# SonSang/dmesh2_renderer

Hardware: AMD Instinct MI355X
Metric: Mpixels/s fwd+bwd @1080p/1M tris (higher is better)
Workload: dtype f32

## Files before the change

dmesh2_renderer_amd/_C.py:

```python
from __future__ import annotations

import ctypes
import os
import threading

import torch

_HERE = os.path.dirname(os.path.abspath(__file__))
LIB_PATH = os.environ.get("DM2_HIP_LIB") or os.path.join(_HERE, "csrc", "libdm2_hip.so")
_lib = None
_lock = threading.Lock()

DM2_FLAG_CORRECTED_DV = 1
DM2_FLAG_LEGACY_KERNELS = 2
DM2_FLAG_NO_BACKWARD = 4
DM2_FLAG_ANALYTIC_RAYS = 8
DM2_FLAG_AA_GRAD_TO_VERTS = 16
DM2_FLAG_TABLES_FROM_IMAGE = 32
DM2_FLAG_NO_PAIR_POOL = 64
SCRATCH_FACE, SCRATCH_IMAGE, SCRATCH_BINNING, SCRATCH_LAYER_IMAGE, SCRATCH_LAYER_TETS, SCRATCH_PAIR_POOL, SCRATCH_TIE_QUEUE = range(7)
FWD_UNKNOWN, FWD_NONE, FWD_MASKS, FWD_POOL, FWD_POINT = 0, 1, 2, 3, 4
ABI_VERSION = 6

_flags = 0
_bin_hint: dict = {}

_vp, _i32, _i64, _sz = ctypes.c_void_p, ctypes.c_int32, ctypes.c_int64, ctypes.c_size_t


class RenderDesc(ctypes.Structure):
    _fields_ = [
        ("B", _i32), ("P", _i32), ("F", _i32), ("W", _i32), ("H", _i32), ("K", _i32),
        ("aa_temperature", ctypes.c_float), ("flags", _i32), ("full_W", _i32), ("full_H", _i32),
        ("background", _vp), ("patch_min", _vp), ("verts", _vp), ("faces", _vp), ("verts_color", _vp),
        ("faces_opacity", _vp), ("verts_ndc", _vp), ("verts_image", _vp), ("faces_intense", _vp),
        ("aa_face_verts", _vp), ("aa_face_edges", _vp), ("aa_face_edges_iszero", _vp),
        ("aa_face_edges_recip", _vp), ("aa_face_edges_normal", _vp), ("aa_face_edges_normal_c", _vp),
        ("image_ray_o", _vp), ("image_ray_d", _vp), ("ray_cam", _vp),
    ]


class PrepDesc(ctypes.Structure):
    _fields_ = [
        ("B", _i32), ("P", _i32), ("F", _i32), ("W", _i32), ("H", _i32),
        ("verts", _vp), ("faces", _vp), ("mv", _vp), ("proj", _vp),
        ("verts_ndc", _vp), ("verts_image", _vp), ("aa_face_verts", _vp), ("aa_face_edges", _vp),
        ("aa_face_edges_iszero", _vp), ("aa_face_edges_recip", _vp), ("aa_face_edges_normal", _vp),
        ("aa_face_edges_normal_c", _vp),
    ]


class LayersDesc(ctypes.Structure):
    _fields_ = [
        ("B", _i32), ("P", _i32), ("F", _i32), ("T", _i32), ("W", _i32), ("H", _i32), ("L", _i32), ("flags", _i32),
        ("verts", _vp), ("faces", _vp), ("tets", _vp), ("face_tets", _vp), ("tet_faces", _vp),
        ("face_existence", _vp), ("verts_ndc", _vp), ("verts_image", _vp), ("image_ray_o", _vp), ("image_ray_d", _vp),
        ("ray_cam", _vp),
    ]


class LayerCompositeDesc(ctypes.Structure):
    _fields_ = [
        ("B", _i32), ("P", _i32), ("F", _i32), ("W", _i32), ("H", _i32), ("L", _i32), ("flags", _i32),
        ("render_layers", _vp), ("verts", _vp), ("faces", _vp), ("verts_color", _vp), ("faces_opacity", _vp),
        ("faces_intense", _vp), ("verts_ndc", _vp), ("background", _vp), ("image_ray_o", _vp), ("image_ray_d", _vp),
        ("ray_cam", _vp),
    ]


EXPORTS = {
    "dm2_abi_version": (ctypes.c_int, []),
    "dm2_last_error": (ctypes.c_char_p, []),
    "dm2_scratch_bytes": (_sz, [ctypes.c_int, _i64, _i64]),
    "dm2_forward_plan": (ctypes.c_int, [ctypes.POINTER(RenderDesc), _vp, _sz, _vp, ctypes.POINTER(_i64), ctypes.POINTER(_i64), ctypes.POINTER(_i64)]),
    "dm2_forward_run": (ctypes.c_int, [ctypes.POINTER(RenderDesc), _i64, _i64, _i64, _vp, _sz, _vp, _sz, _vp, _sz, _vp, _vp, _vp, _vp,
                                       ctypes.POINTER(_i32)]),
    "dm2_forward": (ctypes.c_int, [ctypes.POINTER(RenderDesc), _vp, _sz, _vp, _sz, _vp, _sz, _vp, _vp, _vp, _vp,
                                   ctypes.POINTER(_i64), ctypes.POINTER(_i64), ctypes.POINTER(_i64), ctypes.POINTER(_i32)]),
    "dm2_backward": (ctypes.c_int, [ctypes.POINTER(RenderDesc), _i64, _i32, _vp, _vp, _vp, _sz, _vp, _sz, _vp, _sz, _vp, _sz,
                                    _vp, _vp, _vp, _vp, _vp, _vp, _vp]),
    "dm2_layers_plan": (ctypes.c_int, [ctypes.POINTER(LayersDesc), _vp, _sz, _vp, ctypes.POINTER(_i64), ctypes.POINTER(_i64)]),
    "dm2_layers_run": (ctypes.c_int, [ctypes.POINTER(LayersDesc), _i64, _i64, _vp, _sz, _vp, _sz, _vp, _sz, _vp, _sz, _vp, _vp, _vp]),
    "dm2_rasterize_run": (ctypes.c_int, [ctypes.POINTER(LayersDesc), _i64, _i64, _vp, _sz, _vp, _sz, _vp, _sz, _vp, _vp, _vp, _vp, _vp]),
    "dm2_rasterize_backward": (ctypes.c_int, [ctypes.POINTER(LayersDesc), _vp, _vp, _vp, _vp, _vp]),
    "dm2_interpolate": (ctypes.c_int, [_i32] * 8 + [_vp] * 6),
    "dm2_interpolate_backward": (ctypes.c_int, [_i32] * 8 + [_vp] * 8),
    "dm2_texture": (ctypes.c_int, [_i32] * 10 + [_vp] * 5),
    "dm2_texture_backward": (ctypes.c_int, [_i32] * 10 + [_vp] * 7),
    "dm2_layers_composite": (ctypes.c_int, [ctypes.POINTER(LayerCompositeDesc), _vp, _vp, _vp, _vp, _vp]),
    "dm2_layers_composite_backward": (ctypes.c_int, [ctypes.POINTER(LayerCompositeDesc), _vp, _vp, _vp, _vp, _vp, _vp, _vp, _vp]),
    "dm2_layers_composite_backward_alpha": (ctypes.c_int, [ctypes.POINTER(LayerCompositeDesc), _vp, _vp, _vp, _vp, _vp, _vp, _vp, _vp,
                                                            _vp]),
    "dm2_forward_alpha": (ctypes.c_int, [ctypes.POINTER(RenderDesc), _vp, _sz, _vp, _vp]),
    "dm2_forward_weights": (ctypes.c_int, [ctypes.POINTER(RenderDesc), _vp, _sz, _vp, _sz, _vp, _sz, _vp, _vp, _vp, _vp, _vp,
                                           ctypes.POINTER(_i64), ctypes.POINTER(_i64), ctypes.POINTER(_i64), ctypes.POINTER(_i32)]),
    "dm2_forward_run_weights": (ctypes.c_int, [ctypes.POINTER(RenderDesc), _i64, _i64, _i64, _vp, _sz, _vp, _sz, _vp, _sz, _vp, _vp,
                                               _vp, _vp, _vp, ctypes.POINTER(_i32)]),
    "dm2_layers_composite_weights": (ctypes.c_int, [ctypes.POINTER(LayerCompositeDesc), _vp, _vp, _vp, _vp, _vp, _vp]),
    "dm2_backward_alpha": (ctypes.c_int, [ctypes.POINTER(RenderDesc), _i64, _i32, _vp, _vp, _vp, _vp, _sz, _vp, _sz, _vp, _sz, _vp,
                                          _sz, _vp, _vp, _vp, _vp, _vp, _vp, _vp]),
    "dm2_prepare_faces": (ctypes.c_int, [ctypes.POINTER(PrepDesc), _vp]),
    "dm2_prepare_faces_backward": (ctypes.c_int, [ctypes.POINTER(PrepDesc), _vp, _vp, _vp, _vp, _vp, _vp]),
    "dm2_prepare_faces_camera_scratch_bytes": (_sz, [_i32, _i32]),
    "dm2_prepare_faces_backward_camera": (ctypes.c_int, [ctypes.POINTER(PrepDesc), _vp, _vp, _vp, _vp, _vp, _vp, _vp, _vp, _vp]),
    "dm2_exchange_mark": (ctypes.c_int, [_i32, _i32, _i32, _i32, _vp, _vp, _sz, _vp, _vp, _vp]),
    "dm2_exchange_pack": (ctypes.c_int, [_i32, _i32, _i32, _i32, _vp, _vp, _vp, _vp, _vp, _vp, _vp, _vp, _vp]),
    "dm2_exchange_unpack": (ctypes.c_int, [_i32, _i32, _i32, _i32, _i32, _vp, _vp, _i64, _vp, _vp, _vp]),
    "dm2_debug_aa_overlap": (ctypes.c_int, [ctypes.c_int, _i64, _vp, _vp, _vp, _vp, _vp, _vp, _vp, _vp, _vp, _vp, _vp]),
    "dm2_debug_fetch": (ctypes.c_int, [ctypes.c_int, _i64, _i64, _i64, _vp, _sz, _vp, _vp]),
    "dm2_profile_enable": (None, [ctypes.c_int]),
    "dm2_profile_read": (ctypes.c_int, [ctypes.POINTER(ctypes.c_float), ctypes.c_int]),
    "dm2_debug_stamps": (ctypes.c_int, [ctypes.POINTER(ctypes.c_uint64), ctypes.c_int, ctypes.c_int]),
}

STAGE_NAMES = ["preprocess_scan", "bin_scatter", "tile_sort", "tile_ranges", "forward_composite", "backward_composite", "backward_ties"]


def profile_enable(on: bool):
    load_library().dm2_profile_enable(1 if on else 0)


def profile_read():
    buf = (ctypes.c_float * len(STAGE_NAMES))()
    n = load_library().dm2_profile_read(buf, len(STAGE_NAMES))
    return {STAGE_NAMES[i]: float(buf[i]) for i in range(n)}


def load_library(path: str | None = None):
    global _lib
    with _lock:
        if _lib is not None and path is None:
            return _lib
        p = path or LIB_PATH
        if not os.path.exists(p):
            raise RuntimeError(
                f"dmesh2_renderer_amd: native library not found at {p}; build it with "
                f"`python -c 'import __graft_entry__ as g; g.build()'` or `make -C dmesh2_renderer_amd/csrc` "
                f"(there is no CPU fallback)")
        lib = ctypes.CDLL(p)
        for name, (res, args) in EXPORTS.items():
            fn = getattr(lib, name)
            fn.restype = res
            fn.argtypes = args
        if lib.dm2_abi_version() != ABI_VERSION:
            raise RuntimeError("dmesh2_renderer_amd: ABI version mismatch")
        if path is None:
            _lib = lib
        return lib


def set_flags(flags: int):
    global _flags
    old, _flags = _flags, int(flags)
    return old


def _err(lib, what):
    msg = lib.dm2_last_error()
    return RuntimeError(f"{what}: {msg.decode() if msg else 'unknown error'}")


def _require_gpu(*tensors):
    for t in tensors:
        if not t.is_cuda:
            raise RuntimeError(
                "dmesh2_renderer_amd: all tensors must live on a ROCm GPU (got a CPU tensor); "
                "this build has no CPU path -- the CPU restatement under oracle/ is test infrastructure only")
    dev = tensors[0].device
    for t in tensors:
        if t.device != dev:
            raise RuntimeError("dmesh2_renderer_amd: tensors are on different devices")
    return dev


def _c(t, dtype):
    if t.dtype != dtype:
        raise RuntimeError(f"expected dtype {dtype}, got {t.dtype}")
    return t.contiguous()


def _ptr(t):
    return ctypes.c_void_p(t.data_ptr() if t is not None and t.numel() > 0 else 0)


def _stream(dev):
    return ctypes.c_void_p(torch.cuda.current_stream(dev).cuda_stream)


def _bytes(dev, n):
    return torch.empty((max(int(n), 0),), dtype=torch.uint8, device=dev)


def _check_render_shapes(background, patch_min, verts, faces, verts_color, faces_opacity, verts_ndc, verts_image,
                         faces_intense, aa_v, aa_e, aa_z, aa_r, aa_n, aa_c, ray_o, ray_d, temp, K):
    def bad(cond, msg):
        if cond:
            raise RuntimeError(msg)
    bad(background.dim() != 1 or background.size(0) != 3, "background must have dimensions (3,)")
    bad(patch_min.dim() != 2 or patch_min.size(1) != 2, "patch_min must have dimensions (B, 2)")
    bad(verts.dim() != 2 or verts.size(1) != 3, "verts must have dimensions (P, 3)")
    bad(faces.dim() != 2 or faces.size(1) != 3, "faces must have dimensions (F, 3)")
    bad(verts_color.dim() != 2 or verts_color.size(1) != 3, "vert color must have dimensions (P, 3)")
    bad(faces_opacity.dim() != 1 or faces_opacity.size(0) != faces.size(0), "face opacity must have dimensions (F,)")
    bad(verts_ndc.dim() != 3 or verts_ndc.size(2) != 3, "verts_ndc must have dimensions (B, P, 3)")
    bad(verts_image.dim() != 3 or verts_image.size(2) != 2, "verts_image must have dimensions (B, P, 2)")
    bad(faces_intense.dim() != 2 or faces_intense.size(1) != faces.size(0), "faces_intense must have dimensions (B, F,)")
    for t, nm in ((aa_v, "aa_face_verts"), (aa_e, "aa_face_edges"), (aa_z, "aa_face_edges_iszero"),
                  (aa_r, "aa_face_edges_recip"), (aa_n, "aa_face_edges_normal")):
        bad(t.dim() != 4 or t.size(2) != 3 or t.size(3) != 2, f"{nm} must have dimensions (B, F, 3, 2)")
    bad(aa_c.dim() != 3 or aa_c.size(2) != 3, "aa_face_edges_normal_c must have dimensions (B, F, 3)")
    bad(ray_o.dim() != 4 or ray_o.size(3) != 3, "image_ray_o must have dimensions (B, H, W, 3)")
    bad(ray_d.dim() != 4 or ray_d.size(3) != 3, "image_ray_d must have dimensions (B, H, W, 3)")
    bad(temp < 0 or temp > 1, "aa_temperature must be in the range [0, 1]")
    bad(K < 0, "len_oarea_buffer must be non-negative")


def _make_desc(args, keep):
    (background, patch_min, pw, ph, verts, faces, verts_color, faces_opacity, verts_ndc, verts_image, faces_intense,
     temp, aa_v, aa_e, aa_z, aa_r, aa_n, aa_c, K, ray_o, ray_d) = args
    temp = float(temp); K = int(K); pw = int(pw); ph = int(ph)
    _check_render_shapes(background, patch_min, verts, faces, verts_color, faces_opacity, verts_ndc, verts_image,
                         faces_intense, aa_v, aa_e, aa_z, aa_r, aa_n, aa_c, ray_o, ray_d, temp, K)
    dev = _require_gpu(background, patch_min, verts, faces, verts_color, faces_opacity, verts_ndc, verts_image,
                       faces_intense, aa_v, aa_e, aa_z, aa_r, aa_n, aa_c, ray_o, ray_d)
    f32, i32 = torch.float32, torch.int32
    B, P, F = verts_ndc.size(0), verts.size(0), faces.size(0)
    def need(t, shape, nm):
        if tuple(t.shape) != tuple(shape):
            raise RuntimeError(f"{nm} has shape {tuple(t.shape)}, expected {tuple(shape)}")
    need(patch_min, (B, 2), "patch_min"); need(verts_color, (P, 3), "verts_color"); need(verts_ndc, (B, P, 3), "verts_ndc")
    need(verts_image, (B, P, 2), "verts_image"); need(faces_intense, (B, F), "faces_intense")
    from_image = bool(getattr(_tls, "tables_from_image", False))
    if not from_image:
        for t, nm in ((aa_v, "aa_face_verts"), (aa_e, "aa_face_edges"), (aa_z, "aa_face_edges_iszero"),
                      (aa_r, "aa_face_edges_recip"), (aa_n, "aa_face_edges_normal")):
            need(t, (B, F, 3, 2), nm)
        need(aa_c, (B, F, 3), "aa_face_edges_normal_c")
    ana = _analytic(B, dev)
    if ana is None:
        need(ray_o, (B, ph, pw, 3), "image_ray_o"); need(ray_d, (B, ph, pw, 3), "image_ray_d")
    if temp == 0.0:
        K = 0
    ts = dict(
        background=_c(background, f32), patch_min=_c(patch_min, i32), verts=_c(verts, f32), faces=_c(faces, i32),
        verts_color=_c(verts_color, f32), faces_opacity=_c(faces_opacity, f32), verts_ndc=_c(verts_ndc, f32),
        verts_image=_c(verts_image, f32), faces_intense=_c(faces_intense, f32), aa_face_verts=_c(aa_v, f32),
        aa_face_edges=_c(aa_e, f32), aa_face_edges_iszero=_c(aa_z, torch.bool), aa_face_edges_recip=_c(aa_r, f32),
        aa_face_edges_normal=_c(aa_n, f32), aa_face_edges_normal_c=_c(aa_c, f32), image_ray_o=_c(ray_o, f32),
        image_ray_d=_c(ray_d, f32))
    keep.append(ts)
    d = RenderDesc()
    d.B, d.P, d.F, d.W, d.H, d.K = B, P, F, pw, ph, K
    d.aa_temperature = temp
    d.flags = _flags
    for k, t in ts.items():
        setattr(d, k, t.data_ptr() if t.numel() > 0 else None)
    if from_image:
        d.flags |= DM2_FLAG_TABLES_FROM_IMAGE
        for k in ("aa_face_verts", "aa_face_edges", "aa_face_edges_iszero", "aa_face_edges_recip", "aa_face_edges_normal", "aa_face_edges_normal_c"):
            setattr(d, k, None)
    if ana is not None:
# ... 101 lines not shown

    def __exit__(self, *exc):
        _tls.fwd_mode = self.old


def last_forward_mode():
    return getattr(_tls, "last_fwd_mode", FWD_UNKNOWN)


def last_pair_bound():
    return getattr(_tls, "last_pair_bound", 0)


def _pool_budget(N, R):
    return min(max(256 * N, 16 * R, 1 << 24), 400_000_000)


def _analytic(B, dev):
    a = getattr(_tls, "analytic", None)
    if a is None:
        return None
    cam, w, h = a
    if cam.dtype != torch.float32 or tuple(cam.shape) != (B, 32) or cam.device != dev:
        raise RuntimeError(f"analytic_rays: ray_cam must be float32 (B, 32) on {dev}, got {cam.dtype} {tuple(cam.shape)} on {cam.device}")
    return cam.contiguous(), w, h


def render_forward_cuda(*args):
    if len(args) != 21:
        raise TypeError(f"render_forward_cuda() takes 21 positional arguments ({len(args)} given)")
    lib = load_library()
    keep: list = []
    d, dev, (B, P, F, W, H, K) = _make_desc(args, keep)
    if getattr(_tls, "forward_only", False):
        d.flags |= DM2_FLAG_NO_BACKWARD
    if getattr(_tls, "aa_to_verts", False):
        d.flags |= DM2_FLAG_AA_GRAD_TO_VERTS
    want_alpha = bool(getattr(_tls, "alpha_output", False))
    want_weights = bool(getattr(_tls, "face_weights_output", False))
    with torch.cuda.device(dev):
        st = _stream(dev)
        f32, i32 = torch.float32, torch.int32
        weights = torch.zeros((B, F), dtype=f32, device=dev) if want_weights else None
        color = torch.empty((B, H, W, 3), dtype=f32, device=dev)
        depth = torch.empty((B, H, W), dtype=f32, device=dev)
        oarea = torch.empty((B, H, W, 0), dtype=f32, device=dev)
        tri_id = torch.empty((B, H, W, 0), dtype=i32, device=dev)
        doarea = torch.empty((B, H, W, 0, 3, 2), dtype=f32, device=dev)
        N, Tn, BF = B * H * W, _tiles(B, W, H), B * F
        if P == 0 or BF == 0 or N == 0:
            color.zero_(); depth.zero_()
            tri_cnt = torch.zeros((B, H, W), dtype=i32, device=dev)
            e = _bytes(dev, 0)
            _tls.last_pair_bound = 0
            out = (0, color, depth, oarea, tri_id, tri_cnt, doarea, e, _bytes(dev, 0), _bytes(dev, 0))
            if want_alpha:
                out += (torch.zeros((B, H, W), dtype=f32, device=dev),)
            return out + (weights,) if want_weights else out
        tri_cnt = torch.empty((B, H, W), dtype=i32, device=dev)
        face_buf = _bytes(dev, lib.dm2_scratch_bytes(SCRATCH_FACE, BF, 2 * Tn + 1))
        img_buf = _bytes(dev, lib.dm2_scratch_bytes(SCRATCH_IMAGE, N, Tn))
        nr, longest, pairs, mode = _i64(0), _i64(0), _i64(0), _i32(0)
        key = (dev.index, B, W, H, F)
        with _lock:
            hint = _bin_hint.get(key, 0)
        if _pool_budget(N, 0) <= 0:
            d.flags |= DM2_FLAG_NO_PAIR_POOL
        bin_buf = _bytes(dev, hint)
        fwd_args = (ctypes.byref(d), _ptr(face_buf), face_buf.numel(), _ptr(bin_buf), bin_buf.numel(), _ptr(img_buf), img_buf.numel(),
                    _ptr(color), _ptr(depth), _ptr(tri_cnt))
        fwd_tail = (st, ctypes.byref(nr), ctypes.byref(longest), ctypes.byref(pairs), ctypes.byref(mode))
        if want_weights:
            rc = lib.dm2_forward_weights(*fwd_args, _ptr(weights), *fwd_tail)
        else:
            rc = lib.dm2_forward(*fwd_args, *fwd_tail)
        if rc not in (0, 2):
            raise _err(lib, "render_forward_cuda")
        R = int(nr.value)
        wants_pool = d.aa_temperature > 0.0 and not (d.flags & (DM2_FLAG_NO_BACKWARD | DM2_FLAG_LEGACY_KERNELS | DM2_FLAG_NO_PAIR_POOL))
        over = wants_pool and int(pairs.value) > _pool_budget(N, R)
        pool = lib.dm2_scratch_bytes(SCRATCH_PAIR_POOL, int(pairs.value), 0) if wants_pool and not over else 0
        need = lib.dm2_scratch_bytes(SCRATCH_BINNING, R, Tn) + pool
        if rc == 2 or (over and int(mode.value) == FWD_POOL):
            if over:
                d.flags |= DM2_FLAG_NO_PAIR_POOL
            bin_buf = _bytes(dev, need + need // 4)
            run_args = (ctypes.byref(d), R, int(longest.value), int(pairs.value), _ptr(face_buf), face_buf.numel(), _ptr(bin_buf),
                        bin_buf.numel(), _ptr(img_buf), img_buf.numel(), _ptr(color), _ptr(depth), _ptr(tri_cnt))
            if want_weights:
                weights.zero_()
                rc = lib.dm2_forward_run_weights(*run_args, _ptr(weights), st, ctypes.byref(mode))
            else:
                rc = lib.dm2_forward_run(*run_args, st, ctypes.byref(mode))
            if rc:
                raise _err(lib, "render_forward_cuda (run)")
        with _lock:
            hint = _bin_hint.get(key, 0)
            if need > hint or 2 * (need + need // 4) < hint:
                if len(_bin_hint) > 64:
                    _bin_hint.clear()
                _bin_hint[key] = need + need // 4
        if want_alpha:
            alpha = torch.empty((B, H, W), dtype=f32, device=dev)
            if lib.dm2_forward_alpha(ctypes.byref(d), _ptr(img_buf), img_buf.numel(), _ptr(alpha), st):
                raise _err(lib, "render_forward_cuda (alpha)")
    _tls.last_fwd_mode = int(mode.value)
    _tls.last_pair_bound = int(pairs.value)
    bin_buf._dm2_fwd_mode = int(mode.value)
    out = (R, color, depth, oarea, tri_id, tri_cnt, doarea, face_buf, bin_buf, img_buf)
    if want_alpha:
        out += (alpha,)
    return out + (weights,) if want_weights else out


def render_backward_cuda(*args, dL_dout_alpha=None):
    if len(args) != 31:
        raise TypeError(f"render_backward_cuda() takes 31 positional arguments ({len(args)} given)")
    lib = load_library()
    num_rendered = int(args[0])
    fwd_args = args[1:22]
    dL_dcolor, dL_ddepth = args[22], args[23]
    face_buf, bin_buf, img_buf = args[24], args[25], args[26]
    keep: list = []
    d, dev, (B, P, F, W, H, K) = _make_desc(fwd_args, keep)
    _require_gpu(dL_dcolor, dL_ddepth)
    f32 = torch.float32
    to_verts = bool(getattr(_tls, "aa_to_verts", False))
    if to_verts:
        d.flags |= DM2_FLAG_AA_GRAD_TO_VERTS
    sizes = [P * 3, P * 3, F, B * F, B * P * 3, B * P * 2 if to_verts else B * F * 6]
    packed = torch.zeros((sum(sizes),), dtype=f32, device=dev)
    parts = torch.split(packed, sizes)
    g_verts = parts[0].view(P, 3); g_color = parts[1].view(P, 3); g_opac = parts[2].view(F)
    g_int = parts[3].view(B, F); g_ndc = parts[4].view(B, P, 3)
    g_aa = parts[5].view(B, P, 2) if to_verts else parts[5].view(B, F, 3, 2)
    if F != 0 and P != 0 and num_rendered > 0 and B * H * W > 0:
        if tuple(dL_dcolor.shape) != (B, H, W, 3) or tuple(dL_ddepth.shape) != (B, H, W):
            raise RuntimeError("dL_dout_color / dL_dout_depth must have dimensions (B, H, W, 3) / (B, H, W)")
        dc = _c(dL_dcolor, f32); dd = _c(dL_ddepth, f32)
        da = None
        if dL_dout_alpha is not None:
            if tuple(dL_dout_alpha.shape) != (B, H, W):
                raise RuntimeError("dL_dout_alpha must have dimensions (B, H, W)")
            _require_gpu(dL_dcolor, dL_dout_alpha)
            da = _c(dL_dout_alpha, f32)
        mode = getattr(_tls, "fwd_mode", None)
        if mode is None:
            mode = getattr(bin_buf, "_dm2_fwd_mode", FWD_UNKNOWN)
        with torch.cuda.device(dev):
            tie_buf = None
            if mode not in (FWD_MASKS, FWD_NONE) and d.aa_temperature > 0.0 and not (d.flags & DM2_FLAG_LEGACY_KERNELS):
                pool_pairs = max(0, bin_buf.numel() - lib.dm2_scratch_bytes(SCRATCH_BINNING, num_rendered, _tiles(B, W, H))) // 4
                if pool_pairs > 0:
                    tie_buf = _bytes(dev, lib.dm2_scratch_bytes(SCRATCH_TIE_QUEUE, pool_pairs, 0))
            tail = (_ptr(face_buf), face_buf.numel(), _ptr(bin_buf), bin_buf.numel(), _ptr(img_buf), img_buf.numel(),
                    _ptr(tie_buf), tie_buf.numel() if tie_buf is not None else 0,
                    _ptr(g_verts), _ptr(g_color), _ptr(g_opac), _ptr(g_ndc), _ptr(g_int), _ptr(g_aa), _stream(dev))
            if da is None:
                rc = lib.dm2_backward(ctypes.byref(d), num_rendered, int(mode), _ptr(dc), _ptr(dd), *tail)
            else:
                rc = lib.dm2_backward_alpha(ctypes.byref(d), num_rendered, int(mode), _ptr(dc), _ptr(dd), _ptr(da), *tail)
            if rc:
                raise _err(lib, "render_backward_cuda")
    g_verts._dm2_packed = packed
    return g_verts, g_color, g_opac, g_ndc, g_int, g_aa


def generate_render_layers_cuda(width, height, verts, faces, tets, face_tets, tet_faces, face_existence,
                                verts_ndc, verts_image, image_ray_o, image_ray_d, num_layers):
    lib = load_library()

    def bad(cond, msg):
        if cond:
            raise RuntimeError(msg)
    bad(verts.dim() != 2 or verts.size(1) != 3, "verts must have dimensions (P, 3)")
    bad(faces.dim() != 2 or faces.size(1) != 3, "faces must have dimensions (F, 3)")
    bad(tets.dim() != 2 or tets.size(1) != 4, "tets must have dimensions (T, 4)")
    bad(face_tets.dim() != 2 or face_tets.size(1) != 2, "face_tets must have dimensions (F, 2)")
    bad(tet_faces.dim() != 2 or tet_faces.size(1) != 4, "tet_faces must have dimensions (T, 4)")
    bad(face_existence.dim() != 1 or face_existence.size(0) != faces.size(0), "face_existence must have dimensions (F,)")
    bad(verts_ndc.dim() != 3 or verts_ndc.size(2) != 3, "verts_ndc must have dimensions (B, P, 3)")
    bad(verts_image.dim() != 3 or verts_image.size(2) != 2, "verts_image must have dimensions (B, P, 2)")
    bad(image_ray_o.dim() != 4 or image_ray_o.size(3) != 3, "image_ray_o must have dimensions (B, H, W, 3)")
    bad(image_ray_d.dim() != 4 or image_ray_d.size(3) != 3, "image_ray_d must have dimensions (B, H, W, 3)")
    num_layers = int(num_layers); width = int(width); height = int(height)
    bad(num_layers < 0, "num_layers must be non-negative")
    dev = _require_gpu(verts, faces, tets, face_tets, tet_faces, face_existence, verts_ndc, verts_image, image_ray_o, image_ray_d)
    f32, i32 = torch.float32, torch.int32
    B, P, F, T = verts_ndc.size(0), verts.size(0), faces.size(0), tets.size(0)
    bad(tuple(face_tets.shape) != (F, 2), "face_tets must have dimensions (F, 2)")
    bad(tuple(tet_faces.shape) != (T, 4), "tet_faces must have dimensions (T, 4)")
    bad(tuple(verts_ndc.shape) != (B, P, 3) or tuple(verts_image.shape) != (B, P, 2), "verts_ndc/verts_image shape mismatch")
    ana = _analytic(B, dev)
    bad(ana is None and (tuple(image_ray_o.shape) != (B, height, width, 3) or tuple(image_ray_d.shape) != (B, height, width, 3)),
        "image_ray_o/image_ray_d must have dimensions (B, H, W, 3)")
    ts = dict(verts=_c(verts, f32), faces=_c(faces, i32), tets=_c(tets, i32), face_tets=_c(face_tets, i32),
              tet_faces=_c(tet_faces, i32), face_existence=_c(face_existence, i32), verts_ndc=_c(verts_ndc, f32),
              verts_image=_c(verts_image, f32), image_ray_o=_c(image_ray_o, f32), image_ray_d=_c(image_ray_d, f32))
    d = LayersDesc()
    d.B, d.P, d.F, d.T, d.W, d.H, d.L, d.flags = B, P, F, T, width, height, num_layers, _flags
    for k, t in ts.items():
        setattr(d, k, t.data_ptr() if t.numel() > 0 else None)
    if ana is not None:
        if (ana[1], ana[2]) != (width, height):
            raise RuntimeError("analytic_rays: the image size differs from generate_render_layers_cuda's width / height")
        d.flags |= DM2_FLAG_ANALYTIC_RAYS
        d.ray_cam = ana[0].data_ptr()
        d.image_ray_o = d.image_ray_d = None
    with torch.cuda.device(dev):
        st = _stream(dev)
        cnt = torch.zeros((B, height, width), dtype=i32, device=dev)
        layers = torch.full((B, height, width, num_layers), -1, dtype=i32, device=dev)
        N, Tn, BF = B * height * width, _tiles(B, width, height), B * F
        if N == 0:
            return layers, cnt
        face_buf = _bytes(dev, lib.dm2_scratch_bytes(SCRATCH_FACE, BF, 2 * Tn))
        img_buf = _bytes(dev, lib.dm2_scratch_bytes(SCRATCH_LAYER_IMAGE, N, Tn))
        nr, longest = _i64(0), _i64(0)
        if lib.dm2_layers_plan(ctypes.byref(d), _ptr(face_buf), face_buf.numel(), st, ctypes.byref(nr), ctypes.byref(longest)):
            raise _err(lib, "generate_render_layers_cuda (plan)")
        R = int(nr.value)
        bin_buf = _bytes(dev, lib.dm2_scratch_bytes(SCRATCH_BINNING, R, Tn))
        tet_buf = _bytes(dev, lib.dm2_scratch_bytes(SCRATCH_LAYER_TETS, T, 0))
        if lib.dm2_layers_run(ctypes.byref(d), R, int(longest.value), _ptr(face_buf), face_buf.numel(), _ptr(bin_buf), bin_buf.numel(),
                              _ptr(img_buf), img_buf.numel(), _ptr(tet_buf), tet_buf.numel(), _ptr(layers), _ptr(cnt), st):
            raise _err(lib, "generate_render_layers_cuda (run)")
    generate_render_layers_cuda.last_debug = (R, face_buf, bin_buf, img_buf)
    return layers, cnt


def _rasterize_desc(width, height, B, verts, faces, image_ray_o, image_ray_d, num_layers, keep, face_existence=None,
                    verts_ndc=None, verts_image=None):
    def bad(cond, msg):
        if cond:
            raise RuntimeError(msg)
    bad(verts.dim() != 2 or verts.size(1) != 3, "verts must have dimensions (P, 3)")
    bad(faces.dim() != 2 or faces.size(1) != 3, "faces must have dimensions (F, 3)")
    bad(face_existence is not None and (face_existence.dim() != 1 or face_existence.size(0) != faces.size(0)),
        "face_existence must have dimensions (F,)")
    bad(verts_ndc is not None and (verts_ndc.dim() != 3 or verts_ndc.size(2) != 3), "verts_ndc must have dimensions (B, P, 3)")
    bad(verts_image is not None and (verts_image.dim() != 3 or verts_image.size(2) != 2), "verts_image must have dimensions (B, P, 2)")
    bad(image_ray_o.dim() != 4 or image_ray_o.size(3) != 3, "image_ray_o must have dimensions (B, H, W, 3)")
    bad(image_ray_d.dim() != 4 or image_ray_d.size(3) != 3, "image_ray_d must have dimensions (B, H, W, 3)")
    num_layers = int(num_layers); width = int(width); height = int(height)
    bad(num_layers < 0, "num_layers must be non-negative")
    tensors = [t for t in (verts, faces, face_existence, verts_ndc, verts_image, image_ray_o, image_ray_d) if t is not None]
    dev = _require_gpu(*tensors)
    f32, i32 = torch.float32, torch.int32
    P, F = verts.size(0), faces.size(0)
    bad((verts_ndc is not None and tuple(verts_ndc.shape) != (B, P, 3)) or (verts_image is not None and tuple(verts_image.shape) != (B, P, 2)),
        "verts_ndc/verts_image shape mismatch")
    ana = _analytic(B, dev)
    bad(ana is None and (tuple(image_ray_o.shape) != (B, height, width, 3) or tuple(image_ray_d.shape) != (B, height, width, 3)),
        "image_ray_o/image_ray_d must have dimensions (B, H, W, 3)")
    ts = dict(verts=_c(verts, f32), faces=_c(faces, i32), image_ray_o=_c(image_ray_o, f32), image_ray_d=_c(image_ray_d, f32))
    for k, x, dt in (("face_existence", face_existence, i32), ("verts_ndc", verts_ndc, f32), ("verts_image", verts_image, f32)):
        if x is not None:
            ts[k] = _c(x, dt)
    keep += list(ts.values())
    d = LayersDesc()
    d.B, d.P, d.F, d.T, d.W, d.H, d.L, d.flags = B, P, F, 0, width, height, num_layers, _flags
    for k, t in ts.items():
        setattr(d, k, t.data_ptr() if t.numel() > 0 else None)
    if ana is not None:
        if (ana[1], ana[2]) != (width, height):
            raise RuntimeError("analytic_rays: the image size differs from the rasterize call's width / height")
        keep.append(ana[0])
        d.flags |= DM2_FLAG_ANALYTIC_RAYS
        d.ray_cam = ana[0].data_ptr()
        d.image_ray_o = d.image_ray_d = None
    return d, dev


def rasterize_layers_cuda(width, height, verts, faces, face_existence, verts_ndc, verts_image, image_ray_o, image_ray_d,
                          num_layers):
    lib = load_library()
    keep: list = []
    if verts_ndc is None or verts_ndc.dim() != 3 or verts_image is None:
        raise RuntimeError("verts_ndc / verts_image must have dimensions (B, P, 3) / (B, P, 2)")
    d, dev = _rasterize_desc(width, height, verts_ndc.size(0), verts, faces, image_ray_o, image_ray_d, num_layers, keep,
                             face_existence=face_existence, verts_ndc=verts_ndc, verts_image=verts_image)
    B, F, H, W, L = d.B, d.F, d.H, d.W, d.L
    f32, i32 = torch.float32, torch.int32
    N, Tn, BF = B * H * W, _tiles(B, W, H), B * F
    if N == 0 or L == 0 or F == 0:
        return (torch.full((B, H, W, L), -1, dtype=i32, device=dev), torch.zeros((B, H, W), dtype=i32, device=dev),
                torch.full((B, H, W, L, 3), -1.0, dtype=f32, device=dev), torch.full((B, H, W, L), -1.0, dtype=f32, device=dev))
    layers = torch.empty((B, H, W, L), dtype=i32, device=dev)
    cnt = torch.empty((B, H, W), dtype=i32, device=dev)
    bary = torch.empty((B, H, W, L, 3), dtype=f32, device=dev)
    t = torch.empty((B, H, W, L), dtype=f32, device=dev)
    with torch.cuda.device(dev):
        st = _stream(dev)
        face_buf = _bytes(dev, lib.dm2_scratch_bytes(SCRATCH_FACE, BF, 2 * Tn))
        img_buf = _bytes(dev, lib.dm2_scratch_bytes(SCRATCH_LAYER_IMAGE, N, Tn))
        nr, longest = _i64(0), _i64(0)
        if lib.dm2_layers_plan(ctypes.byref(d), _ptr(face_buf), face_buf.numel(), st, ctypes.byref(nr), ctypes.byref(longest)):
            raise _err(lib, "rasterize_layers_cuda (plan)")
        R = int(nr.value)
        bin_buf = _bytes(dev, lib.dm2_scratch_bytes(SCRATCH_BINNING, R, Tn))
        if lib.dm2_rasterize_run(ctypes.byref(d), R, int(longest.value), _ptr(face_buf), face_buf.numel(), _ptr(bin_buf),
                                 bin_buf.numel(), _ptr(img_buf), img_buf.numel(), _ptr(layers), _ptr(cnt), _ptr(bary), _ptr(t), st):
            raise _err(lib, "rasterize_layers_cuda (run)")
    return layers, cnt, bary, t


def rasterize_layers_backward_cuda(render_layers, verts, faces, image_ray_o, image_ray_d, dL_dbary, dL_dt):
# ... 197 lines not shown
    f32 = torch.float32
    color = torch.empty((B, H, W, 3), dtype=f32, device=dev)
    depth = torch.empty((B, H, W), dtype=f32, device=dev)
    final_T = torch.empty((B, H, W), dtype=f32, device=dev)
    n_contrib = torch.empty((B, H, W), dtype=torch.int32, device=dev)
    weights = torch.zeros((B, d.F), dtype=f32, device=dev) if getattr(_tls, "face_weights_output", False) else None
    extra = (weights,) if weights is not None else ()
    if B * H * W == 0:
        return (color, depth, final_T, n_contrib) + extra
    with torch.cuda.device(dev):
        if weights is None:
            rc = lib.dm2_layers_composite(ctypes.byref(d), _ptr(color), _ptr(depth), _ptr(final_T), _ptr(n_contrib), _stream(dev))
        else:
            rc = lib.dm2_layers_composite_weights(ctypes.byref(d), _ptr(color), _ptr(depth), _ptr(final_T), _ptr(n_contrib),
                                                  _ptr(weights), _stream(dev))
        if rc:
            raise _err(lib, "composite_layers_cuda")
    return (color, depth, final_T, n_contrib) + extra


def composite_layers_backward_cuda(render_layers, verts, faces, verts_color, faces_opacity, faces_intense, verts_ndc, background,
                                   image_ray_o, image_ray_d, n_contrib, dL_dcolor, dL_ddepth, dL_dout_alpha=None):
    lib = load_library()
    keep: list = []
    d, dev = _composite_desc(render_layers, verts, faces, verts_color, faces_opacity, faces_intense, verts_ndc, background,
                             image_ray_o, image_ray_d, keep)
    B, P, F, H, W = d.B, d.P, d.F, d.H, d.W
    f32 = torch.float32
    checks = [(n_contrib, (B, H, W), "n_contrib"), (dL_dcolor, (B, H, W, 3), "dL_dcolor"), (dL_ddepth, (B, H, W), "dL_ddepth")]
    if dL_dout_alpha is not None:
        checks.append((dL_dout_alpha, (B, H, W), "dL_dout_alpha"))
    for t, shape, nm in checks:
        if tuple(t.shape) != shape:
            raise RuntimeError(f"{nm} must have dimensions {shape}, got {tuple(t.shape)}")
        _require_gpu(render_layers, t)
    nc, gc, gd = _c(n_contrib, torch.int32), _c(dL_dcolor, f32), _c(dL_ddepth, f32)
    ga = _c(dL_dout_alpha, f32) if dL_dout_alpha is not None else None
    dcolor = torch.zeros((P, 3), dtype=f32, device=dev)
    dopacity = torch.zeros((F,), dtype=f32, device=dev)
    dndc = torch.zeros((B, P, 3), dtype=f32, device=dev)
    dintense = torch.zeros((B, F), dtype=f32, device=dev)
    if B * H * W == 0:
        return dcolor, dopacity, dndc, dintense
    with torch.cuda.device(dev):
        if ga is None:
            rc = lib.dm2_layers_composite_backward(ctypes.byref(d), _ptr(gc), _ptr(gd), _ptr(nc), _ptr(dcolor), _ptr(dopacity),
                                                   _ptr(dndc), _ptr(dintense), _stream(dev))
        else:
            rc = lib.dm2_layers_composite_backward_alpha(ctypes.byref(d), _ptr(gc), _ptr(gd), _ptr(ga), _ptr(nc), _ptr(dcolor),
                                                         _ptr(dopacity), _ptr(dndc), _ptr(dintense), _stream(dev))
        if rc:
            raise _err(lib, "composite_layers_backward_cuda")
    return dcolor, dopacity, dndc, dintense

def _prep_desc(verts, faces, mv, proj, width, height, keep):
    dev = _require_gpu(verts, faces, mv, proj)
    if verts.dim() != 2 or verts.size(1) != 3:
        raise RuntimeError("verts must have dimensions (P, 3)")
    if faces.dim() != 2 or faces.size(1) != 3:
        raise RuntimeError("faces must have dimensions (F, 3)")
    if mv.dim() != 3 or tuple(mv.shape[1:]) != (4, 4) or tuple(proj.shape) != tuple(mv.shape):
        raise RuntimeError("mv and proj must have dimensions (B, 4, 4)")
    f32, i32 = torch.float32, torch.int32
    v, fc, m, pr = _c(verts, f32), _c(faces, i32), _c(mv, f32), _c(proj, f32)
    keep += [v, fc, m, pr]
    d = PrepDesc()
    d.B, d.P, d.F, d.W, d.H = m.shape[0], v.shape[0], fc.shape[0], int(width), int(height)
    d.verts, d.faces, d.mv, d.proj = _ptr(v), _ptr(fc), _ptr(m), _ptr(pr)
    return d, dev


def prepare_faces(verts, faces, mv, proj, width, height, tables=True):
    lib = load_library()
    keep = []
    d, dev = _prep_desc(verts, faces, mv, proj, width, height, keep)
    B, P, F = d.B, d.P, d.F
    f32 = torch.float32
    ndc = torch.empty((B, P, 3), dtype=f32, device=dev)
    image = torch.empty((B, P, 2), dtype=f32, device=dev)
    d.verts_ndc, d.verts_image = _ptr(ndc), _ptr(image)
    outs = [ndc, image]
    if tables:
        aav, aae, aar, aan = (torch.empty((B, F, 3, 2), dtype=f32, device=dev) for _ in range(4))
        aaz = torch.empty((B, F, 3, 2), dtype=torch.bool, device=dev)
        aac = torch.empty((B, F, 3), dtype=f32, device=dev)
        d.aa_face_verts, d.aa_face_edges, d.aa_face_edges_iszero = _ptr(aav), _ptr(aae), _ptr(aaz)
        d.aa_face_edges_recip, d.aa_face_edges_normal, d.aa_face_edges_normal_c = _ptr(aar), _ptr(aan), _ptr(aac)
        outs += [aav, aae, aaz, aar, aan, aac]
    with torch.cuda.device(dev):
        if lib.dm2_prepare_faces(ctypes.byref(d), _stream(dev)):
            raise _err(lib, "dm2_prepare_faces")
    return tuple(outs)


def prepare_faces_backward(verts, faces, mv, proj, width, height, g_verts_ndc=None, g_verts_image=None, g_aa_face_verts=None,
                           need_verts=True, need_camera=False):
    lib = load_library()
    keep = []
    d, dev = _prep_desc(verts, faces, mv, proj, width, height, keep)
    f32 = torch.float32
    gs = []
    for g, shape in ((g_verts_ndc, (d.B, d.P, 3)), (g_verts_image, (d.B, d.P, 2)), (g_aa_face_verts, (d.B, d.F, 3, 2))):
        if g is not None:
            if tuple(g.shape) != shape:
                raise RuntimeError(f"upstream gradient has shape {tuple(g.shape)}, expected {shape}")
            g = _c(g, f32)
            _require_gpu(verts, g)
        gs.append(g)
    need_verts = bool(need_verts) or not need_camera
    scratch = torch.empty((d.B * d.P * 2,), dtype=f32, device=dev) if gs[2] is not None else None
    out = torch.empty((d.P, 3), dtype=f32, device=dev) if need_verts else None
    if not need_camera:
        with torch.cuda.device(dev):
            if lib.dm2_prepare_faces_backward(ctypes.byref(d), _ptr(gs[0]), _ptr(gs[1]), _ptr(gs[2]), _ptr(scratch), _ptr(out),
                                              _stream(dev)):
                raise _err(lib, "dm2_prepare_faces_backward")
        return out
    g_mv = torch.empty((d.B, 4, 4), dtype=f32, device=dev)
    g_proj = torch.empty((d.B, 4, 4), dtype=f32, device=dev)
    cam = _bytes(dev, lib.dm2_prepare_faces_camera_scratch_bytes(d.B, d.P))
    with torch.cuda.device(dev):
        if lib.dm2_prepare_faces_backward_camera(ctypes.byref(d), _ptr(gs[0]), _ptr(gs[1]), _ptr(gs[2]), _ptr(scratch), _ptr(out),
                                                 _ptr(g_mv), _ptr(g_proj), _ptr(cam), _stream(dev)):
            raise _err(lib, "dm2_prepare_faces_backward_camera")
    return out, g_mv, g_proj


def debug_fetch(what, count, aux, num_rendered, scratch, dtype, n):
    lib = load_library()
    out = torch.empty((n,), dtype=dtype, device=scratch.device)
    if n == 0:
        return out
    with torch.cuda.device(scratch.device):
        if lib.dm2_debug_fetch(what, count, aux, num_rendered, _ptr(scratch), scratch.numel(), _ptr(out), _stream(scratch.device)):
            raise _err(lib, "debug_fetch")
    return out


def debug_aa_overlap(variant, aa_v, aa_e, aa_z, aa_r, aa_n, aa_c, pixmin):
    lib = load_library()
    dev = _require_gpu(aa_v, aa_e, aa_z, aa_r, aa_n, aa_c, pixmin)
    f32 = torch.float32
    n = aa_v.shape[0]
    ts = [_c(aa_v, f32), _c(aa_e, f32), _c(aa_z, torch.bool), _c(aa_r, f32), _c(aa_n, f32), _c(aa_c, f32), _c(pixmin, f32)]
    area = torch.zeros((n,), dtype=f32, device=dev)
    grad = torch.zeros((n, 3, 2), dtype=f32, device=dev)
    code = torch.zeros((n,), dtype=torch.int32, device=dev)
    with torch.cuda.device(dev):
        if lib.dm2_debug_aa_overlap(int(variant), n, *[_ptr(t) for t in ts], _ptr(area), _ptr(grad), _ptr(code), _stream(dev)):
            raise _err(lib, "debug_aa_overlap")
    return area, grad, code


def touched_faces(face_buf, B, F):
    t = debug_fetch(8, B * F, 1, 0, face_buf, torch.int32, B * F)
    return (t.view(B, F) != 0).any(dim=0)


def exchange_mark(face_buf, faces, B, P, N):
    lib = load_library()
    dev = _require_gpu(face_buf, faces)
    F = faces.shape[0]
    fc = _c(faces, torch.int32)
    flags = torch.empty((F + P,), dtype=torch.uint8, device=dev)
    counts = torch.empty((N, 2), dtype=torch.int32, device=dev)
    with torch.cuda.device(dev):
        if lib.dm2_exchange_mark(B, P, F, N, _ptr(fc), _ptr(face_buf), face_buf.numel(), _ptr(flags), _ptr(counts), _stream(dev)):
            raise _err(lib, "dm2_exchange_mark")
    return flags, counts


def exchange_pack(flags, counts, total_floats, dverts, dcolor, dopacity, dintense):
    lib = load_library()
    dev = _require_gpu(flags, counts, dverts, dcolor, dopacity, dintense)
    f32 = torch.float32
    P, F, B, N = dverts.shape[0], dopacity.shape[0], dintense.shape[0], counts.shape[0]
    ts = [_c(dverts, f32), _c(dcolor, f32), _c(dopacity, f32), _c(dintense, f32)]
    send = torch.empty((int(total_floats),), dtype=f32, device=dev)
    cursors = torch.empty((N, 2), dtype=torch.int32, device=dev)
    with torch.cuda.device(dev):
        if lib.dm2_exchange_pack(B, P, F, N, _ptr(flags), _ptr(counts), _ptr(cursors), *[_ptr(t) for t in ts], _ptr(send), _stream(dev)):
            raise _err(lib, "dm2_exchange_pack")
    return send


def exchange_unpack(recv, recv_counts, rows, rank, B, P, F):
    lib = load_library()
    dev = _require_gpu(recv)
    recv_counts = torch.as_tensor(recv_counts, dtype=torch.int32, device="cpu").reshape(-1, 2).contiguous()
    N = recv_counts.shape[0]
    Ps, Fs = -(-P // N), -(-F // N)
    slice_v = torch.empty((Ps, 6), dtype=torch.float32, device=dev)
    slice_f = torch.empty((Fs, 1 + B), dtype=torch.float32, device=dev)
    with torch.cuda.device(dev):
        if lib.dm2_exchange_unpack(B, P, F, N, int(rank), _ptr(recv), ctypes.c_void_p(recv_counts.data_ptr()), int(rows), _ptr(slice_v), _ptr(slice_f),
                                   _stream(dev)):
            raise _err(lib, "dm2_exchange_unpack")
    return slice_v, slice_f
```

dmesh2_renderer_amd/csrc/dm2_api.hip:

```cpp
#include <hip/hip_runtime.h>

#include <cstdio>
#include <cstring>
#include <string>

#include "dm2_device_math.h"
#include "dm2_stamps.h"
#include "dm2_state.h"

#ifdef DM2_STAMPS
namespace dm2 {
unsigned long long* stamps_table() {
    static unsigned long long* p = nullptr;
    if (!p) { (void)hipMalloc((void**)&p, 2 * DM2_NSTAMP * sizeof(unsigned long long)); (void)hipMemset(p, 0, 2 * DM2_NSTAMP * sizeof(unsigned long long)); }
    return p;
}
}
#endif

namespace {

thread_local std::string g_err;

int fail(const std::string& m) { g_err = m; return 1; }
// ... 8 lines not shown
    uint32_t* p = nullptr;
    uint32_t* dp = nullptr;
    int dev = -1;
    uint32_t seq = 0;
    hipEvent_t ev = nullptr;
    ~PinnedWord() { if (p) (void)hipHostFree(p); if (ev) (void)hipEventDestroy(ev); }
};
thread_local PinnedWord g_pin;

int plan_meta_prepare(uint32_t** host_meta_dev, uint32_t* seq) {
    if (!g_pin.p) {
        DM2_HIP(hipHostMalloc((void**)&g_pin.p, 64, hipHostMallocMapped | hipHostMallocPortable));
        for (int k = 0; k < 8; k++) g_pin.p[k] = 0u;
    }
    int cur = 0;
    DM2_HIP(hipGetDevice(&cur));
    if (cur != g_pin.dev) {
        void* dp = nullptr;
        DM2_HIP(hipHostGetDevicePointer(&dp, g_pin.p, 0));
        g_pin.dp = (uint32_t*)dp; g_pin.dev = cur;
        if (g_pin.ev) { (void)hipEventDestroy(g_pin.ev); g_pin.ev = nullptr; }
    }
    if (!g_pin.ev) DM2_HIP(hipEventCreateWithFlags(&g_pin.ev, hipEventDisableTiming));
    g_pin.seq = g_pin.seq + 1u ? g_pin.seq + 1u : 1u;
    *host_meta_dev = g_pin.dp; *seq = g_pin.seq;
    return 0;
}
int plan_meta_wait(const uint32_t* plan_meta, hipStream_t st, int64_t* num_rendered, int64_t* max_tile_entries, int64_t* pair_bound) {
    DM2_HIP(hipEventRecord(g_pin.ev, st));
    volatile uint32_t* hp = g_pin.p;
    uint32_t r = 0, longest = 0, plo = 0, phi = 0;
    bool seen = false;
    auto take = [&]() { r = hp[0]; longest = hp[1]; plo = hp[2]; phi = hp[3]; seen = true; };
    for (long spin = 0; ; spin++) {
        if (__atomic_load_n(&hp[4], __ATOMIC_ACQUIRE) == g_pin.seq) { take(); break; }
        if ((spin & 1023) == 1023) {
            if (hipEventQuery(g_pin.ev) != hipErrorNotReady) {
                if (__atomic_load_n(&hp[4], __ATOMIC_ACQUIRE) == g_pin.seq) take();
                break;
            }
            if (spin > (1l << 17)) { (void)hipEventSynchronize(g_pin.ev); if (__atomic_load_n(&hp[4], __ATOMIC_ACQUIRE) == g_pin.seq) take(); break; }
        }
        __builtin_ia32_pause();
    }
    if (!seen) {
        uint32_t tmp[4] = {0u, 0u, 0u, 0u};
        DM2_HIP(hipMemcpyAsync(tmp, plan_meta, sizeof(tmp), hipMemcpyDeviceToHost, st));
        DM2_HIP(hipStreamSynchronize(st));
        r = tmp[0]; longest = tmp[1]; plo = tmp[2]; phi = tmp[3];
    }
    *num_rendered = (int64_t)r;
    *max_tile_entries = (int64_t)longest;
    if (pair_bound) *pair_bound = (int64_t)(((uint64_t)phi << 32) | plo);
    if (longest == 0xFFFFFFFFu) { *num_rendered = 0; *max_tile_entries = 0; return fail("more than 2^31 - 1 (tile, face) pairs: render smaller patches"); }
    return 0;
}

int check_render_desc(const dm2_render_desc* d) {
    if (!d) return fail("null descriptor");
    if (d->B < 0 || d->P < 0 || d->F < 0 || d->W < 0 || d->H < 0) return fail("negative size in descriptor");
    if (d->aa_temperature < 0 || d->aa_temperature > 1) return fail("aa_temperature must be in the range [0, 1]");
    if (d->K < 0) return fail("len_oarea_buffer must be non-negative");
    const int64_t gx = (d->W + dm2::TILE - 1) / dm2::TILE, gy = (d->H + dm2::TILE - 1) / dm2::TILE;
    if (gx > 0xFFFF || gy > 0xFFFF) return fail("patch too large: more than 65535 tiles per axis");
    if (d->B > 65535) return fail("more than 65535 views per call");
    if ((int64_t)d->B * gx * gy >= (1ll << 31)) return fail("too many tiles");
    if (!(d->flags & DM2_FLAG_TABLES_FROM_IMAGE) && d->B > 0 && d->F > 0 && d->P > 0 &&
        (!d->aa_face_verts || !d->aa_face_edges || !d->aa_face_edges_iszero || !d->aa_face_edges_recip || !d->aa_face_edges_normal || !d->aa_face_edges_normal_c))
        return fail("the aa_face_* tables must not be null (or set DM2_FLAG_TABLES_FROM_IMAGE)");
    if (d->flags & DM2_FLAG_ANALYTIC_RAYS) {
        if (!d->ray_cam && d->B > 0) return fail("DM2_FLAG_ANALYTIC_RAYS needs ray_cam");
        if (d->full_W <= 0 || d->full_H <= 0) return fail("DM2_FLAG_ANALYTIC_RAYS needs the full image size");
    }
    return 0;
}

struct Profiler {
    bool on = false;
    hipEvent_t ev[2 * DM2_PROFILE_STAGES] = {};
    bool have[DM2_PROFILE_STAGES] = {};
    bool created = false;
};
thread_local Profiler g_prof;

inline int64_t tiles_of(int B, int W, int H) {
    return (int64_t)B * ((W + dm2::TILE - 1) / dm2::TILE) * ((H + dm2::TILE - 1) / dm2::TILE);
}

}

namespace dm2 {
void prof_begin(int stage, hipStream_t st) {
    Profiler& p = g_prof;
    if (!p.on) return;
    if (!p.created) { for (auto& e : p.ev) (void)hipEventCreate(&e); p.created = true; }
    (void)hipEventRecord(p.ev[2 * stage], st);
}
void prof_end(int stage, hipStream_t st) {
    Profiler& p = g_prof;
    if (!p.on) return;
    (void)hipEventRecord(p.ev[2 * stage + 1], st);
    p.have[stage] = true;
}
}

extern "C" {

void dm2_profile_enable(int on) {
    g_prof.on = on != 0;
    for (auto& h : g_prof.have) h = false;
}

int dm2_profile_read(float* ms, int capacity) {
    Profiler& p = g_prof;
    int n = 0;
    for (int s = 0; s < DM2_PROFILE_STAGES && s < capacity; s++, n++) {
        ms[s] = 0.f;
        if (!p.on || !p.have[s]) continue;
        if (hipEventSynchronize(p.ev[2 * s + 1]) != hipSuccess) continue;
        float t = 0.f;
        if (hipEventElapsedTime(&t, p.ev[2 * s], p.ev[2 * s + 1]) == hipSuccess) ms[s] = t;
    }
    return n;
}

int dm2_debug_stamps(uint64_t* out, int capacity, int reset) {
#ifdef DM2_STAMPS
    unsigned long long h[2][DM2_NSTAMP];
    if (hipMemcpy(h, dm2::stamps_table(), sizeof(h), hipMemcpyDeviceToHost) != hipSuccess) return -2;
    int n = 0;
    for (int k = 0; k < 2; k++) for (int i = 0; i < DM2_NSTAMP && n < capacity; i++) out[n++] = h[k][i];
    if (reset) (void)hipMemset(dm2::stamps_table(), 0, sizeof(h));
    return n;
#else
    (void)out; (void)capacity; (void)reset;
    return -1;
#endif
}

int dm2_abi_version(void) { return DM2_ABI_VERSION; }
const char* dm2_last_error(void) { return g_err.c_str(); }

size_t dm2_scratch_bytes(int kind, int64_t count, int64_t aux) {
    size_t total = 0;
    if (count < 0) count = 0;
    if (aux < 0) aux = 0;
    switch (kind) {
        case DM2_SCRATCH_FACE: dm2::FaceState::carve(nullptr, count, aux >> 1, dm2::scan_temp_bytes(count), (aux & 1) != 0, &total); break;
        case DM2_SCRATCH_IMAGE: dm2::ImageState::carve(nullptr, count, aux, &total); break;
        case DM2_SCRATCH_BINNING: dm2::BinningState::carve(nullptr, count, dm2::sort_temp_bytes(count, aux), &total); break;
        case DM2_SCRATCH_LAYER_IMAGE: dm2::LayerImageState::carve(nullptr, count, aux, &total); break;
        case DM2_SCRATCH_LAYER_TETS: return dm2::tet_scratch_bytes(count);
        case DM2_SCRATCH_PAIR_POOL: return dm2::BinningState::pool_bytes(count);
        case DM2_SCRATCH_TIE_QUEUE: return count > 0 ? (size_t)count * sizeof(dm2::TieEntry) + dm2::ALIGN : 0;
        default: return 0;
    }
    return total;
}

static int forward_plan(const dm2_render_desc* d, void* face_scratch, size_t face_bytes, void* stream, int64_t* num_rendered,
                        int64_t* max_tile_entries, int64_t* pair_bound, uint2* ranges_to_clear, uint32_t* tile_order) {
    if (check_render_desc(d)) return 1;
    if (!num_rendered || !max_tile_entries) return fail("num_rendered / max_tile_entries is null");
    hipStream_t st = (hipStream_t)stream;
    const int64_t BF = (int64_t)d->B * d->F, Tn = tiles_of(d->B, d->W, d->H);
    *num_rendered = 0; *max_tile_entries = 0;
    if (pair_bound) *pair_bound = 0;
    if (d->P == 0 || BF == 0 || Tn == 0) return 0;
    if (dm2_scratch_bytes(DM2_SCRATCH_FACE, BF, 2 * Tn + 1) > face_bytes) return fail("face scratch too small");
    dm2::FaceState fs = dm2::FaceState::carve(face_scratch, BF, Tn, dm2::scan_temp_bytes(BF), true);
    uint32_t* host_meta = nullptr; uint32_t seq = 0;
    if (plan_meta_prepare(&host_meta, &seq)) return 1;
    DM2_HIP(dm2::launch_preprocess_scan(d->B, d->P, d->F, d->W, d->H, d->patch_min, d->faces, d->verts_ndc, d->verts_image, fs, d,
                                        host_meta, seq, ranges_to_clear, tile_order, st));
    DM2_HIP(hipGetLastError());
    return plan_meta_wait(fs.plan_meta, st, num_rendered, max_tile_entries, pair_bound);
}

int dm2_forward_plan(const dm2_render_desc* d, void* face_scratch, size_t face_bytes, void* stream, int64_t* num_rendered,
                     int64_t* max_tile_entries, int64_t* pair_bound) {
    return forward_plan(d, face_scratch, face_bytes, stream, num_rendered, max_tile_entries, pair_bound, nullptr, nullptr);
}

static int forward_run(const dm2_render_desc* d, int64_t num_rendered, int64_t max_tile_entries, int64_t pair_bound, void* face_scratch, size_t face_bytes,
                       void* binning_scratch, size_t binning_bytes, void* image_scratch, size_t image_bytes,
                       float* out_color, float* out_depth, int32_t* out_tri_cnt, float* out_face_weights, void* stream,
                       bool ranges_cleared, int32_t* forward_mode) {
    if (forward_mode) *forward_mode = DM2_FWD_NONE;
    if (check_render_desc(d)) return 1;
    hipStream_t st = (hipStream_t)stream;
    const int64_t BF = (int64_t)d->B * d->F, N = (int64_t)d->B * d->H * d->W, Tn = tiles_of(d->B, d->W, d->H);
    if (N == 0) return 0;
    if (dm2_scratch_bytes(DM2_SCRATCH_IMAGE, N, Tn) > image_bytes) return fail("image scratch too small");
    dm2::ImageState is = dm2::ImageState::carve(image_scratch, N, Tn);
    const bool have_faces = (d->P != 0 && BF != 0);
    dm2::BinningState bs{};
    if (have_faces) {
        if (dm2_scratch_bytes(DM2_SCRATCH_FACE, BF, 2 * Tn + 1) > face_bytes) return fail("face scratch too small");
        if (dm2_scratch_bytes(DM2_SCRATCH_BINNING, num_rendered, Tn) > binning_bytes) return fail("binning scratch too small");
        dm2::FaceState fs = dm2::FaceState::carve(face_scratch, BF, Tn, dm2::scan_temp_bytes(BF), true);
        bs = dm2::BinningState::carve(binning_scratch, num_rendered, dm2::sort_temp_bytes(num_rendered, Tn), nullptr, binning_bytes);
        is.face_recs = fs.recs;
        DM2_HIP(dm2::launch_bin_sort(d->B, d->F, d->W, d->H, num_rendered, max_tile_entries, (d->flags & DM2_FLAG_LEGACY_KERNELS) != 0,
                                     fs.depths, fs, bs, is.ranges, ranges_cleared, is.tile_order, st));
    } else {
        DM2_HIP(hipMemsetAsync(is.ranges, 0, (size_t)Tn * sizeof(uint2), st));
        dm2::launch_tile_order_identity(Tn, is.tile_order, st);
    }
    const bool use_pool = have_faces && pair_bound > 0 && bs.pool_cap >= pair_bound && !(d->flags & DM2_FLAG_NO_PAIR_POOL);
    const float pairs_per_entry = num_rendered > 0 ? (float)((double)pair_bound / (double)num_rendered) : 0.0f;
    const int mode = dm2::launch_render_forward(*d, is.ranges, bs.face_list, is, out_color, out_depth, out_tri_cnt, bs, use_pool, pairs_per_entry,
                                                out_face_weights, st);
    if (forward_mode) *forward_mode = mode;
    DM2_HIP(hipGetLastError());
    return 0;
}

int dm2_forward_run(const dm2_render_desc* d, int64_t num_rendered, int64_t max_tile_entries, int64_t pair_bound, void* face_scratch, size_t face_bytes,
                    void* binning_scratch, size_t binning_bytes, void* image_scratch, size_t image_bytes,
                    float* out_color, float* out_depth, int32_t* out_tri_cnt, void* stream, int32_t* forward_mode) {
    return dm2_forward_run_weights(d, num_rendered, max_tile_entries, pair_bound, face_scratch, face_bytes, binning_scratch, binning_bytes,
                                   image_scratch, image_bytes, out_color, out_depth, out_tri_cnt, nullptr, stream, forward_mode);
}

int dm2_forward_run_weights(const dm2_render_desc* d, int64_t num_rendered, int64_t max_tile_entries, int64_t pair_bound,
                            void* face_scratch, size_t face_bytes, void* binning_scratch, size_t binning_bytes,
                            void* image_scratch, size_t image_bytes, float* out_color, float* out_depth, int32_t* out_tri_cnt,
                            float* out_face_weights, void* stream, int32_t* forward_mode) {
    return forward_run(d, num_rendered, max_tile_entries, pair_bound, face_scratch, face_bytes, binning_scratch, binning_bytes, image_scratch,
                       image_bytes, out_color, out_depth, out_tri_cnt, out_face_weights, stream, false, forward_mode);
}

int dm2_forward(const dm2_render_desc* d, void* face_scratch, size_t face_bytes, void* binning_scratch, size_t binning_bytes,
                void* image_scratch, size_t image_bytes, float* out_color, float* out_depth, int32_t* out_tri_cnt, void* stream,
                int64_t* num_rendered, int64_t* max_tile_entries, int64_t* pair_bound, int32_t* forward_mode) {
    return dm2_forward_weights(d, face_scratch, face_bytes, binning_scratch, binning_bytes, image_scratch, image_bytes, out_color,
                               out_depth, out_tri_cnt, nullptr, stream, num_rendered, max_tile_entries, pair_bound, forward_mode);
}

int dm2_forward_weights(const dm2_render_desc* d, void* face_scratch, size_t face_bytes, void* binning_scratch, size_t binning_bytes,
                        void* image_scratch, size_t image_bytes, float* out_color, float* out_depth, int32_t* out_tri_cnt,
                        float* out_face_weights, void* stream, int64_t* num_rendered, int64_t* max_tile_entries, int64_t* pair_bound,
                        int32_t* forward_mode) {
    if (check_render_desc(d)) return 1;
    if (!pair_bound) return fail("pair_bound is null");
    if (forward_mode) *forward_mode = DM2_FWD_NONE;
    const int64_t N = (int64_t)d->B * d->H * d->W, Tn = tiles_of(d->B, d->W, d->H);
    uint2* ranges = nullptr; uint32_t* tile_order = nullptr;
    if (N > 0 && image_scratch && dm2_scratch_bytes(DM2_SCRATCH_IMAGE, N, Tn) <= image_bytes) {
        const dm2::ImageState is0 = dm2::ImageState::carve(image_scratch, N, Tn);
        ranges = is0.ranges; tile_order = is0.tile_order;
    }
    if (forward_plan(d, face_scratch, face_bytes, stream, num_rendered, max_tile_entries, pair_bound, ranges, tile_order)) return 1;
    const bool planned = d->P != 0 && (int64_t)d->B * d->F != 0 && Tn != 0;
    const bool wants_pool = d->aa_temperature > 0.0f && !(d->flags & (DM2_FLAG_NO_BACKWARD | DM2_FLAG_LEGACY_KERNELS | DM2_FLAG_NO_PAIR_POOL));
    if (dm2_scratch_bytes(DM2_SCRATCH_BINNING, *num_rendered, Tn) + (wants_pool ? dm2_scratch_bytes(DM2_SCRATCH_PAIR_POOL, *pair_bound, 0) : 0) > binning_bytes)
        return 2;
    return forward_run(d, *num_rendered, *max_tile_entries, *pair_bound, face_scratch, face_bytes, binning_scratch, binning_bytes,
                       image_scratch, image_bytes, out_color, out_depth, out_tri_cnt, out_face_weights, stream, planned && ranges != nullptr,
                       forward_mode);
}

int dm2_forward_alpha(const dm2_render_desc* d, const void* image_scratch, size_t image_bytes, float* out_alpha, void* stream) {
    if (check_render_desc(d)) return 1;
    const int64_t N = (int64_t)d->B * d->H * d->W, Tn = tiles_of(d->B, d->W, d->H);
    if (N == 0) return 0;
    if (!image_scratch || !out_alpha) return fail("image_scratch / out_alpha must not be null");
    if (dm2_scratch_bytes(DM2_SCRATCH_IMAGE, N, Tn) > image_bytes) return fail("image scratch too small");
    dm2::launch_forward_alpha(dm2::ImageState::carve(const_cast<void*>(image_scratch), N, Tn), N, out_alpha, (hipStream_t)stream);
    DM2_HIP(hipGetLastError());
    return 0;
}

int dm2_backward(const dm2_render_desc* d, int64_t num_rendered, int32_t forward_mode, const float* dL_dout_color, const float* dL_dout_depth,
                 const void* face_scratch, size_t face_bytes, void* binning_scratch, size_t binning_bytes,
                 const void* image_scratch, size_t image_bytes, void* tie_scratch, size_t tie_bytes,
                 float* dL_dverts, float* dL_dverts_color, float* dL_dfaces_opacity, float* dL_dverts_ndc,
                 float* dL_dfaces_intense, float* dL_daa_face_verts, void* stream) {
    return dm2_backward_alpha(d, num_rendered, forward_mode, dL_dout_color, dL_dout_depth, nullptr, face_scratch, face_bytes,
                              binning_scratch, binning_bytes, image_scratch, image_bytes, tie_scratch, tie_bytes, dL_dverts,
                              dL_dverts_color, dL_dfaces_opacity, dL_dverts_ndc, dL_dfaces_intense, dL_daa_face_verts, stream);
}

int dm2_backward_alpha(const dm2_render_desc* d, int64_t num_rendered, int32_t forward_mode, const float* dL_dout_color,
                       const float* dL_dout_depth, const float* dL_dout_alpha,
                       const void* face_scratch, size_t face_bytes, void* binning_scratch, size_t binning_bytes,
                       const void* image_scratch, size_t image_bytes, void* tie_scratch, size_t tie_bytes,
                       float* dL_dverts, float* dL_dverts_color, float* dL_dfaces_opacity, float* dL_dverts_ndc,
                       float* dL_dfaces_intense, float* dL_daa_face_verts, void* stream) {
    if (check_render_desc(d)) return 1;
    hipStream_t st = (hipStream_t)stream;
    const int64_t N = (int64_t)d->B * d->H * d->W, Tn = tiles_of(d->B, d->W, d->H);
    if (d->F == 0 || d->P == 0 || N == 0 || num_rendered <= 0) return 0;
    const int64_t BF = (int64_t)d->B * d->F;
    if (dm2_scratch_bytes(DM2_SCRATCH_FACE, BF, 2 * Tn + 1) > face_bytes) return fail("face scratch too small");
    if (dm2_scratch_bytes(DM2_SCRATCH_IMAGE, N, Tn) > image_bytes) return fail("image scratch too small");
    if (dm2_scratch_bytes(DM2_SCRATCH_BINNING, num_rendered, Tn) > binning_bytes) return fail("binning scratch too small");
    dm2::ImageState is = dm2::ImageState::carve(const_cast<void*>(image_scratch), N, Tn);
    if (forward_mode < DM2_FWD_UNKNOWN || forward_mode > DM2_FWD_POINT) return fail("forward_mode must be one of DM2_FWD_*");
    dm2::BinningState bs = dm2::BinningState::carve(binning_scratch, num_rendered, dm2::sort_temp_bytes(num_rendered, Tn), nullptr, binning_bytes);
    is.face_recs = dm2::FaceState::carve(const_cast<void*>(face_scratch), BF, Tn, dm2::scan_temp_bytes(BF), true).recs;
    dm2::TieEntry* tie_queue = nullptr; int64_t tie_cap = 0;
    if (tie_scratch && tie_bytes >= sizeof(dm2::TieEntry) + dm2::ALIGN) {
        dm2::Carver c(tie_scratch);
        tie_queue = c.take<dm2::TieEntry>(0);
        tie_cap = (int64_t)((tie_bytes - c.used(tie_scratch)) / sizeof(dm2::TieEntry));
    }
    const bool pool_route = d->aa_temperature > 0.0f && !(d->flags & DM2_FLAG_LEGACY_KERNELS) &&
                            (forward_mode == DM2_FWD_POOL || forward_mode == DM2_FWD_UNKNOWN || forward_mode == DM2_FWD_POINT);
    if (pool_route) {
        if (forward_mode == DM2_FWD_POOL && bs.pool_cap <= 0) return fail("forward_mode is DM2_FWD_POOL but the binning scratch has no pool part");
        if (tie_cap < bs.pool_cap) return fail("tie scratch too small for the pool part of the binning scratch");
    }
    dm2::launch_render_backward(*d, is.ranges, bs.face_list, is, dL_dout_color, dL_dout_depth, dL_dverts, dL_dverts_color,
                                dL_dfaces_opacity, dL_dverts_ndc, dL_dfaces_intense, dL_daa_face_verts, bs, forward_mode, tie_queue, tie_cap,
                                dL_dout_alpha, st);
    DM2_HIP(hipGetLastError());
    return 0;
}

static int check_layers_desc(const dm2_layers_desc* d) {
    if (!d) return fail("null descriptor");
    if (d->B < 0 || d->P < 0 || d->F < 0 || d->T < 0 || d->W < 0 || d->H < 0) return fail("negative size in descriptor");
    if (d->L < 0) return fail("num_layers must be non-negative");
    const int64_t gx = (d->W + dm2::TILE - 1) / dm2::TILE, gy = (d->H + dm2::TILE - 1) / dm2::TILE;
    if (gx > 0xFFFF || gy > 0xFFFF || d->B > 65535) return fail("image too large");
    if ((int64_t)d->B * gx * gy >= (1ll << 31)) return fail("too many tiles");
    if ((d->flags & DM2_FLAG_ANALYTIC_RAYS) && !d->ray_cam && d->B > 0) return fail("DM2_FLAG_ANALYTIC_RAYS needs ray_cam");
    return 0;
}

int dm2_layers_plan(const dm2_layers_desc* d, void* face_scratch, size_t face_bytes, void* stream, int64_t* num_rendered,
                    int64_t* max_tile_entries) {
    if (check_layers_desc(d)) return 1;
    if (!num_rendered || !max_tile_entries) return fail("num_rendered / max_tile_entries is null");
    hipStream_t st = (hipStream_t)stream;
    const int64_t BF = (int64_t)d->B * d->F, Tn = tiles_of(d->B, d->W, d->H);
    *num_rendered = 0; *max_tile_entries = 0;
    if (BF == 0 || Tn == 0) return 0;
    if (dm2_scratch_bytes(DM2_SCRATCH_FACE, BF, 2 * Tn) > face_bytes) return fail("face scratch too small");
    dm2::FaceState fs = dm2::FaceState::carve(face_scratch, BF, Tn, dm2::scan_temp_bytes(BF), false);
    uint32_t* host_meta = nullptr; uint32_t seq = 0;
    if (plan_meta_prepare(&host_meta, &seq)) return 1;
    DM2_HIP(dm2::launch_preprocess_scan(d->B, d->P, d->F, d->W, d->H, nullptr, d->faces, d->verts_ndc, d->verts_image, fs, nullptr,
                                        host_meta, seq, nullptr, nullptr, st));
    DM2_HIP(hipGetLastError());
    return plan_meta_wait(fs.plan_meta, st, num_rendered, max_tile_entries, nullptr);
}

int dm2_layers_run(const dm2_layers_desc* d, int64_t num_rendered, int64_t max_tile_entries, void* face_scratch, size_t face_bytes,
                   void* binning_scratch, size_t binning_bytes, void* image_scratch, size_t image_bytes,
                   void* tet_scratch, size_t tet_bytes,
                   int32_t* render_layers, int32_t* render_layers_cnt, void* stream) {
    if (check_layers_desc(d)) return 1;
    hipStream_t st = (hipStream_t)stream;
    const int64_t BF = (int64_t)d->B * d->F, N = (int64_t)d->B * d->H * d->W, Tn = tiles_of(d->B, d->W, d->H);
    if (N == 0) return 0;
    if (dm2_scratch_bytes(DM2_SCRATCH_LAYER_IMAGE, N, Tn) > image_bytes) return fail("image scratch too small");
    dm2::LayerImageState ls = dm2::LayerImageState::carve(image_scratch, N, Tn);
    dm2::FaceState fs{};
    dm2::BinningState bs{};
    if (BF != 0) {
        if (dm2_scratch_bytes(DM2_SCRATCH_FACE, BF, 2 * Tn) > face_bytes) return fail("face scratch too small");
        if (dm2_scratch_bytes(DM2_SCRATCH_BINNING, num_rendered, Tn) > binning_bytes) return fail("binning scratch too small");
        fs = dm2::FaceState::carve(face_scratch, BF, Tn, dm2::scan_temp_bytes(BF), false);
        bs = dm2::BinningState::carve(binning_scratch, num_rendered, dm2::sort_temp_bytes(num_rendered, Tn));
        DM2_HIP(dm2::launch_bin_sort(d->B, d->F, d->W, d->H, num_rendered, max_tile_entries, (d->flags & DM2_FLAG_LEGACY_KERNELS) != 0,
                                     fs.min_depths, fs, bs, ls.ranges, false, nullptr, st));
    } else {
        DM2_HIP(hipMemsetAsync(ls.ranges, 0, (size_t)Tn * sizeof(uint2), st));
    }
    if (tet_scratch && dm2_scratch_bytes(DM2_SCRATCH_LAYER_TETS, d->T, 0) > tet_bytes) return fail("tet scratch too small");
    dm2::launch_layers(*d, fs, ls.ranges, bs.face_list, ls, tet_scratch, render_layers, render_layers_cnt, st);
    DM2_HIP(hipGetLastError());
    return 0;
}

static int check_rasterize_inputs(const dm2_layers_desc* d) {
    if (d->F > 0 && d->B > 0 && (!d->verts || !d->faces)) return fail("verts / faces must not be null");
    if (!(d->flags & DM2_FLAG_ANALYTIC_RAYS) && d->B > 0 && (!d->image_ray_o || !d->image_ray_d))
        return fail("image_ray_o / image_ray_d must not be null");
    return 0;
}

int dm2_rasterize_run(const dm2_layers_desc* d, int64_t num_rendered, int64_t max_tile_entries, void* face_scratch, size_t face_bytes,
                      void* binning_scratch, size_t binning_bytes, void* image_scratch, size_t image_bytes,
                      int32_t* render_layers, int32_t* render_layers_cnt, float* bary, float* t, void* stream) {
    if (check_layers_desc(d) || check_rasterize_inputs(d)) return 1;
    hipStream_t st = (hipStream_t)stream;
    const int64_t BF = (int64_t)d->B * d->F, N = (int64_t)d->B * d->H * d->W, Tn = tiles_of(d->B, d->W, d->H);
    if (N == 0) return 0;
    if (!render_layers_cnt || (d->L > 0 && (!render_layers || !bary || !t))) return fail("rasterize outputs must not be null");
    if (d->L == 0) {
        DM2_HIP(hipMemsetAsync(render_layers_cnt, 0, (size_t)N * sizeof(int32_t), st));
        return 0;
    }
    if (dm2_scratch_bytes(DM2_SCRATCH_LAYER_IMAGE, N, Tn) > image_bytes) return fail("image scratch too small");
    dm2::LayerImageState ls = dm2::LayerImageState::carve(image_scratch, N, Tn);
    dm2::FaceState fs{};
    dm2::BinningState bs{};
    if (BF != 0) {
        if (dm2_scratch_bytes(DM2_SCRATCH_FACE, BF, 2 * Tn) > face_bytes) return fail("face scratch too small");
        if (dm2_scratch_bytes(DM2_SCRATCH_BINNING, num_rendered, Tn) > binning_bytes) return fail("binning scratch too small");
        fs = dm2::FaceState::carve(face_scratch, BF, Tn, dm2::scan_temp_bytes(BF), false);
        bs = dm2::BinningState::carve(binning_scratch, num_rendered, dm2::sort_temp_bytes(num_rendered, Tn));
        DM2_HIP(dm2::launch_bin_sort(d->B, d->F, d->W, d->H, num_rendered, max_tile_entries, (d->flags & DM2_FLAG_LEGACY_KERNELS) != 0,
                                     fs.min_depths, fs, bs, ls.ranges, false, nullptr, st));
    } else {
        DM2_HIP(hipMemsetAsync(ls.ranges, 0, (size_t)Tn * sizeof(uint2), st));
    }
    dm2::launch_rasterize(*d, fs, ls.ranges, bs.face_list, render_layers, render_layers_cnt, bary, t, st);
    DM2_HIP(hipGetLastError());
    return 0;
}

int dm2_rasterize_backward(const dm2_layers_desc* d, const int32_t* render_layers, const float* dL_dbary, const float* dL_dt,
                           float* dL_dverts, void* stream) {
    if (check_layers_desc(d) || check_rasterize_inputs(d)) return 1;
    if ((int64_t)d->B * d->H * d->W == 0 || d->L == 0 || d->F == 0 || (!dL_dbary && !dL_dt)) return 0;
    if (!render_layers || !dL_dverts) return fail("render_layers / dL_dverts must not be null");
    dm2::launch_rasterize_backward(*d, render_layers, dL_dbary, dL_dt, dL_dverts, (hipStream_t)stream);
    DM2_HIP(hipGetLastError());
    return 0;
}

static int check_interpolate_sizes(int32_t B, int32_t H, int32_t W, int32_t L, int32_t F, int32_t N, int32_t C, int32_t view_tables) {
    if (B < 0 || H < 0 || W < 0 || L < 0 || F < 0 || N < 0) return fail("interpolate: negative size");
    if (C < 1) return fail("interpolate: C must be at least 1");
    if (view_tables && (int64_t)B * N > 0x7FFFFFFF) return fail("interpolate: B * N must be below 2^31");
    if (((int64_t)B * H * W * L + 255) / 256 > 0x7FFFFFFF || B > 65535) return fail("interpolate: too many slots or views");
    return 0;
}

int dm2_interpolate(int32_t B, int32_t H, int32_t W, int32_t L, int32_t F, int32_t N, int32_t C, int32_t view_tables,
                    const int32_t* render_layers, const float* bary, const float* attr, const int32_t* attr_faces,
                    float* out, void* stream) {
    if (check_interpolate_sizes(B, H, W, L, F, N, C, view_tables)) return 1;
    const int64_t S = (int64_t)B * H * W * L;
    if (S == 0) return 0;
    if (!out) return fail("interpolate: out must not be null");
    if (F == 0 || N == 0) {
        DM2_HIP(hipMemsetAsync(out, 0, (size_t)S * C * sizeof(float), (hipStream_t)stream));
        return 0;
    }
    if (!render_layers || !bary || !attr || !attr_faces) return fail("interpolate: inputs must not be null");
    dm2::launch_interpolate(B, H, W, L, F, N, C, view_tables, render_layers, bary, attr, attr_faces, out, (hipStream_t)stream);
    DM2_HIP(hipGetLastError());
    return 0;
}

int dm2_interpolate_backward(int32_t B, int32_t H, int32_t W, int32_t L, int32_t F, int32_t N, int32_t C, int32_t view_tables,
                             const int32_t* render_layers, const float* bary, const float* attr, const int32_t* attr_faces,
                             const float* dL_dout, float* dL_dattr, float* dL_dbary, void* stream) {
    if (check_interpolate_sizes(B, H, W, L, F, N, C, view_tables)) return 1;
    const int64_t S = (int64_t)B * H * W * L;
    if (S == 0 || (!dL_dattr && !dL_dbary)) return 0;
    if (F == 0 || N == 0) {
        if (dL_dbary) DM2_HIP(hipMemsetAsync(dL_dbary, 0, (size_t)S * 3 * sizeof(float), (hipStream_t)stream));
        return 0;
    }
    if (!render_layers || !attr_faces || !dL_dout) return fail("interpolate_backward: inputs must not be null");
    if (dL_dattr && !bary) return fail("interpolate_backward: bary must not be null");
    if (dL_dbary && !attr) return fail("interpolate_backward: attr must not be null");
    dm2::launch_interpolate_backward(B, H, W, L, F, N, C, view_tables, render_layers, bary, attr, attr_faces, dL_dout, dL_dattr,
                                     dL_dbary, (hipStream_t)stream);
// ... 50 lines not shown
    const int64_t gx = (d->W + dm2::TILE - 1) / dm2::TILE, gy = (d->H + dm2::TILE - 1) / dm2::TILE;
    if (gx > 0x7FFFFFFF || gy > 0xFFFF || d->B > 65535) return fail("image too large");
    const int64_t N = (int64_t)d->B * d->H * d->W;
    if (N == 0) return 0;
    if (!d->background) return fail("background must not be null");
    if (d->L > 0 && !d->render_layers) return fail("render_layers must not be null");
    if (d->F > 0 && (!d->faces || !d->verts || !d->verts_color || !d->faces_opacity || !d->faces_intense || !d->verts_ndc))
        return fail("the per-face / per-vertex inputs must not be null");
    if (d->flags & DM2_FLAG_ANALYTIC_RAYS) {
        if (!d->ray_cam) return fail("DM2_FLAG_ANALYTIC_RAYS needs ray_cam");
    } else if (!d->image_ray_o || !d->image_ray_d) {
        return fail("image_ray_o / image_ray_d must not be null");
    }
    return 0;
}

int dm2_layers_composite(const dm2_layer_composite_desc* d, float* out_color, float* out_depth, float* out_final_T,
                         int32_t* out_n_contrib, void* stream) {
    return dm2_layers_composite_weights(d, out_color, out_depth, out_final_T, out_n_contrib, nullptr, stream);
}

int dm2_layers_composite_weights(const dm2_layer_composite_desc* d, float* out_color, float* out_depth, float* out_final_T,
                                 int32_t* out_n_contrib, float* out_face_weights, void* stream) {
    if (check_composite_desc(d)) return 1;
    if ((int64_t)d->B * d->H * d->W == 0) return 0;
    if (!out_color || !out_depth || !out_n_contrib) return fail("out_color / out_depth / out_n_contrib must not be null");
    dm2::launch_layer_composite(*d, out_color, out_depth, out_final_T, out_n_contrib, out_face_weights, (hipStream_t)stream);
    DM2_HIP(hipGetLastError());
    return 0;
}

int dm2_layers_composite_backward(const dm2_layer_composite_desc* d, const float* dL_dout_color, const float* dL_dout_depth,
                                  const int32_t* n_contrib, float* dL_dverts_color, float* dL_dfaces_opacity,
                                  float* dL_dverts_ndc, float* dL_dfaces_intense, void* stream) {
    return dm2_layers_composite_backward_alpha(d, dL_dout_color, dL_dout_depth, nullptr, n_contrib, dL_dverts_color,
                                               dL_dfaces_opacity, dL_dverts_ndc, dL_dfaces_intense, stream);
}

int dm2_layers_composite_backward_alpha(const dm2_layer_composite_desc* d, const float* dL_dout_color, const float* dL_dout_depth,
                                        const float* dL_dout_alpha, const int32_t* n_contrib, float* dL_dverts_color,
                                        float* dL_dfaces_opacity, float* dL_dverts_ndc, float* dL_dfaces_intense, void* stream) {
    if (check_composite_desc(d)) return 1;
    if ((int64_t)d->B * d->H * d->W == 0 || d->L == 0 || d->F == 0) return 0;
    if (!dL_dout_color || !dL_dout_depth || !n_contrib) return fail("dL_dout_color / dL_dout_depth / n_contrib must not be null");
    if (!dL_dverts_color || !dL_dfaces_opacity || !dL_dverts_ndc || !dL_dfaces_intense) return fail("gradient outputs must not be null");
    dm2::launch_layer_composite_backward(*d, dL_dout_color, dL_dout_depth, n_contrib, dL_dverts_color, dL_dfaces_opacity,
                                         dL_dverts_ndc, dL_dfaces_intense, dL_dout_alpha, (hipStream_t)stream);
    DM2_HIP(hipGetLastError());
    return 0;
}

static int check_prep_desc(const dm2_prep_desc* d) {
    if (!d) return fail("null descriptor");
    if (d->B < 0 || d->P < 0 || d->F < 0 || d->W < 0 || d->H < 0) return fail("negative size in descriptor");
    if (d->B > 65535) return fail("more than 65535 views per call");
    if (d->P > 0 && d->B > 0 && (!d->verts || !d->mv || !d->proj)) return fail("verts, mv and proj must not be null");
    if (d->F > 0 && !d->faces) return fail("faces must not be null");
    return 0;
}

int dm2_prepare_faces(const dm2_prep_desc* d, void* stream) {
    if (check_prep_desc(d)) return 1;
    const bool tables = d->aa_face_verts || d->aa_face_edges || d->aa_face_edges_iszero || d->aa_face_edges_recip ||
                        d->aa_face_edges_normal || d->aa_face_edges_normal_c;
    if (tables && d->F > 0 && d->B > 0 && !d->verts_image) return fail("the AA tables are built from verts_image: it must not be null");
    dm2::launch_prepare_faces(*d, (hipStream_t)stream);
    DM2_HIP(hipGetLastError());
    return 0;
}

int dm2_prepare_faces_backward(const dm2_prep_desc* d, const float* g_verts_ndc, const float* g_verts_image,
                               const float* g_aa_face_verts, float* image_grad_scratch, float* g_verts, void* stream) {
    if (check_prep_desc(d)) return 1;
    if (d->P > 0 && !g_verts) return fail("g_verts must not be null");
    return dm2_prepare_faces_backward_camera(d, g_verts_ndc, g_verts_image, g_aa_face_verts, image_grad_scratch, g_verts, nullptr,
                                             nullptr, nullptr, stream);
}

size_t dm2_prepare_faces_camera_scratch_bytes(int32_t B, int32_t P) { return dm2::prepare_camera_scratch_bytes(B, P); }

int dm2_prepare_faces_backward_camera(const dm2_prep_desc* d, const float* g_verts_ndc, const float* g_verts_image,
                                      const float* g_aa_face_verts, float* image_grad_scratch, float* g_verts, float* g_mv,
                                      float* g_proj, void* camera_scratch, void* stream) {
    if (check_prep_desc(d)) return 1;
    const bool camera = (g_mv || g_proj) && d->B > 0;
    if (g_aa_face_verts && d->F > 0 && d->B > 0 && d->P > 0 && (g_verts || camera) && !image_grad_scratch)
        return fail("image_grad_scratch must not be null");
    if (camera && dm2::prepare_camera_scratch_bytes(d->B, d->P) > 0 && !camera_scratch) return fail("camera_scratch must not be null");
    dm2::launch_prepare_faces_backward(*d, g_verts_ndc, g_verts_image, g_aa_face_verts, image_grad_scratch, g_verts, g_mv, g_proj,
                                       (double*)camera_scratch, (hipStream_t)stream);
    DM2_HIP(hipGetLastError());
    return 0;
}

static int check_exchange(int32_t B, int32_t P, int32_t F, int32_t N) {
    if (B < 0 || P < 0 || F < 0) return fail("negative size");
    if (N < 1 || N > dm2::exchange_max_ranks()) return fail("dm2_exchange_*: 1 <= N <= 64 ranks");
    return 0;
}

int dm2_exchange_mark(int32_t B, int32_t P, int32_t F, int32_t N, const int32_t* faces, const void* face_scratch, size_t face_bytes,
                      uint8_t* flags, uint32_t* counts, void* stream) {
    if (check_exchange(B, P, F, N)) return 1;
    if (!flags || !counts) return fail("dm2_exchange_mark: null output");
    const int64_t BF = (int64_t)B * F;
    const uint32_t* touched = nullptr;
    if (BF > 0 && P > 0) {
        if (!faces || !face_scratch) return fail("dm2_exchange_mark: null input");
        dm2::FaceState fs = dm2::FaceState::carve(const_cast<void*>(face_scratch), BF, 0, dm2::scan_temp_bytes(BF), false);
        touched = fs.tiles_touched;
        if ((size_t)((const char*)(touched + BF) - (const char*)face_scratch) > face_bytes) return fail("dm2_exchange_mark: face scratch too small");
    }
    DM2_HIP(dm2::launch_exchange_mark(B, P, F, N, faces, touched, flags, counts, (hipStream_t)stream));
    DM2_HIP(hipGetLastError());
    return 0;
}

int dm2_exchange_pack(int32_t B, int32_t P, int32_t F, int32_t N, const uint8_t* flags, const uint32_t* counts, uint32_t* cursors,
                      const float* dverts, const float* dverts_color, const float* dfaces_opacity, const float* dfaces_intense,
                      float* send, void* stream) {
    if (check_exchange(B, P, F, N)) return 1;
    if (!flags || !counts || !cursors) return fail("dm2_exchange_pack: null scratch");
    if (P > 0 && F > 0 && (!dverts || !dverts_color || !dfaces_opacity || !dfaces_intense)) return fail("dm2_exchange_pack: null gradient");
    DM2_HIP(dm2::launch_exchange_pack(B, P, F, N, flags, counts, cursors, dverts, dverts_color, dfaces_opacity, dfaces_intense, send, (hipStream_t)stream));
    DM2_HIP(hipGetLastError());
    return 0;
}

int dm2_exchange_unpack(int32_t B, int32_t P, int32_t F, int32_t N, int32_t rank, const float* recv, const uint32_t* recv_counts,
                        int64_t rows, float* slice_v, float* slice_f, void* stream) {
    if (check_exchange(B, P, F, N)) return 1;
    if (rank < 0 || rank >= N) return fail("dm2_exchange_unpack: rank out of range");
    if (!slice_v || !slice_f || !recv_counts || (rows > 0 && !recv)) return fail("dm2_exchange_unpack: null pointer");
    DM2_HIP(dm2::launch_exchange_unpack(B, P, F, N, rank, recv, recv_counts, rows, slice_v, slice_f, (hipStream_t)stream));
    DM2_HIP(hipGetLastError());
    return 0;
}

int dm2_debug_aa_overlap(int variant, int64_t n, const float* aa_face_verts, const float* aa_face_edges,
                         const uint8_t* aa_face_edges_iszero, const float* aa_face_edges_recip, const float* aa_face_edges_normal,
                         const float* aa_face_edges_normal_c, const float* pixmin, float* area, float* grad, int32_t* code,
                         void* stream) {
    if (variant < 0 || variant > 4) return fail("dm2_debug_aa_overlap: unknown variant");
    if (n < 0) return fail("dm2_debug_aa_overlap: negative count");
    if (n > 0 && (!aa_face_verts || !aa_face_edges || !aa_face_edges_iszero || !aa_face_edges_recip || !aa_face_edges_normal ||
                  !aa_face_edges_normal_c || !pixmin || !area || !grad || !code))
        return fail("dm2_debug_aa_overlap: null pointer");
    dm2::launch_debug_aa_overlap(variant, n, aa_face_verts, aa_face_edges, aa_face_edges_iszero, aa_face_edges_recip,
                                 aa_face_edges_normal, aa_face_edges_normal_c, pixmin, area, grad, code, (hipStream_t)stream);
    DM2_HIP(hipGetLastError());
    return 0;
}

int dm2_debug_fetch(int what, int64_t count, int64_t aux, int64_t num_rendered, const void* scratch, size_t scratch_bytes,
                    void* dst, void* stream) {
    hipStream_t st = (hipStream_t)stream;
    void* base = const_cast<void*>(scratch);
    const void* src = nullptr; size_t bytes = 0;
    switch (what) {
        case 0: { auto s = dm2::ImageState::carve(base, count, aux); src = s.ranges; bytes = (size_t)aux * 8; break; }
        case 1: { auto s = dm2::BinningState::carve(base, num_rendered, dm2::sort_temp_bytes(num_rendered, aux)); src = s.face_list; bytes = (size_t)num_rendered * 4; break; }
        case 2: { auto s = dm2::ImageState::carve(base, count, aux); src = s.final_T; bytes = (size_t)count * 4; break; }
        case 3: { auto s = dm2::ImageState::carve(base, count, aux); src = s.final_prev_T; bytes = (size_t)count * 4; break; }
        case 4: { auto s = dm2::ImageState::carve(base, count, aux); src = s.n_contrib; bytes = (size_t)count * 4; break; }
        case 5: { auto s = dm2::LayerImageState::carve(base, count, aux); src = s.first_face; bytes = (size_t)count * 4; break; }
        case 6: { auto s = dm2::LayerImageState::carve(base, count, aux); src = s.first_tet; bytes = (size_t)count * 4; break; }
        case 7: { auto s = dm2::LayerImageState::carve(base, count, aux); src = s.ranges; bytes = (size_t)aux * 8; break; }
        case 8: { auto s = dm2::FaceState::carve(base, count, 0, dm2::scan_temp_bytes(count), false); src = s.tiles_touched; bytes = (size_t)count * 4; break; }
        case 9: { auto s = dm2::BinningState::carve(base, num_rendered, dm2::sort_temp_bytes(num_rendered, aux)); src = s.hit_valid; bytes = 4 * 4; break; }
        default: return fail("dm2_debug_fetch: unknown item");
    }
    if (!scratch && bytes) return fail("dm2_debug_fetch: null scratch");
    if (bytes && (size_t)((const char*)src - (const char*)scratch) + bytes > scratch_bytes) return fail("dm2_debug_fetch: item lies beyond scratch_bytes");
    if (bytes) DM2_HIP(hipMemcpyAsync(dst, src, bytes, hipMemcpyDeviceToDevice, st));
    return 0;
}

}
```

dmesh2_renderer_amd/csrc/dm2_backward_fast.hip:

```cpp
#include <hip/hip_runtime.h>

#include "dm2_bwd_shared.h"
#include "dm2_clip_fast.h"
#include "dm2_clip_seg.h"
#include "dm2_device_math.h"
#include "dm2_dpp.h"
#include "dm2_pairs.h"
#include "dm2_stage.h"
#include "dm2_stamps.h"
#include "dm2_state.h"

namespace dm2 {

#ifndef DM2_BF_CAND
#define DM2_BF_CAND 30
#endif
#ifndef DM2_BF_BLOCKS
#define DM2_BF_BLOCKS 4
#endif
enum Coverage { POOL, POINT, CLIP };
template <Coverage COV> struct BfTraits {
    using Rec = FaceRecB;
    static constexpr int PARTS = FACE_RECB_PARTS;
    static __device__ __forceinline__ int src_part(int rp) { return recb_src_part(rp); }
    static constexpr int CAND = DM2_BF_CAND, BLOCKS = DM2_BF_BLOCKS;
};
template <> struct BfTraits<CLIP> {
    using Rec = FaceRec;
    static constexpr int PARTS = (int)(sizeof(FaceRec) / 16);
    static __device__ __forceinline__ int src_part(int rp) { return rp; }
    static constexpr int CAND = 32, BLOCKS = 3;
};

template <Coverage COV, bool ALPHA>
__global__ void __launch_bounds__(TILE_PIX, BfTraits<COV>::BLOCKS)
k_render_backward_fast(dm2_render_desc d, const uint2* __restrict__ ranges, const uint32_t* __restrict__ face_list,
                       ImageState is, const float* __restrict__ dL_dcolor, const float* __restrict__ dL_ddepth,
                       float* __restrict__ dL_dverts, float* __restrict__ dL_dverts_color,
                       float* __restrict__ dL_dfaces_opacity, float* __restrict__ dL_dverts_ndc,
                       float* __restrict__ dL_dfaces_intense, float* __restrict__ dL_daa_face_verts,
                       const uint64_t* __restrict__ hit_masks, uint32_t* __restrict__ hit_valid,
                       const uint32_t* __restrict__ hit_base, const float* __restrict__ pool,
                       TieEntry* __restrict__ tie_queue, uint32_t tie_cap, bool check_mode,
                       const float* __restrict__ dL_dalpha STAMP_PARAM) {
    if (check_mode && hit_valid[0] != (COV == POINT ? 1u : COV == CLIP ? 2u : 3u)) return;
    using Rec = typename BfTraits<COV>::Rec;
    constexpr int BM_CAND = BfTraits<COV>::CAND;
    static_assert(BM_CAND * 4 <= TILE_PIX && 2 * BM_CAND <= 64, "one scan thread per (face, wave); one id window per wave");
    constexpr int BM_SLOTS = BM_CAND * 4;
    constexpr int REC_CHUNKS = BfTraits<COV>::PARTS;
    constexpr int REC_PER_INSTR = 64 / REC_CHUNKS;
    static_assert(8 * REC_PER_INSTR >= BM_CAND, "two LDS-direct instructions per wave fetch a chunk");

    __shared__ Rec recs2[2][BM_CAND];
    __shared__ float acc[BM_CAND * BM_ACC];
    __shared__ BfPair s_pair[TILE_PIX];
    __shared__ float s_ray[TILE_PIX * 6];
    __shared__ __attribute__((aligned(16))) unsigned long long s_hit2[2][BM_SLOTS];
    __shared__ uint16_t s_wbase[4][BM_CAND];
    __shared__ uint16_t s_efirst[4][BM_CAND];
    __shared__ uint32_t s_hb2[2][BM_CAND];
    __shared__ uint32_t s_mark[4][64];
    __shared__ unsigned long long s_mask[TILE_PIX];
    __shared__ uint32_t s_ids2[2][64];
    __shared__ float s_pixc[6][TILE_PIX];
    __shared__ float* s_fl_base[32];
    __shared__ int s_fl_sel[32];

    const uint32_t gx = (d.W + TILE - 1) / TILE, gy = (d.H + TILE - 1) / TILE;
    uint32_t tile;
    if (!tile_of_block(gx * gy * (uint32_t)d.B, is.tile_order, tile)) return;
    const int b = (int)(tile / (gx * gy));
    const uint32_t tyx = tile - (uint32_t)b * gx * gy;
    const int tile_y = (int)(tyx / gx), tile_x = (int)(tyx - (uint32_t)tile_y * gx);
    const int tid = threadIdx.x, lane = tid & 63, wid = tid >> 6;
    STAMP_DECL
    s_mask[tid] = 0;
    const int lx = tid & 15, ly = tid >> 4;
    const int X0 = tile_x * TILE, Y0 = tile_y * TILE;
    const uint32_t px = X0 + lx, py = Y0 + ly;
    const bool inside = (px < (uint32_t)d.W) && (py < (uint32_t)d.H);
    const int64_t pix = ((int64_t)b * d.H + py) * d.W + px;
    const uint32_t pmx = (uint32_t)d.patch_min[2 * b], pmy = (uint32_t)d.patch_min[2 * b + 1];
    const int X0a = X0 + (int)pmx, Y0a = Y0 + (int)pmy;
    const bool corrected = (d.flags & DM2_FLAG_CORRECTED_DV) != 0;

    uint2 range = ranges[tile];
    range.x = __builtin_amdgcn_readfirstlane(range.x); range.y = __builtin_amdgcn_readfirstlane(range.y);
    const int total = (int)min((uint32_t)__builtin_amdgcn_readfirstlane(is.tile_max_lc[tile]), range.y - range.x);
    const uint4* const grecs = is.face_recs + (int64_t)b * d.F * FACE_REC_U4;
    auto walk_entry = [&](int k) -> int64_t { return (int64_t)range.x + (uint32_t)(total - 1 - k); };
    const int rl = lane / REC_CHUNKS, rp = lane - rl * REC_CHUNKS;
    const int rsrc = BfTraits<COV>::src_part(rp);
    auto request_ids = [&](int buf, int nb) {
        if (wid == 2 && nb + lane < total)
            glds4(face_list + walk_entry(nb + lane), &s_ids2[buf][0]);
    };
    if (total > 0) request_ids(0, 0);

    uint32_t last_contributor = 0;
    float T = 0.f;
    {
    float T_final = 0.f, prev_T_final = 0.f;
    float dLc0 = 0.f, dLc1 = 0.f, dLc2 = 0.f, dLd = 0.f, dLa = 0.f;
    if (inside) {
        f3 ro, rd;
        pixel_ray(d, b, pix, px + pmx, py + pmy, d.full_W, d.full_H, ro, rd);
        s_ray[tid * 6] = ro.x; s_ray[tid * 6 + 1] = ro.y; s_ray[tid * 6 + 2] = ro.z;
        s_ray[tid * 6 + 3] = rd.x; s_ray[tid * 6 + 4] = rd.y; s_ray[tid * 6 + 5] = rd.z;
        T_final = is.final_T[pix]; prev_T_final = is.final_prev_T[pix];
        last_contributor = is.n_contrib[pix];
        dLc0 = dL_dcolor[3 * pix]; dLc1 = dL_dcolor[3 * pix + 1]; dLc2 = dL_dcolor[3 * pix + 2];
        dLd = dL_ddepth[pix];
        if constexpr (ALPHA) dLa = dL_dalpha[pix];
    }
    s_pixc[0][tid] = dLc0; s_pixc[1][tid] = dLc1; s_pixc[2][tid] = dLc2; s_pixc[3][tid] = dLd;
    if constexpr (ALPHA) {
        float bg_dot = 0.f;
        bg_dot += d.background[0] * dLc0; bg_dot += d.background[1] * dLc1; bg_dot += d.background[2] * dLc2;
        const float K = (bg_dot + (float)(0.0 + 1.0 * (double)dLd)) - dLa;
        s_pixc[4][tid] = T_final * K; s_pixc[5][tid] = prev_T_final * K;
    } else {
        s_pixc[4][tid] = T_final; s_pixc[5][tid] = prev_T_final;
    }
    T = prev_T_final;
    }
    if (tid < M_N) fill_flush_table(tid, b, d.P, d.F, dL_dverts, dL_dverts_color, dL_dfaces_opacity, dL_dverts_ndc, dL_dfaces_intense,
                                    dL_daa_face_verts, s_fl_base, s_fl_sel, (d.flags & DM2_FLAG_AA_GRAD_TO_VERTS) != 0);

    const float temp = d.aa_temperature;
    const float pix_area = 1.0f;
    const float bg0 = d.background[0], bg1 = d.background[1], bg2 = d.background[2];

    bool T_first_pass = true;
    float accum_rec0 = 0.f, accum_rec1 = 0.f, accum_rec2 = 0.f, accum_recd = 0.f;
    float last_alpha = 0.f, last_c0 = 0.f, last_c1 = 0.f, last_c2 = 0.f, last_depth = 0.f;

    auto request_chunk = [&](int buf, int nb, const uint32_t* ids) {
        const int nc2 = min(BM_CAND, total - nb);
        if (wid == 1 && (lane >> 1) < nc2)
            glds16(hit_masks + walk_entry(nb + (lane >> 1)) * 4 + (lane & 1) * 2, &s_hit2[buf][0]);
        if (COV == POOL && wid == 3 && lane < nc2) glds4(hit_base + walk_entry(nb + lane), &s_hb2[buf][0]);
#pragma unroll
        for (int i = 0; i < 2; i++) {
            const int r0 = (i * 4 + wid) * REC_PER_INSTR;
            const int r = r0 + rl;
            if (rl < REC_PER_INSTR && r < nc2) glds16(grecs + (int64_t)ids[r] * FACE_REC_U4 + rsrc, &recs2[buf][0] + r0);
        }
    };
    if (total > 0) {
        lds_prefetch_wait();
        __syncthreads();
        request_chunk(0, 0, s_ids2[0]);
        lds_prefetch_wait();
    }
    for (int k = tid; k < BM_CAND * BM_ACC; k += TILE_PIX) acc[k] = 0.f;
    __syncthreads();

    STAMP(0)
    int n = 0, cur = 0;
    for (int base = 0; base < total; base += n, cur ^= 1) {
        STAMP(1)
        const int nc = min(BM_CAND, total - base);
        Rec* const recs = recs2[cur];
        const unsigned long long* const s_hit = s_hit2[cur];
        const uint32_t* const s_ids = s_ids2[cur];
        const uint32_t* const s_hb = s_hb2[cur];
        STAMP(2)
        const ulonglong2 hh = reinterpret_cast<const ulonglong2*>(s_hit)[lane];
        const unsigned long long h0 = (2 * lane < nc * 4) ? hh.x : 0ull, h1 = (2 * lane + 1 < nc * 4) ? hh.y : 0ull;
        const int c0 = __popcll(h0), c1 = __popcll(h1);
        const int inc = wave_inclusive_scan(c0 + c1);
        const int b0 = inc - c0 - c1, b1 = inc - c1;
        n = max(1, __popcll(__ballot((lane & 1) && inc <= TILE_PIX && (lane >> 1) < nc)));
        const int S = __builtin_amdgcn_readlane(inc, 2 * n - 1);
        if ((lane & 1) == (wid >> 1) && (lane >> 1) < BM_CAND) s_wbase[wid][lane >> 1] = (uint16_t)((wid & 1) ? b1 : b0);
        if (COV == POOL && (lane & 1) == 0 && (lane >> 1) < BM_CAND) s_efirst[wid][lane >> 1] = (uint16_t)b0;
        const int lo_pair = wid * 64;
        uint32_t* const mark_row = s_mark[wid];
        mark_row[lane] = 0u;
        { const int r0 = b0 - lo_pair, r1 = b1 - lo_pair;
          if (c0 > 0 && (uint32_t)r0 < 64u) mark_row[r0] = ((uint32_t)(2 * lane + 1) << 9) | (uint32_t)b0;
          if (c1 > 0 && (uint32_t)r1 < 64u) mark_row[r1] = ((uint32_t)(2 * lane + 2) << 9) | (uint32_t)b1; }
        uint32_t seed = 0u;
        { const unsigned long long e0 = __ballot(c0 > 0 && b0 <= lo_pair), e1 = __ballot(c1 > 0 && b1 <= lo_pair);
          if (e0) { const int l = 63 - __clzll((long long)e0); seed = ((uint32_t)(2 * l + 1) << 9) | (uint32_t)__builtin_amdgcn_readlane(b0, l); }
          if (e1) { const int l = 63 - __clzll((long long)e1); seed = max(seed, ((uint32_t)(2 * l + 2) << 9) | (uint32_t)__builtin_amdgcn_readlane(b1, l)); } }
        __builtin_amdgcn_fence(__ATOMIC_SEQ_CST, "wavefront");
        const uint32_t mk = max(wave_inclusive_max(mark_row[lane]), seed);
        STAMP(3)

        const bool have = tid < S;
        int j = 0, q = 0;
        float dg[6] = {0.f, 0.f, 0.f, 0.f, 0.f, 0.f};
        float i0 = 0.f, i1 = 0.f, i2 = 0.f, ratio = 0.f, alpha = 0.f;
        int code = 0;
        bool blend = false;
        f3 k_ro = {0, 0, 0}, k_rd = {0, 0, 0}, k_p0 = {0, 0, 0}, k_p1 = {0, 0, 0}, k_p2 = {0, 0, 0};
        float k_col[9] = {0, 0, 0, 0, 0, 0, 0, 0, 0}, k_dep[3] = {0, 0, 0}, k_int = 0.f, k_opa = 0.f;
        if (have) {
            const int lo = (int)(mk >> 9) - 1;
            j = lo >> 2;
            q = ((lo & 3) << 6) + nth_set_bit64(s_hit[lo], tid - (int)(mk & 511u));
            if constexpr (COV == CLIP) {
                const float pxmin = (float)(uint32_t)(X0a + (q & 15)), pymin = (float)(uint32_t)(Y0a + (q >> 4));
                float oarea;
                seg_area_grad(recs[j].aa, pxmin, pxmin + 1, pymin, pymin + 1, pix_area, oarea, dg, recs[j].opacity > 0.9f);
                ratio = fmaxf(oarea, 0.0f) / pix_area;
            } else {
                ratio = COV == POINT ? 1.0f : pool[s_hb[j] + (uint32_t)(tid - (int)s_efirst[wid][j])];
            }
            const Rec& fc = recs[j];
            BfPair out; out.alpha = 0.f; out.c0 = out.c1 = out.c2 = out.depth = 0.f; out.flags = 0;
            const f3 ro = {s_ray[q * 6], s_ray[q * 6 + 1], s_ray[q * 6 + 2]};
            const f3 rd = {s_ray[q * 6 + 3], s_ray[q * 6 + 4], s_ray[q * 6 + 5]};
            const f3 p0 = {fc.v[0], fc.v[1], fc.v[2]}, p1 = {fc.v[3], fc.v[4], fc.v[5]}, p2 = {fc.v[6], fc.v[7], fc.v[8]};
            f3 tuv = {0, 0, 0};
            k_ro = ro; k_rd = rd; k_p0 = p0; k_p1 = p1; k_p2 = p2;
#pragma unroll
            for (int c = 0; c < 9; c++) k_col[c] = fc.col[c];
            k_dep[0] = fc.dep[0]; k_dep[1] = fc.dep[1]; k_dep[2] = fc.dep[2]; k_int = fc.intense; k_opa = fc.opacity;
            if (ray_tri_intersection(ro, rd, p0, p1, p2, tuv)) {
                float iuc, ivc;
                clamp_bary_uv(tuv.y, tuv.z, iuc, ivc, code);
                i0 = 1 - iuc - ivc; i1 = iuc; i2 = ivc;
                if constexpr (COV == CLIP) ratio = mix_coverage(code, ratio, temp);
                float c0 = i0 * fc.col[0] + i1 * fc.col[3] + i2 * fc.col[6];
                float c1 = i0 * fc.col[1] + i1 * fc.col[4] + i2 * fc.col[7];
                float c2 = i0 * fc.col[2] + i1 * fc.col[5] + i2 * fc.col[8];
                out.c0 = c0 * fc.intense; out.c1 = c1 * fc.intense; out.c2 = c2 * fc.intense;
                out.depth = i0 * fc.dep[0] + i1 * fc.dep[1] + i2 * fc.dep[2];
                alpha = fc.opacity * ratio;
                out.alpha = alpha;
                out.flags = MB_BLEND;
                blend = true;
            }
            s_pair[tid] = out;
            if (blend) atomicOr(&s_mask[q], 1ull << j);
        }
        STAMP(5)
        __syncthreads();
        if (base + n < total) {
            request_chunk(cur ^ 1, base + n, s_ids + n);
            request_ids(cur ^ 1, base + n);
        }
        STAMP(6)

        {
            unsigned long long m = s_mask[tid];
            s_mask[tid] = 0;
            float dLc0 = 0.f, dLc1 = 0.f, dLc2 = 0.f, dLd = 0.f, T_final = 0.f, prev_T_final = 0.f;
            if (m) {
                dLc0 = s_pixc[0][tid]; dLc1 = s_pixc[1][tid]; dLc2 = s_pixc[2][tid]; dLd = s_pixc[3][tid];
                T_final = s_pixc[4][tid]; prev_T_final = s_pixc[5][tid];
            }
            while (m) {
                const int jj = __ffsll((long long)m) - 1;
                m &= m - 1;
                const uint32_t e = (uint32_t)(total - 1 - base - jj);
                if (e >= last_contributor) continue;
                const int t = jj * 4 + wid;
                BfPair& pr = s_pair[(int)s_wbase[wid][jj] + __popcll(s_hit[t] & ((1ull << lane) - 1ull))];
                const float a = pr.alpha, iC0 = pr.c0, iC1 = pr.c1, iC2 = pr.c2, iD = pr.depth;
                const bool alpha_is_one = (a == 1.0f) || (T_first_pass && T_final == 0.0f);
                const float inv_1ma = rcp_refined(1.f - a);
                if (!T_first_pass) T = T * inv_1ma;
                T_first_pass = false;
                float dL_dalpha = 0.0f;
                accum_rec0 = last_alpha * last_c0 + (1.f - last_alpha) * accum_rec0; last_c0 = iC0;
                dL_dalpha += (iC0 - accum_rec0) * dLc0;
                accum_rec1 = last_alpha * last_c1 + (1.f - last_alpha) * accum_rec1; last_c1 = iC1;
                dL_dalpha += (iC1 - accum_rec1) * dLc1;
                accum_rec2 = last_alpha * last_c2 + (1.f - last_alpha) * accum_rec2; last_c2 = iC2;
                dL_dalpha += (iC2 - accum_rec2) * dLc2;
                accum_recd = last_alpha * last_depth + (1.f - last_alpha) * accum_recd; last_depth = iD;
                dL_dalpha += (iD - accum_recd) * dLd;
                dL_dalpha *= T;
                last_alpha = a;
                if constexpr (ALPHA) {
                    if (alpha_is_one) dL_dalpha += -prev_T_final;
                    else dL_dalpha += (-T_final) * inv_1ma;
                } else {
                    float bg_dot = 0.f;
                    bg_dot += bg0 * dLc0; bg_dot += bg1 * dLc1; bg_dot += bg2 * dLc2;
                    const float bd_dot = (float)(0.0 + 1.0 * (double)dLd);
                    if (alpha_is_one) {
                        dL_dalpha += (-prev_T_final) * bg_dot;
                        dL_dalpha += (-prev_T_final) * bd_dot;
                    } else {
                        dL_dalpha += (-T_final * inv_1ma) * bg_dot;
                        dL_dalpha += (-T_final * inv_1ma) * bd_dot;
                    }
                }
                pr.depth = T; pr.alpha = dL_dalpha; pr.flags = MB_BLEND | MB_ACTIVE;
            }
        }
        STAMP(7)
        __syncthreads();
        STAMP(8)

        {
            const int jkey = have ? j : -1;
            const int l16 = tid & 15;
            const int k1 = dpp_shr_i<1>(jkey), k2 = dpp_shr_i<2>(jkey), k4 = dpp_shr_i<4>(jkey), k8 = dpp_shr_i<8>(jkey);
            const int kn = dpp_shl_i<1>(jkey);
            const bool s1 = (l16 >= 1) & (k1 == jkey);
            const bool s2 = (l16 >= 2) & (k2 == jkey);
            const bool s4 = (l16 >= 4) & (k4 == jkey);
            const bool s8 = (l16 >= 8) & (k8 == jkey);
            const float m1 = s1 ? 1.f : 0.f, m2 = s2 ? 1.f : 0.f, m4 = s4 ? 1.f : 0.f, m8 = s8 ? 1.f : 0.f;
            uint32_t pflags = 0; float pr_T = 0.f, pr_dL_dalpha = 0.f;
            if (have && blend) { const BfPair& pr = s_pair[tid]; pflags = pr.flags; pr_T = pr.depth; pr_dL_dalpha = pr.alpha; }
            const bool active = (pflags & MB_ACTIVE) != 0;
            float nact = active ? 1.f : 0.f;
            seg_scan16(nact, s1, s2, s4, s8);
            const bool emit = ((l16 == 15) | (kn != jkey)) & (jkey >= 0) & (nact > 0.f);
            float* const arow = acc + j * BM_ACC;
            float dL_diu = 0.f, dL_div = 0.f, dL_doarea = 0.f;
            ISA_MARK(D_group1)
            {
                float g1[14];
#pragma unroll
                for (int c = 0; c < 14; c++) g1[c] = 0.f;
                if (active) {
                    const float Tq = pr_T, dL_dalpha = pr_dL_dalpha;
                    const float qc0 = s_pixc[0][q], qc1 = s_pixc[1][q], qc2 = s_pixc[2][q], qd = s_pixc[3][q];
                    const float intense = k_int, opacity = k_opa;
                    const float* const colD = k_col; const float* const depD = k_dep;
                    const float dics[3] = {qc0 * alpha * Tq, qc1 * alpha * Tq, qc2 * alpha * Tq};
                    const float did = qd * alpha * Tq;
                    g1[12] = dL_dalpha * ratio;
                    const float dL_dratio = (dL_dalpha * opacity) * temp;
                    dL_doarea = dL_dratio / pix_area;
                    float dL_di0 = 0.f, dL_di1 = 0.f, dL_di2 = 0.f, dL_dfint = 0.f;
#pragma unroll
                    for (int ch = 0; ch < 3; ch++) {
                        dL_di0 += colD[ch] * dics[ch] * intense;
                        dL_di1 += colD[3 + ch] * dics[ch] * intense;
                        dL_di2 += colD[6 + ch] * dics[ch] * intense;
                        g1[ch] = 0.f + i0 * dics[ch] * intense;
                        g1[3 + ch] = 0.f + i1 * dics[ch] * intense;
                        g1[6 + ch] = 0.f + i2 * dics[ch] * intense;
                        dL_dfint += (i0 * colD[ch] + i1 * colD[3 + ch] + i2 * colD[6 + ch]) * dics[ch];
                    }
                    g1[13] = dL_dfint;
                    dL_di0 += depD[0] * did; dL_di1 += depD[1] * did; dL_di2 += depD[2] * did;
                    g1[9] = 0.f + i0 * did; g1[10] = 0.f + i1 * did; g1[11] = 0.f + i2 * did;
                    float diuc_diu, diuc_div, divc_diu, divc_div;
                    clamp_bary_uv_grad(code, diuc_diu, diuc_div, divc_diu, divc_div);
                    const float di0_diu = -1.f * diuc_diu + -1.f * divc_diu, di0_div = -1.f * diuc_div + -1.f * divc_div;
                    const float di1_diu = 1.f * diuc_diu + 0.f * divc_diu, di1_div = 1.f * diuc_div + 0.f * divc_div;
                    const float di2_diu = 0.f * diuc_diu + 1.f * divc_diu, di2_div = 0.f * diuc_div + 1.f * divc_div;
                    dL_diu = dL_di0 * di0_diu + dL_di1 * di1_diu + dL_di2 * di2_diu;
                    dL_div = dL_di0 * di0_div + dL_di1 * di1_div + dL_di2 * di2_div;
                }
                seg_scan16_safe(g1, m1, m2, m4, m8, s1, s2, s4, s8);
                if (emit) {
#pragma unroll
                    for (int c = 0; c < 12; c++) atomicAdd(arow + M_DC + c, g1[c]);
                    atomicAdd(arow + M_OP, g1[12]);
                    atomicAdd(arow + M_IN, g1[13]);
                    arow[M_FLAG] = 1.0f;
                }
            }
            ISA_MARK(D_group2)
            bool tie_push = false;
            uint32_t tie_base = 0;
            unsigned long long tie_bal = 0;
            if constexpr (COV == CLIP) {
                float g2[6];
#pragma unroll
                for (int c = 0; c < 6; c++) g2[c] = dL_doarea * dg[c];
                seg_scan16_safe(g2, m1, m2, m4, m8, s1, s2, s4, s8);
                if (emit) {
#pragma unroll
                    for (int c = 0; c < 6; c++) atomicAdd(arow + M_AA + c, g2[c]);
                }
            } else if constexpr (COV == POOL) {
                float g2[6];
                bool tie = false;
                {
                    const FaceRecB& fb = recs[j];
                    const AAFaceB fa = {fb.v2, fb.e, fb.r, rec_zmask(fb)};
                    const float pxmin = (float)(uint32_t)(X0a + (q & 15)), pymin = (float)(uint32_t)(Y0a + (q >> 4));
                    fast_area_grad(fa, pxmin, pxmin + 1, pymin, pymin + 1, g2, tie);
                }
                tie_push = tie && active && (dL_doarea != 0.0f);
                const bool use = active && !tie;
#pragma unroll
                for (int c = 0; c < 6; c++) g2[c] = use ? dL_doarea * g2[c] : 0.0f;
                tie_bal = __ballot(tie_push);
                if (tie_bal && lane == (int)(__ffsll((long long)tie_bal) - 1)) tie_base = atomicAdd(hit_valid + 2, (uint32_t)__popcll(tie_bal));
                seg_scan16_safe(g2, m1, m2, m4, m8, s1, s2, s4, s8);
                if (emit) {
#pragma unroll
                    for (int c = 0; c < 6; c++) atomicAdd(arow + M_AA + c, g2[c]);
                }
            }
            ISA_MARK(D_group3)
            {
                float g3[9];
#pragma unroll
                for (int c = 0; c < 9; c++) g3[c] = 0.f;
                if (active) {
                    const f3 ro = k_ro, rd = k_rd, p0 = k_p0, p1 = k_p1, p2 = k_p2;
                    f3 du0, du1, du2, dv0, dv1, dv2;
                    ray_tri_intersection_grad<true>(ro, rd, p0, p1, p2, corrected, du0, du1, du2, dv0, dv1, dv2);
                    const f3 dp0 = dL_diu * du0 + dL_div * dv0;
                    const f3 dp1 = dL_diu * du1 + dL_div * dv1;
                    const f3 dp2 = dL_diu * du2 + dL_div * dv2;
                    g3[0] = dp0.x; g3[1] = dp0.y; g3[2] = dp0.z;
                    g3[3] = dp1.x; g3[4] = dp1.y; g3[5] = dp1.z;
                    g3[6] = dp2.x; g3[7] = dp2.y; g3[8] = dp2.z;
                }
                seg_scan16_safe(g3, m1, m2, m4, m8, s1, s2, s4, s8);
                if (emit) {
#pragma unroll
                    for (int c = 0; c < 9; c++) atomicAdd(arow + M_DV + c, g3[c]);
                }
            }
            if (tie_bal) {
                const uint32_t tb = (uint32_t)__shfl((int)tie_base, __ffsll((long long)tie_bal) - 1);
                const uint32_t at = tb + __builtin_amdgcn_mbcnt_hi((uint32_t)(tie_bal >> 32), __builtin_amdgcn_mbcnt_lo((uint32_t)tie_bal, 0u));
                if (tie_push && at < tie_cap)
                    tie_queue[at] = tie_pack((uint32_t)recs[j].face_id, (uint32_t)b, (uint32_t)(X0 + (q & 15)), (uint32_t)(Y0 + (q >> 4)), dL_doarea);
            }
        }
        STAMP(9)
        lds_prefetch_wait();
        __syncthreads();
        STAMP(10)

        const int comp = tid & 31;
        if (comp < (COV == POINT ? M_AA : M_N)) {
            float* const basep = s_fl_base[comp];
            const int entry = s_fl_sel[comp];
            const bool corner = (entry & 0x80) != 0;
            int sel0, mult;
            flush_id_and_mult(entry, 0u, sel0, mult);
            for (int e = tid >> 5; e < n; e += TILE_PIX / 32) {
                float* a = acc + e * BM_ACC;
                const float flag = a[M_FLAG];
                const float val = a[comp];
                int sel = sel0;
                if (corner) { int m_; flush_id_and_mult(entry, rec_zmask(recs[e]), sel, m_); }
                const int id = (&recs[e].face_id)[sel];
                if (flag != 0.f) {
                    a[comp] = 0.f;
                    if (comp == 0) a[M_FLAG] = 0.f;
                    atomicAdd(basep + (int64_t)id * mult, val);
                }
            }
        }
        STAMP(11)
    }
    STAMP_FLUSH
}

__global__ void __launch_bounds__(256)
k_aa_ties(dm2_render_desc d, const uint4* __restrict__ face_recs, const TieEntry* __restrict__ queue, uint32_t cap,
          uint32_t* __restrict__ counters, float* __restrict__ dL_daa_face_verts, bool check_mode) {
    if (check_mode && counters[0] != 3u) return;
    const uint32_t n = min(counters[2], cap);
    const uint32_t working = min(gridDim.x, (n + blockDim.x - 1u) / blockDim.x);
    if (blockIdx.x >= working) return;
    const bool to_verts = (d.flags & DM2_FLAG_AA_GRAD_TO_VERTS) != 0;
    const uint32_t lane = threadIdx.x & 63u;
    for (uint32_t i0 = (blockIdx.x * blockDim.x + threadIdx.x) - lane; i0 < n; i0 += gridDim.x * blockDim.x) {
        const uint32_t i = i0 + lane;
        const bool valid = i < n;
        TieEntry e = tie_pack(0u, 0u, 0u, 0u, 0.0f);
        if (valid) e = queue[i];
        uint32_t b, x, y;
        tie_unpack(e, b, x, y);
        const int64_t bf = (int64_t)b * d.F + e.face;
        const uint4* src = face_recs + bf * FACE_REC_U4;
        AAFace f;
        float g[6] = {0.f, 0.f, 0.f, 0.f, 0.f, 0.f};
        if (valid) {
            uint4* dst = reinterpret_cast<uint4*>(&f);
#pragma unroll
            for (int k = 0; k < 8; k++) dst[k] = src[k];
            const float pxmin = (float)(x + (uint32_t)d.patch_min[2 * b]), pymin = (float)(y + (uint32_t)d.patch_min[2 * b + 1]);
            float area;
            (void)tri_pix_overlap_area<true>(f, pxmin, pxmin + 1, pymin, pymin + 1, 1.0f, area, g);
#pragma unroll
            for (int c = 0; c < 6; c++) g[c] *= e.dL_doarea;
        }
        const int key = valid ? (int)e.face : -1 - (int)lane, kv = (int)b, l16 = (int)(lane & 15u);
        const int cont = (int)(l16 >= 1) & (int)(dpp_shr_i<1>(key) == key) & (int)(dpp_shr_i<1>(kv) == kv);
        const int c2 = cont & dpp_shr_i<1>(cont), c4 = c2 & dpp_shr_i<2>(c2), c8 = c4 & dpp_shr_i<4>(c4);
        const bool s1 = cont != 0, s2 = (c2 != 0) & (l16 >= 2), s4 = (c4 != 0) & (l16 >= 4), s8 = (c8 != 0) & (l16 >= 8);
        const bool last = (l16 == 15) | (dpp_shl_i<1>(cont) == 0);
#pragma unroll
        for (int c = 0; c < 6; c++) seg_scan16(g[c], s1, s2, s4, s8);
        const bool emit = valid & last;
        if (!emit) continue;
        if (to_verts) {
            const uint4 ids = src[14];
            const int vid[3] = {(int)ids.x, (int)ids.y, (int)ids.z};
            const uint32_t zm = src[4].z;
            const bool flip = (zm >> 8) & 1u;
#pragma unroll
            for (int c = 0; c < 3; c++) {
                const int v = vid[c == 0 ? 0 : (flip ? 3 - c : c)];
                float* dstp = dL_daa_face_verts + ((int64_t)b * d.P + v) * 2;
                atomicAdd(dstp, g[2 * c]); atomicAdd(dstp + 1, g[2 * c + 1]);
            }
        } else {
            float* dstp = dL_daa_face_verts + bf * 6;
#pragma unroll
            for (int c = 0; c < 6; c++) atomicAdd(dstp + c, g[c]);
        }
    }
    __shared__ uint32_t s_ticket;
    __syncthreads();
    if (threadIdx.x == 0) s_ticket = atomicAdd(counters + 3, 1u);
    __syncthreads();
    if (s_ticket == working - 1 && threadIdx.x == 0) { counters[2] = 0u; counters[3] = 0u; }
}

void launch_render_backward_fast(const dm2_render_desc& d, const uint2* ranges, const uint32_t* face_list, ImageState is,
                                 const float* dL_dcolor, const float* dL_ddepth, float* dL_dverts, float* dL_dverts_color,
                                 float* dL_dfaces_opacity, float* dL_dverts_ndc, float* dL_dfaces_intense,
                                 float* dL_daa_face_verts, const BinningState& bs, bool clip, TieEntry* tie_queue, int64_t tie_cap,
                                 bool check_mode, const float* dL_dalpha, hipStream_t st) {
    const uint32_t Tn = (uint32_t)(((d.W + TILE - 1) / TILE) * ((d.H + TILE - 1) / TILE) * d.B);
    const uint32_t cap = (uint32_t)(tie_cap > 0xFFFFFFF0ll ? 0xFFFFFFF0ll : tie_cap);
    auto launch = [&](auto kernel, uint32_t kcap) {
        StageTimer tm(check_mode ? -1 : ST_BWD, st);
        hipLaunchKernelGGL(kernel, dim3(tile_grid_blocks(Tn)), dim3(TILE_PIX), 0, st, d, ranges, face_list, is, dL_dcolor, dL_ddepth,
                           dL_dverts, dL_dverts_color, dL_dfaces_opacity, dL_dverts_ndc, dL_dfaces_intense, dL_daa_face_verts,
                           bs.hit_masks, bs.hit_valid, bs.hit_base, bs.pool, tie_queue, kcap, check_mode, dL_dalpha STAMP_ARG(1));
    };
    const bool A = dL_dalpha != nullptr;
    if (!(d.aa_temperature > 0.0f)) {
        launch(A ? k_render_backward_fast<POINT, true> : k_render_backward_fast<POINT, false>, 0u); return;
    }
    if (clip) { launch(A ? k_render_backward_fast<CLIP, true> : k_render_backward_fast<CLIP, false>, 0u); return; }
    launch(A ? k_render_backward_fast<POOL, true> : k_render_backward_fast<POOL, false>, cap);
    const unsigned blocks = (unsigned)((cap + 255u) / 256u < 1024u ? (cap + 255u) / 256u : 1024u);
    StageTimer tm(check_mode ? -1 : ST_TIES, st);
    if (blocks) hipLaunchKernelGGL(k_aa_ties, dim3(blocks), dim3(256), 0, st, d, is.face_recs, tie_queue, cap, bs.hit_valid, dL_daa_face_verts, check_mode);
}

}
```

dmesh2_renderer_amd/csrc/dm2_debug.hip:

```cpp
#include <hip/hip_runtime.h>

#include "dm2_clip_area.h"
#include "dm2_clip_fast.h"
#include "dm2_clip_seg.h"
#include "dm2_device_math.h"
#include "dm2_state.h"

namespace dm2 {

__global__ void __launch_bounds__(64)
k_debug_aa_overlap(int variant, int64_t n, const float* __restrict__ tv, const float* __restrict__ te,
                   const uint8_t* __restrict__ tz, const float* __restrict__ tr, const float* __restrict__ tn,
                   const float* __restrict__ tc, const float* __restrict__ pixmin, float* __restrict__ area,
                   float* __restrict__ grad, int32_t* __restrict__ code) {
    const int64_t i = (int64_t)blockIdx.x * blockDim.x + threadIdx.x;
    if (i >= n) return;
    AAFace f;
    uint32_t zm = 0;
#pragma unroll
    for (int k = 0; k < 6; k++) {
        f.v[k] = tv[6 * i + k]; f.e[k] = te[6 * i + k]; f.r[k] = tr[6 * i + k]; f.n[k] = tn[6 * i + k];
        zm |= (tz[6 * i + k] ? 1u : 0u) << k;
    }
#pragma unroll
    for (int k = 0; k < 3; k++) f.c[k] = tc[3 * i + k];
    f.zmask = zm;
    f.bb[0] = fminf(fminf(f.v[0], f.v[2]), f.v[4]); f.bb[1] = fmaxf(fmaxf(f.v[0], f.v[2]), f.v[4]);
    f.bb[2] = fminf(fminf(f.v[1], f.v[3]), f.v[5]); f.bb[3] = fmaxf(fmaxf(f.v[1], f.v[3]), f.v[5]);
    const float pxmin = pixmin[2 * i], pymin = pixmin[2 * i + 1], pxmax = pxmin + 1, pymax = pymin + 1;
    float a = 0.f, g[6] = {0.f, 0.f, 0.f, 0.f, 0.f, 0.f};
    int err = 0;
    if (variant == 0) {
        err = tri_pix_overlap_area<true>(f, pxmin, pxmax, pymin, pymax, 1.0f, a, g);
    } else if (variant == 1) {
        err = tri_pix_overlap_area_only(f, pxmin, pxmax, pymin, pymax, 1.0f, a);
    } else if (variant == 4) {
        err = tri_pix_overlap_area_only(f, pxmin, pxmax, pymin, pymax, 1.0f, a);
        if (err == 0 && a != 0.0f) {
            bool tie;
            fast_area_grad(f, pxmin, pxmax, pymin, pymax, g, tie);
            if (tie) { err = -1; for (int k = 0; k < 6; k++) g[k] = 0.f; }
        }
    } else {
        float af = 0.f;
        err = tri_pix_overlap_area_only(f, pxmin, pxmax, pymin, pymax, 1.0f, af);
        if (err == 0 && af != 0.0f) seg_area_grad(f, pxmin, pxmax, pymin, pymax, 1.0f, a, g, variant == 3);
    }
    if (err > 0) { a = 0.f; for (int k = 0; k < 6; k++) g[k] = 0.f; }
    area[i] = a; code[i] = err;
    for (int k = 0; k < 6; k++) grad[6 * i + k] = g[k];
}

void launch_debug_aa_overlap(int variant, int64_t n, const float* tv, const float* te, const uint8_t* tz, const float* tr,
                             const float* tn, const float* tc, const float* pixmin, float* area, float* grad, int32_t* code,
                             hipStream_t st) {
    if (n <= 0) return;
    hipLaunchKernelGGL(k_debug_aa_overlap, dim3((unsigned)((n + 63) / 64)), dim3(64), 0, st, variant, n, tv, te, tz, tr, tn, tc,
                       pixmin, area, grad, code);
}

}
```

dmesh2_renderer_amd/csrc/dm2_device_math.h:

```cpp
#pragma once
#include <hip/hip_runtime.h>
#include <stdint.h>

namespace dm2 {

constexpr int TILE = 16;
constexpr int TILE_PIX = TILE * TILE;
constexpr float T_EPS = 0.0001f;
constexpr int MAX_POLY = 10;

struct f3 { float x, y, z; };
__device__ __forceinline__ f3 operator-(f3 a, f3 b) { return {a.x - b.x, a.y - b.y, a.z - b.z}; }
__device__ __forceinline__ f3 operator+(f3 a, f3 b) { return {a.x + b.x, a.y + b.y, a.z + b.z}; }
__device__ __forceinline__ f3 operator-(f3 a) { return {-a.x, -a.y, -a.z}; }
__device__ __forceinline__ f3 operator*(f3 a, float b) { return {a.x * b, a.y * b, a.z * b}; }
__device__ __forceinline__ f3 operator*(float b, f3 a) { return {b * a.x, b * a.y, b * a.z}; }
__device__ __forceinline__ f3 operator/(f3 a, float b) { return {a.x / b, a.y / b, a.z / b}; }
__device__ __forceinline__ float dot(f3 a, f3 b) { return a.x * b.x + a.y * b.y + a.z * b.z; }
__device__ __forceinline__ f3 cross(f3 a, f3 b) {
    return {a.y * b.z - a.z * b.y, a.z * b.x - a.x * b.z, a.x * b.y - a.y * b.x};
}

__device__ __forceinline__ void analytic_ray(const float* __restrict__ cam, float x_abs, float y_abs, float Wf, float Hf, f3& ro, f3& rd) {
    const float* imv = cam;
    const float* ipr = cam + 16;
    const float h[4] = {((x_abs + 0.5f) / Wf * 2.0f) - 1.0f, ((y_abs + 0.5f) / Hf * 2.0f) - 1.0f, -1.0f, 1.0f};
    float v[4], w[3];
#pragma unroll
    for (int j = 0; j < 4; j++) v[j] = ((h[0] * ipr[4 * j] + h[1] * ipr[4 * j + 1]) + h[2] * ipr[4 * j + 2]) + h[3] * ipr[4 * j + 3];
#pragma unroll
    for (int j = 0; j < 3; j++) w[j] = ((v[0] * imv[4 * j] + v[1] * imv[4 * j + 1]) + v[2] * imv[4 * j + 2]) + v[3] * imv[4 * j + 3];
    ro = {imv[3], imv[7], imv[11]};
    const f3 dd = {w[0] - ro.x, w[1] - ro.y, w[2] - ro.z};
    const float len = sqrtf((dd.x * dd.x + dd.y * dd.y) + dd.z * dd.z) + 1e-6f;
    rd = {dd.x / len, dd.y / len, dd.z / len};
}

__device__ __forceinline__ bool ray_tri_intersection(f3 ro, f3 rd, f3 p0, f3 p1, f3 p2, f3& tuv) {
    f3 T = ro - p0, E1 = p1 - p0, E2 = p2 - p0;
    f3 P = cross(rd, E2), Q = cross(T, E1);
    float denom = dot(P, E1);
    if (denom == 0.0f) return false;
    float inv_denom = 1.0f / denom;
    tuv.x = dot(Q, E2) * inv_denom;
    tuv.y = dot(P, T) * inv_denom;
    tuv.z = dot(Q, rd) * inv_denom;
    return true;
}

__device__ __forceinline__ float rcp_refined(float x) {
    const float r = __builtin_amdgcn_rcpf(x);
    return __builtin_fmaf(__builtin_fmaf(-x, r, 1.0f), r, r);
}

template <bool FAST_RCP = false>
__device__ __forceinline__ void ray_tri_intersection_grad(f3 ro, f3 rd, f3 p0, f3 p1, f3 p2, bool corrected,
                                                          f3& du_dp0, f3& du_dp1, f3& du_dp2,
                                                          f3& dv_dp0, f3& dv_dp1, f3& dv_dp2) {
    f3 T = ro - p0, E1 = p1 - p0, E2 = p2 - p0;
    f3 dxE2 = cross(rd, E2);
    float denom_sqrt = dot(dxE2, E1);
    float denom = denom_sqrt * denom_sqrt;
    float denom_inv = FAST_RCP ? rcp_refined(denom) : 1.0f / denom;
    float v0 = dot(dxE2, T);
    float v1 = denom_sqrt;
    f3 E1xd = cross(E1, rd);
    f3 du_dE1 = ((-1.0f * dxE2) * v0) * denom_inv;
    f3 du_dE2 = (cross(T, rd) * v1 - v0 * E1xd) * denom_inv;
    f3 du_dT = (dxE2 * v1) * denom_inv;
    f3 dv_dE1, dv_dE2, dv_dT;
    if (!corrected) {
        float v2 = dot(cross(T, E1), E2);
        dv_dE1 = ((cross(E2, T) * v1) - (v2 * dxE2)) * denom_inv;
        dv_dE2 = ((cross(T, E1) * v1) - (v2 * E1xd)) * denom_inv;
        dv_dT = (cross(E1, E2) * v1) * denom_inv;
    } else {
        float N = dot(cross(T, E1), rd);
        dv_dE1 = ((cross(rd, T) * v1) - (N * dxE2)) * denom_inv;
        dv_dE2 = ((-N) * E1xd) * denom_inv;
        dv_dT = (E1xd * v1) * denom_inv;
    }
    du_dp0 = -du_dE1 - du_dE2 - du_dT;
    dv_dp0 = -dv_dE1 - dv_dE2 - dv_dT;
    du_dp1 = du_dE1; dv_dp1 = dv_dE1;
    du_dp2 = du_dE2; dv_dp2 = dv_dE2;
}

__device__ __forceinline__ void clamp_bary_uv(float u, float v, float& u_c, float& v_c, int& code) {
    if (u >= 0.0f && v >= 0.0f && u + v <= 1.0f) { u_c = u; v_c = v; code = 0; }
    else if (u <= 0.0f && v <= 0.0f) { u_c = 0.0f; v_c = 0.0f; code = 1; }
    else if ((u >= 1.0f && v <= 0.0f) || (v >= 0.0f && v <= u - 1.0f)) { u_c = 1.0f; v_c = 0.0f; code = 2; }
    else if ((u <= 0.0f && v >= 1.0f) || (u >= 0.0f && v >= u + 1.0f)) { u_c = 0.0f; v_c = 1.0f; code = 3; }
    else if (u <= 0.0f && v <= 1.0f && v >= 0.0f) { u_c = 0.0f; v_c = v; code = 4; }
    else if (u <= 1.0f && u >= 0.0f && v <= 0.0f) { u_c = u; v_c = 0.0f; code = 5; }
    else { u_c = (1.0f + u - v) * 0.5f; v_c = (1.0f - u + v) * 0.5f; code = 6; }
}

__device__ __forceinline__ void clamp_bary_uv_grad(int code, float& duc_du, float& duc_dv, float& dvc_du, float& dvc_dv) {
    dvc_du = 0.0f; duc_dv = 0.0f;
    if (code == 0) { duc_du = 1.0f; dvc_dv = 1.0f; }
    else if (code == 1 || code == 2 || code == 3) { duc_du = 0.0f; dvc_dv = 0.0f; }
    else if (code == 4) { duc_du = 0.0f; dvc_dv = 1.0f; }
    else if (code == 5) { duc_du = 1.0f; dvc_dv = 0.0f; }
    else { duc_du = 0.5f; dvc_du = -0.5f; duc_dv = -0.5f; dvc_dv = 0.5f; }
}

__device__ __forceinline__ float mix_coverage(int code, float ratio, float temp) {
    if (code == 0) return (float)(1.0 * (double)(1.0f - temp) + (double)(ratio * temp));
    return (float)(0.0 * (double)(1.0f - temp) + (double)(ratio * temp));
}

__device__ __forceinline__ int f2i_sat(float x) {
    if (x != x) return 0;
    if (x >= 2147483648.0f) return 2147483647;
    if (x <= -2147483648.0f) return (-2147483647 - 1);
    return (int)x;
}

__device__ __forceinline__ void patch_rect_from_tri(uint32_t pmx, uint32_t pmy, float p0x, float p0y, float p1x, float p1y,
                                                    float p2x, float p2y, uint32_t gx, uint32_t gy,
                                                    uint32_t& x0, uint32_t& y0, uint32_t& x1, uint32_t& y1) {
    float min_x = fminf(fminf(p0x, p1x), p2x) - (float)pmx;
    float min_y = fminf(fminf(p0y, p1y), p2y) - (float)pmy;
    float max_x = fmaxf(fmaxf(p0x, p1x), p2x) - (float)pmx;
    float max_y = fmaxf(fmaxf(p0y, p1y), p2y) - (float)pmy;
    int ix0 = f2i_sat(floorf(min_x / TILE)), iy0 = f2i_sat(floorf(min_y / TILE));
    int ix1 = f2i_sat(ceilf(max_x / TILE)), iy1 = f2i_sat(ceilf(max_y / TILE));
    x0 = min(gx, (uint32_t)max(0, ix0)); y0 = min(gy, (uint32_t)max(0, iy0));
    x1 = min(gx, (uint32_t)max(0, ix1)); y1 = min(gy, (uint32_t)max(0, iy1));
}

struct AAFace {
    float v[6];
    float e[6];
    float r[6];
    uint32_t zmask;
    float c[3];
    float n[6];
    float bb[4];
};
static_assert(sizeof(AAFace) == 128, "AAFace: 32 dwords");

struct PolyVert {
    float x, y;
    int idx;
    float g0[4], g1[4];
};

template <bool GRAD>
struct PolyAcc {
    PolyVert first, prev;
    int cnt;
    float area;
    float g[6];
    bool err;
};

__device__ __forceinline__ float one_minus_t_plus(float t, float prod) {
    return (float)((1.0 - (double)t) + (double)prod);
}

__device__ __forceinline__ void grad_rows_add(float* g, int row, float a0, float a1) {
    float s0 = g[0] + a0, s1 = g[1] + a1, s2 = g[2] + a0, s3 = g[3] + a1, s4 = g[4] + a0, s5 = g[5] + a1;
    g[0] = row == 0 ? s0 : g[0]; g[1] = row == 0 ? s1 : g[1];
    g[2] = row == 1 ? s2 : g[2]; g[3] = row == 1 ? s3 : g[3];
    g[4] = row == 2 ? s4 : g[4]; g[5] = row == 2 ? s5 : g[5];
}

__device__ __forceinline__ void update_grad(float* g, const PolyVert& v, float gax, float gay) {
    float a0 = v.g0[0] * gax + v.g0[1] * gay;
    float a1 = v.g0[2] * gax + v.g0[3] * gay;
    float b0 = v.g1[0] * gax + v.g1[1] * gay;
    float b1 = v.g1[2] * gax + v.g1[3] * gay;
    int i0 = v.idx;
    int i1 = (i0 == 2) ? 0 : i0 + 1;
    grad_rows_add(g, i0, a0, a1);
    grad_rows_add(g, i1, b0, b1);
}

template <bool GRAD>
__device__ __forceinline__ void poly_emit(PolyAcc<GRAD>& A, const PolyVert& v) {
    if (A.cnt >= MAX_POLY) { A.err = true; return; }
    if (A.cnt == 0) A.first = v;
    else if (A.cnt >= 2) {
        const PolyVert& ip0 = A.first; const PolyVert& ip1 = A.prev; const PolyVert& ip2 = v;
        float cr = (ip1.x - ip0.x) * (ip2.y - ip0.y) - (ip2.x - ip0.x) * (ip1.y - ip0.y);
        float s_area = (float)(0.5 * (double)cr);
        if (s_area < 0) A.err = true;
        A.area += s_area;
        if (GRAD) {
            update_grad(A.g, ip0, 0.5f * (ip1.y - ip2.y), 0.5f * (-ip1.x + ip2.x));
            update_grad(A.g, ip1, 0.5f * (ip2.y - ip0.y), 0.5f * (-ip2.x + ip0.x));
            update_grad(A.g, ip2, 0.5f * (ip0.y - ip1.y), 0.5f * (-ip0.x + ip1.x));
        }
    }
    if (A.cnt >= 1) A.prev = v;
    A.cnt++;
}

template <int TI, bool GRAD>
__device__ __forceinline__ void clip_tri_edge(const AAFace& f, float pxmin, float pxmax, float pymin, float pymax,
                                              uint32_t inside_mask, PolyAcc<GRAD>& A) {
    constexpr int TJ = (TI + 1) % 3;
    const float p0x = f.v[2 * TI], p0y = f.v[2 * TI + 1];
    const float p1x = f.v[2 * TJ], p1y = f.v[2 * TJ + 1];
    const float ex = f.e[2 * TI], ey = f.e[2 * TI + 1];
    const float rx = f.r[2 * TI], ry = f.r[2 * TI + 1];
    const bool e_vertical = (f.zmask >> (2 * TI)) & 1u;
    const bool e_horizontal = (f.zmask >> (2 * TI + 1)) & 1u;
    const bool p0in = (p0x >= pxmin) && (p0x <= pxmax) && (p0y >= pymin) && (p0y <= pymax);
    const bool p1in = (p1x >= pxmin) && (p1x <= pxmax) && (p1y >= pymin) && (p1y <= pymax);

    PolyVert s0, s1;
    float t0 = 0.f, t1 = 0.f;
    int pe0 = -1, pe1 = -1, n = 0;
    s0.x = s0.y = s1.x = s1.y = 0.f; s0.idx = s1.idx = TI;
#pragma unroll
    for (int k = 0; k < 4; k++) { s0.g0[k] = s0.g1[k] = s1.g0[k] = s1.g1[k] = 0.f; }

#pragma unroll
    for (int pi = 0; pi < 4; pi++) {
        const bool horiz = (pi == 0) || (pi == 2);
        const float iaxis0 = pi == 0 ? pymin : (pi == 1 ? pxmax : (pi == 2 ? pymax : pxmin));
        const bool parallel = horiz ? e_horizontal : e_vertical;
        const float pmin1 = horiz ? pxmin : pymin, pmax1 = horiz ? pxmax : pymax;
        const float p0a0 = horiz ? p0y : p0x, p0a1 = horiz ? p0x : p0y;
        const float p1a0 = horiz ? p1y : p1x;
        const float ra0 = horiz ? ry : rx;
        const float ea1 = horiz ? ex : ey;
        const float t = (iaxis0 - p0a0) * ra0;
        const float iaxis1 = p0a1 + t * ea1;
        const bool valid = (t >= 0) && (t <= 1) && (iaxis1 >= pmin1) && (iaxis1 <= pmax1) && (!parallel);
        if (valid) {
            if ((iaxis1 == pmin1) || (iaxis1 == pmax1)) A.err = true;
            PolyVert nv;
            nv.x = horiz ? iaxis1 : iaxis0;
            nv.y = horiz ? iaxis0 : iaxis1;
            nv.idx = TI;
// ... 109 lines not shown
```

dmesh2_renderer_amd/csrc/dm2_forward_queue.hip:

```cpp
#include <hip/hip_runtime.h>

#include "dm2_clip_area.h"
#include "dm2_device_math.h"
#include "dm2_pairs.h"
#include "dm2_stage.h"
#include "dm2_stamps.h"
#include "dm2_state.h"

namespace dm2 {

#ifndef DM2_FQ_CHUNK
#define DM2_FQ_CHUNK 52
#endif
#ifndef DM2_FQ_BLOCKS
#define DM2_FQ_BLOCKS 4
#endif
#ifndef DM2_FQ_PAIRCAP
#define DM2_FQ_PAIRCAP 768
#endif
#ifndef DM2_FQ_SURVCAP
#define DM2_FQ_SURVCAP 512
#endif
constexpr int FQ_CHUNK = DM2_FQ_CHUNK;
constexpr int FQ_PAIRCAP = DM2_FQ_PAIRCAP;
// ... 57 lines not shown
    const int lx = tid & 15, ly = tid >> 4;
    const int X0 = tile_x * TILE, Y0 = tile_y * TILE;
    const uint32_t px = X0 + lx, py = Y0 + ly;
    const bool inside = (px < (uint32_t)d.W) && (py < (uint32_t)d.H);
    const int64_t pix = ((int64_t)b * d.H + py) * d.W + px;
    const uint32_t pmx = (uint32_t)d.patch_min[2 * b], pmy = (uint32_t)d.patch_min[2 * b + 1];
    const int X0a = X0 + (int)pmx, Y0a = Y0 + (int)pmy;
    const int xlim = min(TILE - 1, d.W - 1 - X0), ylim = min(TILE - 1, d.H - 1 - Y0);

    if (inside) {
        f3 ro, rd;
        pixel_ray(d, b, pix, px + pmx, py + pmy, d.full_W, d.full_H, ro, rd);
        s_ray[tid * 6] = ro.x; s_ray[tid * 6 + 1] = ro.y; s_ray[tid * 6 + 2] = ro.z;
        s_ray[tid * 6 + 3] = rd.x; s_ray[tid * 6 + 4] = rd.y; s_ray[tid * 6 + 5] = rd.z;
    }
    const uint2 range = ranges[tile];
    const int total = (int)(range.y - range.x);
    const uint4* const grecs = is.face_recs + (int64_t)b * d.F * FACE_REC_U4;
    const int rl = lane / FQ_REC_CHUNKS, rp = lane - rl * FQ_REC_CHUNKS;
    auto request_ids = [&](int nb) {
        if (wid == 2 && nb + lane < total) glds4(face_list + range.x + nb + lane, &s_ids[0]);
    };
    auto request_recs = [&](int nb) {
        const int nc2 = min(FQ_CHUNK, total - nb);
        for (int r0 = 4 * wid; r0 < nc2; r0 += 16) {
            const int r = r0 + rl;
            if (rl < 4 && r < nc2) glds16(grecs + (int64_t)s_ids[r] * FACE_REC_U4 + rp, &recs[r0]);
        }
    };
    if (total > 0) {
        request_ids(0);
        lds_prefetch_wait();
        __syncthreads();
        request_recs(0);
    }
    const float temp = d.aa_temperature;
    const bool use_aa = temp > 0.0f;
    const float pix_area = 1.0f;
    const int K = d.K;

    bool done = !inside;
    float pT = 1.0f, T = 1.0f;
    uint32_t last_contributor = 0;
    float C0 = 0.f, C1 = 0.f, C2 = 0.f, D = 0.f;
    int rec_cnt = 0;
    auto flush_weights = [&](int wb, int wn) {
        if (tid < wn) {
            const float w = s_w[tid];
            if (w != 0.0f) { atomicAdd(face_weights + (int64_t)b * d.F + face_list[range.x + wb + tid], w); s_w[tid] = 0.f; }
        }
    };

    STAMP(0)
    int n = 0;
    for (int base = 0; base < total; base += n) {
        lds_prefetch_wait();
        if constexpr (WEIGHTS) {
            const int ndone = __syncthreads_count(done);
            flush_weights(base - n, n);
            if (ndone == TILE_PIX) break;
        } else if (__syncthreads_count(done) == TILE_PIX) {
            break;
        }
        STAMP(1)
        n = min(FQ_CHUNK, total - base);
        const bool last_chunk = base + n >= total;
        int cnt = 0;
        if (tid < n) {
            uint32_t rect;
            cnt = face_pixel_rect(recs[tid].aa.bb, use_aa, X0a, Y0a, xlim, ylim, rect);
            s_rect[tid] = rect;
        }
        if (tid < FQ_CHUNK * 4) s_bmask[tid] = 0;
        if (tid < FQ_SURVCAP / 64) s_blend[tid] = 0;
        STAMP(2)
        if (wid == 0) {
            const int inc = wave_inclusive_scan(cnt);
            if (tid < n) {
                const int ex = inc - cnt;
                s_off[tid] = ex;
                const uint32_t r = s_rect[tid];
                s_kb[tid] = ex - (int)((r >> 4) & 15u) * ((int)((r >> 8) & 15u) + 1) - (int)(r & 15u);
            }
            if (lane == 63) s_off[n] = inc;
        }
        __syncthreads();
        int tot = s_off[n];
        if (tot > FQ_PAIRCAP) {
            n = find_face(s_off, n, FQ_PAIRCAP);
            tot = s_off[n];
        }
        STAMP(3)

        const int Q = (((tot + 3) >> 2) + 63) & ~63;
        int wcount = 0, wfull = 0;
        for (int r = 0; r < Q; r += 64) {
            const int k = wid * Q + r + lane;
            bool surv = false, full = false;
            uint32_t entry = 0;
            if (k < tot) {
                const int j = find_face(s_off, n, k);
                int qx, qy;
                pair_xy(s_rect[j], k - s_off[j], s_inv, qx, qy);
                uint32_t cmask = 0xF;
                surv = true;
                if (use_aa) {
                    const float pxmin = (float)(uint32_t)(X0a + qx), pymin = (float)(uint32_t)(Y0a + qy);
                    surv = classify_pixel(recs[j].aa, pxmin, pxmin + 1, pymin, pymin + 1, cmask);
                }
                full = surv && (cmask == 0xFu);
                entry = (uint32_t)(qy * TILE + qx) | ((uint32_t)j << 8) | (cmask << 14);
            }
            const unsigned long long bal = __ballot(surv);
            const int before = wcount + (int)__builtin_amdgcn_mbcnt_hi((uint32_t)(bal >> 32), __builtin_amdgcn_mbcnt_lo((uint32_t)bal, 0u));
            if (k < tot) s_slot[k] = (uint16_t)before;
            if (CLASSES) {
                const unsigned long long balf = __ballot(full), balc = bal & ~balf;
                const int rf = wfull + (int)__builtin_amdgcn_mbcnt_hi((uint32_t)(balf >> 32), __builtin_amdgcn_mbcnt_lo((uint32_t)balf, 0u));
                const int rc = (wcount - wfull) + (int)__builtin_amdgcn_mbcnt_hi((uint32_t)(balc >> 32), __builtin_amdgcn_mbcnt_lo((uint32_t)balc, 0u));
                if (surv) s_queue[wid * FQ_QCAP + (full ? FQ_QCAP - 1 - rf : rc)] = entry | ((uint32_t)before << 18);
                wfull += __popcll(balf);
            } else if (surv) s_queue[wid * FQ_QCAP + before] = entry;
            wcount += __popcll(bal);
        }
        if (lane == 0) { s_wtot[wid] = wcount; if (CLASSES) s_wtotc[wid] = wcount - wfull; }
        __syncthreads();
        STAMP(4)
        const int wb1 = s_wtot[0], wb2 = wb1 + s_wtot[1], wb3 = wb2 + s_wtot[2];
        int S = wb3 + s_wtot[3];
        const int ST0 = S;
        int wc1 = 0, wc2 = 0, wc3 = 0, SC = 0;
        if (CLASSES) { wc1 = s_wtotc[0]; wc2 = wc1 + s_wtotc[1]; wc3 = wc2 + s_wtotc[2]; SC = wc3 + s_wtotc[3]; }
        const int wf1 = wb1 - wc1, wf2 = wb2 - wc2, wf3 = wb3 - wc3;
        auto surv_before = [&](int k) -> int {
            if (k >= tot) return S;
            const int w = (k >= Q) + (k >= 2 * Q) + (k >= 3 * Q);
            return (w == 0 ? 0 : (w == 1 ? wb1 : (w == 2 ? wb2 : wb3))) + (int)s_slot[k];
        };
        int target = S;
        if (S > FQ_SURVCAP) target = FQ_SURVCAP;
        else if (FQ_TAILMIN > 0 && !last_chunk && S > TILE_PIX && (S & (TILE_PIX - 1)) != 0 && (S & (TILE_PIX - 1)) < FQ_TAILMIN) target = S & ~(TILE_PIX - 1);
        if (target < S) {
            int lo = 1, hi = n;
            while (hi - lo > 1) {
                const int mid = (lo + hi) >> 1;
                if (surv_before(s_off[mid]) <= target) lo = mid; else hi = mid;
            }
            const int S2 = surv_before(s_off[lo]);
            n = lo; tot = s_off[lo]; S = S2;
        }

        if (base + n < total) request_ids(base + n);
        uint32_t cbase = 0;
        if (pool && tid == 0) cbase = atomicAdd(hit_valid + 1, (uint32_t)S);
        constexpr int FQ_ROUNDS = CLASSES ? (FQ_PAIRCAP + TILE_PIX - 1) / TILE_PIX : FQ_SURVCAP / TILE_PIX;
        const int ST = CLASSES ? ST0 : S;
        float pool_ratio[FQ_ROUNDS];
        int pool_s[FQ_ROUNDS];
#pragma unroll
        for (int rnd = 0; rnd < FQ_ROUNDS; rnd++) { pool_ratio[rnd] = 0.f; pool_s[rnd] = -1; }
        if (!CLASSES && pool && lane == 0) s_rcnt[4 + wid] = 0;
#pragma unroll
        for (int rnd = 0; rnd < FQ_ROUNDS; rnd++) {
            if (rnd * TILE_PIX >= ST) break;
            const int t = tid + rnd * TILE_PIX;
            uint32_t entry = 0u;
            int s = t;
            if (CLASSES) {
                const bool isc = t < SC;
                const int tc = isc ? t : t - SC;
                const int b1 = isc ? wc1 : wf1, b2 = isc ? wc2 : wf2, b3 = isc ? wc3 : wf3;
                const int w = (tc >= b1) + (tc >= b2) + (tc >= b3);
                const int within = tc - (w == 0 ? 0 : (w == 1 ? b1 : (w == 2 ? b2 : b3)));
                if (t < ST) entry = s_queue[w * FQ_QCAP + (isc ? within : FQ_QCAP - 1 - within)];
                s = (w == 0 ? 0 : (w == 1 ? wb1 : (w == 2 ? wb2 : wb3))) + (int)((entry >> 18) & 255u);
            } else if (t < ST) {
                const int w = (s >= wb1) + (s >= wb2) + (s >= wb3);
                entry = s_queue[w * FQ_QCAP + (s - (w == 0 ? 0 : (w == 1 ? wb1 : (w == 2 ? wb2 : wb3))))];
            }
            bool blend_s = false;
            if (t < ST && s < S) {
            const int q = (int)(entry & 255u), j = (int)((entry >> 8) & 63u);
            const uint32_t cmask = (entry >> 14) & 15u;
            const FaceRec& fc = recs[j];
            const float pxmin = (float)(uint32_t)(X0a + (q & 15)), pxmax = pxmin + 1;
            const float pymin = (float)(uint32_t)(Y0a + (q >> 4)), pymax = pymin + 1;
            FqPair out; out.alpha = 0.f; out.c0 = out.c1 = out.c2 = out.depth = 0.f; out.flags = 0;
            float oarea = 0.f;
            bool live = true;
            if (use_aa) {
                const int err = clip_area_classified(fc.aa, pxmin, pxmax, pymin, pymax, cmask, pix_area, oarea);
                live = !((err != 0) || (oarea == 0.0f));
                if (live) out.flags |= QF_REC;
            }
            if (live) {
                float ratio = oarea / pix_area;
                const f3 ro = {s_ray[q * 6], s_ray[q * 6 + 1], s_ray[q * 6 + 2]};
                const f3 rd = {s_ray[q * 6 + 3], s_ray[q * 6 + 4], s_ray[q * 6 + 5]};
                const f3 p0 = {fc.v[0], fc.v[1], fc.v[2]}, p1 = {fc.v[3], fc.v[4], fc.v[5]}, p2 = {fc.v[6], fc.v[7], fc.v[8]};
                f3 tuv = {0, 0, 0};
                if (ray_tri_intersection(ro, rd, p0, p1, p2, tuv)) {
                    float iuc, ivc; int code;
                    clamp_bary_uv(tuv.y, tuv.z, iuc, ivc, code);
                    const float i0 = 1 - iuc - ivc, i1 = iuc, i2 = ivc;
                    ratio = mix_coverage(code, ratio, temp);
                    if (ratio != 0.0f) {
                        float c0 = i0 * fc.col[0] + i1 * fc.col[3] + i2 * fc.col[6];
                        float c1 = i0 * fc.col[1] + i1 * fc.col[4] + i2 * fc.col[7];
                        float c2 = i0 * fc.col[2] + i1 * fc.col[5] + i2 * fc.col[8];
                        out.c0 = c0 * fc.intense; out.c1 = c1 * fc.intense; out.c2 = c2 * fc.intense;
                        out.depth = i0 * fc.dep[0] + i1 * fc.dep[1] + i2 * fc.dep[2];
                        out.alpha = fc.opacity * ratio;
                        out.flags |= QF_BLEND;
                        pool_ratio[rnd] = ratio; blend_s = true;
                        if (CLASSES) { pool_s[rnd] = s; if (pool) atomicOr(&s_blend[s >> 6], 1ull << (s & 63)); }
                    }
                }
            }
            if (out.flags) {
                s_pair[s] = out;
                atomicOr(&s_mask[q], 1ull << j);
                if (hit_masks && (out.flags & QF_BLEND)) atomicOr(&s_bmask[j * 4 + (q >> 6)], 1ull << (q & 63));
            }
            }
            if (!CLASSES && pool) {
                const unsigned long long bal = __ballot(blend_s);
                pool_s[rnd] = blend_s ? (int)__builtin_amdgcn_mbcnt_hi((uint32_t)(bal >> 32), __builtin_amdgcn_mbcnt_lo((uint32_t)bal, 0u)) : -1;
                if (lane == 0) s_rcnt[rnd * 4 + wid] = __popcll(bal);
            }
        }
        STAMP(5)
        if (pool && tid == 0) s_cbase = cbase;
        lds_prefetch_wait();
        __syncthreads();
        if (base + n < total) request_recs(base + n);
        if (hit_masks && tid < n * 4) hit_masks[((int64_t)range.x + base + (tid >> 2)) * 4 + (tid & 3)] = s_bmask[tid];
        if (pool) {
            const uint32_t cb = s_cbase;
            if (wid == 0) {
                int cj = 0;
                if (lane < n) {
                    const ulonglong2 m01 = reinterpret_cast<const ulonglong2*>(s_bmask)[2 * lane], m23 = reinterpret_cast<const ulonglong2*>(s_bmask)[2 * lane + 1];
                    cj = __popcll(m01.x) + __popcll(m01.y) + __popcll(m23.x) + __popcll(m23.y);
                }
                const int ex = wave_inclusive_scan(cj) - cj;
                if (lane < n) hit_base[(int64_t)range.x + base + lane] = cb + (uint32_t)ex;
            }
            if (!CLASSES) {
                const uint4 c03 = reinterpret_cast<const uint4*>(s_rcnt)[0], c47 = reinterpret_cast<const uint4*>(s_rcnt)[1];
                const uint32_t r0 = (wid > 0 ? c03.x : 0u) + (wid > 1 ? c03.y : 0u) + (wid > 2 ? c03.z : 0u);
                const uint32_t r1 = c03.x + c03.y + c03.z + c03.w + (wid > 0 ? c47.x : 0u) + (wid > 1 ? c47.y : 0u) + (wid > 2 ? c47.z : 0u);
                if (pool_s[0] >= 0) { const uint32_t slot = cb + r0 + (uint32_t)pool_s[0]; if (slot < pool_cap) pool[slot] = pool_ratio[0]; }
                if (FQ_ROUNDS > 1 && pool_s[FQ_ROUNDS > 1 ? 1 : 0] >= 0) { const uint32_t slot = cb + r1 + (uint32_t)pool_s[1]; if (slot < pool_cap) pool[slot] = pool_ratio[1]; }
            } else {
            {
                const int c = lane < FQ_SURVCAP / 64 ? __popcll(s_blend[lane < FQ_SURVCAP / 64 ? lane : 0]) : 0;
                const int ex = wave_inclusive_scan(c) - c;
                if (lane < FQ_SURVCAP / 64) s_bpre[wid][lane] = ex;
                __builtin_amdgcn_fence(__ATOMIC_SEQ_CST, "wavefront");
            }
#pragma unroll
            for (int rnd = 0; rnd < FQ_ROUNDS; rnd++) {
                const int s = pool_s[rnd];
                if (s >= 0) {
                    const uint32_t slot = cb + (uint32_t)(s_bpre[wid][s >> 6] + __popcll(s_blend[s >> 6] & ((1ull << (s & 63)) - 1ull)));
                    if (slot < pool_cap) pool[slot] = pool_ratio[rnd];
                }
            }
            }
        }

        {
            unsigned long long m = s_mask[tid];
            s_mask[tid] = 0;
            while (m && !done) {
                const int j = __ffsll((long long)m) - 1;
                m &= m - 1;
                const int k = s_kb[j] + ly * ((int)((s_rect[j] >> 8) & 15u) + 1) + lx;
                const FqPair pr = s_pair[surv_before(k)];
                if ((pr.flags & QF_REC) && rec_cnt < K) rec_cnt++;
                if (!(pr.flags & QF_BLEND)) continue;
                const float alpha = pr.alpha;
                const float test_T = T * (1 - alpha);
                if constexpr (WEIGHTS) atomicAdd(&s_w[j], alpha * T);
                C0 += pr.c0 * alpha * T; C1 += pr.c1 * alpha * T; C2 += pr.c2 * alpha * T;
                D += pr.depth * alpha * T;
                pT = T; T = test_T;
                last_contributor = (uint32_t)(base + j + 1);
                if (T < T_EPS) done = true;
            }
        }
        STAMP(6)
    }

    if (tid == 0) s_maxlc = 0;
    __syncthreads();
    if constexpr (WEIGHTS) flush_weights(total - n, n);
    { const uint32_t m = wave_inclusive_max(last_contributor); if (lane == 63 && m) atomicMax(&s_maxlc, m); }
    __syncthreads();
    if (tid == 0) is.tile_max_lc[tile] = s_maxlc;
    if (inside) {
        is.final_prev_T[pix] = pT;
        is.final_T[pix] = T;
        is.n_contrib[pix] = last_contributor;
        out_color[3 * pix] = C0 + T * d.background[0];
        out_color[3 * pix + 1] = C1 + T * d.background[1];
        out_color[3 * pix + 2] = C2 + T * d.background[2];
        out_depth[pix] = D + T * 1.0f;
        if (out_tri_cnt) out_tri_cnt[pix] = rec_cnt;
    }
    STAMP(7)
    STAMP_FLUSH
}

void launch_render_forward_queue(const dm2_render_desc& d, const uint2* ranges, const uint32_t* face_list, ImageState is,
                                 float* out_color, float* out_depth, int32_t* out_tri_cnt, uint64_t* hit_masks,
                                 uint32_t* hit_valid, float* pool, int64_t pool_cap, uint32_t* hit_base, bool classes,
                                 float* face_weights, hipStream_t st) {
    const uint32_t Tn = (uint32_t)(((d.W + TILE - 1) / TILE) * ((d.H + TILE - 1) / TILE) * d.B);
    StageTimer tm(ST_FWD, st);
#define DM2_FQ_LAUNCH(C, W)                                                                                                 \
    hipLaunchKernelGGL((k_render_forward_queue<C, W>), dim3(tile_grid_blocks(Tn)), dim3(TILE_PIX), 0, st, d, ranges, face_list, \
                       is, out_color, out_depth, out_tri_cnt, hit_masks, hit_valid, pool, (uint32_t)pool_cap, hit_base,      \
                       face_weights STAMP_ARG(0))
    if (classes) {
        if (face_weights) DM2_FQ_LAUNCH(true, true); else DM2_FQ_LAUNCH(true, false);
    } else {
        if (face_weights) DM2_FQ_LAUNCH(false, true); else DM2_FQ_LAUNCH(false, false);
    }
#undef DM2_FQ_LAUNCH
}

}
```

dmesh2_renderer_amd/csrc/dm2_state.h:

```cpp
#pragma once
#include <hip/hip_runtime.h>
#include <stddef.h>
#include <stdint.h>

#include "../../include/dm2_hip.h"

namespace dm2 {

constexpr size_t ALIGN = 256;

struct Carver {
    uintptr_t p;
    explicit Carver(const void* base) : p(reinterpret_cast<uintptr_t>(base)) {}
    template <class T> T* take(size_t count) {
        p = (p + ALIGN - 1) & ~(uintptr_t)(ALIGN - 1);
        T* r = reinterpret_cast<T*>(p);
        p += count * sizeof(T);
        return r;
    }
    size_t used(const void* base) const { return (size_t)(p - reinterpret_cast<uintptr_t>(base)); }
};

constexpr int FACE_REC_U4 = 16;

constexpr int PAIR_PARTS = 1024;

struct FaceState {
    float* depths;
    float* min_depths;
    float* max_depths;
    uint32_t* tiles_touched;
    uint32_t* face_offsets;
    uint32_t* rect_lo;
    uint32_t* rect_hi;
    void* scan_temp; size_t scan_temp_bytes;
    uint4* recs;
    uint32_t* tile_cnt;
    uint32_t* tile_cnt_big;
    uint32_t* tile_start;
    uint32_t* plan_meta;
    unsigned long long* pair_part;
    uint4* tile_rank;
    static FaceState carve(void* base, int64_t BF, int64_t Tn, size_t scan_temp_bytes, bool with_recs, size_t* total = nullptr) {
        Carver c(base); FaceState s;
        s.depths = c.take<float>(BF); s.min_depths = c.take<float>(BF); s.max_depths = c.take<float>(BF);
        s.tiles_touched = c.take<uint32_t>(BF); s.face_offsets = c.take<uint32_t>(BF);
        s.rect_lo = c.take<uint32_t>(BF); s.rect_hi = c.take<uint32_t>(BF);
        s.scan_temp = c.take<char>(scan_temp_bytes); s.scan_temp_bytes = scan_temp_bytes;
        s.recs = with_recs ? c.take<uint4>(BF * FACE_REC_U4) : nullptr;
        s.tile_cnt = c.take<uint32_t>(2 * Tn + 2 * PAIR_PARTS); s.tile_cnt_big = s.tile_cnt + Tn;
        s.pair_part = reinterpret_cast<unsigned long long*>(s.tile_cnt + 2 * Tn);
        s.tile_start = c.take<uint32_t>(Tn); s.plan_meta = c.take<uint32_t>(4);
        s.tile_rank = c.take<uint4>(Tn > 0 ? BF : 0);
        if (total) *total = c.used(base) + ALIGN;
        return s;
    }
};

struct ImageState {
    float* final_T;
    float* final_prev_T;
    uint32_t* n_contrib;
    uint2* ranges;
    uint32_t* tile_max_lc;
    uint32_t* tile_order;
    const uint4* face_recs;
    static ImageState carve(void* base, int64_t N, int64_t Tn, size_t* total = nullptr) {
        Carver c(base); ImageState s; s.face_recs = nullptr;
        s.final_T = c.take<float>(N); s.final_prev_T = c.take<float>(N); s.n_contrib = c.take<uint32_t>(N);
        s.ranges = c.take<uint2>(Tn); s.tile_max_lc = c.take<uint32_t>(Tn);
        s.tile_order = c.take<uint32_t>(8 * ((Tn + 7) / 8));
        if (total) *total = c.used(base) + ALIGN;
        return s;
    }
};

struct LayerImageState {
    uint2* ranges;
    int32_t* first_face;
    int32_t* first_tet;
    static LayerImageState carve(void* base, int64_t N, int64_t Tn, size_t* total = nullptr) {
        Carver c(base); LayerImageState s;
        s.ranges = c.take<uint2>(Tn); s.first_face = c.take<int32_t>(N); s.first_tet = c.take<int32_t>(N);
        if (total) *total = c.used(base) + ALIGN;
        return s;
    }
};

struct BinningState {
    uint32_t* face_list;
    uint64_t* keys;
    uint64_t* keys_unsorted;
    uint32_t* face_list_unsorted;
    void* sort_temp; size_t sort_temp_bytes;
    uint64_t* hit_masks;
    uint32_t* hit_base;
    uint32_t* hit_valid;
    float* pool; int64_t pool_cap;
    static BinningState carve(void* base, int64_t R, size_t sort_temp_bytes, size_t* total = nullptr, size_t buffer_bytes = 0) {
        Carver c(base); BinningState s;
        s.face_list = c.take<uint32_t>(R); s.keys = c.take<uint64_t>(R);
        s.keys_unsorted = c.take<uint64_t>(R); s.face_list_unsorted = c.take<uint32_t>(R);
        s.sort_temp = c.take<char>(sort_temp_bytes); s.sort_temp_bytes = sort_temp_bytes;
        s.hit_masks = c.take<uint64_t>(4 * R); s.hit_base = c.take<uint32_t>(R); s.hit_valid = c.take<uint32_t>(4);
        const size_t fixed = c.used(base) + ALIGN;
        if (total) *total = fixed;
        s.pool = c.take<float>(0);
        const size_t off = c.used(base);
        s.pool_cap = buffer_bytes > off ? (int64_t)((buffer_bytes - off) / sizeof(float)) : 0;
        if (s.pool_cap > 0xFFFFFFF0ll) s.pool_cap = 0xFFFFFFF0ll;
        return s;
    }
    static size_t pool_bytes(int64_t pairs) { return pairs > 0 ? (((size_t)pairs * sizeof(float) + ALIGN - 1) & ~(ALIGN - 1)) + ALIGN : 0; }
};

struct __attribute__((aligned(16))) TieEntry { uint32_t face, view_hi, pxy; float dL_doarea; };
__host__ __device__ inline TieEntry tie_pack(uint32_t face, uint32_t view, uint32_t x, uint32_t y, float g) {
    TieEntry e; e.face = face; e.view_hi = view | ((x >> 16) << 16) | ((y >> 16) << 24); e.pxy = (x & 0xFFFFu) | (y << 16); e.dL_doarea = g;
    return e;
}
__host__ __device__ inline void tie_unpack(const TieEntry& e, uint32_t& view, uint32_t& x, uint32_t& y) {
    view = e.view_hi & 0xFFFFu; x = (e.pxy & 0xFFFFu) | (((e.view_hi >> 16) & 0xFFu) << 16); y = (e.pxy >> 16) | ((e.view_hi >> 24) << 16);
}

size_t scan_temp_bytes(int64_t BF);
size_t sort_temp_bytes(int64_t R, int64_t Tn);
unsigned sort_end_bit(int64_t Tn);

hipError_t launch_preprocess_scan(int B, int P, int F, int W, int H, const int32_t* patch_min, const int32_t* faces,
                                  const float* verts_ndc, const float* verts_image, FaceState fs, const dm2_render_desc* pack,
                                  uint32_t* host_meta, uint32_t host_seq, uint2* ranges_to_clear, uint32_t* tile_order, hipStream_t st);
constexpr int64_t TILE_SORT_MAX = 32768;
hipError_t launch_bin_sort(int B, int F, int W, int H, int64_t R, int64_t max_tile_entries, bool legacy, const float* key_depth,
                           FaceState fs, BinningState bs, uint2* ranges, bool ranges_cleared, uint32_t* tile_order, hipStream_t st);

void launch_tile_order_identity(int64_t Tn, uint32_t* tile_order, hipStream_t st);

void launch_render_forward_point(const dm2_render_desc& d, const uint2* ranges, const uint32_t* face_list, ImageState is,
                                 float* out_color, float* out_depth, int32_t* out_tri_cnt, uint64_t* hit_masks,
                                 uint32_t* hit_valid, float* face_weights, hipStream_t st);
int launch_render_forward(const dm2_render_desc& d, const uint2* ranges, const uint32_t* face_list, ImageState is,
                          float* out_color, float* out_depth, int32_t* out_tri_cnt, const BinningState& bs, bool use_pool,
                          float pairs_per_entry, float* face_weights, hipStream_t st);
void launch_prepare_faces(const dm2_prep_desc& d, hipStream_t st);
void launch_prepare_faces_backward(const dm2_prep_desc& d, const float* g_ndc, const float* g_image, const float* g_aa,
                                   float* image_grad_scratch, float* g_verts, float* g_mv, float* g_proj, double* camera_scratch,
                                   hipStream_t st);
size_t prepare_camera_scratch_bytes(int B, int P);
void launch_render_forward_queue(const dm2_render_desc& d, const uint2* ranges, const uint32_t* face_list, ImageState is,
                                 float* out_color, float* out_depth, int32_t* out_tri_cnt, uint64_t* hit_masks,
                                 uint32_t* hit_valid, float* pool, int64_t pool_cap, uint32_t* hit_base, bool classes,
                                 float* face_weights, hipStream_t st);
void launch_render_backward_fast(const dm2_render_desc& d, const uint2* ranges, const uint32_t* face_list, ImageState is,
                                 const float* dL_dcolor, const float* dL_ddepth, float* dL_dverts, float* dL_dverts_color,
                                 float* dL_dfaces_opacity, float* dL_dverts_ndc, float* dL_dfaces_intense,
                                 float* dL_daa_face_verts, const BinningState& bs, bool clip, TieEntry* tie_queue,
                                 int64_t tie_cap, bool check_mode, const float* dL_dalpha, hipStream_t st);
void launch_render_backward(const dm2_render_desc& d, const uint2* ranges, const uint32_t* face_list, ImageState is,
                            const float* dL_dcolor, const float* dL_ddepth, float* dL_dverts, float* dL_dverts_color,
                            float* dL_dfaces_opacity, float* dL_dverts_ndc, float* dL_dfaces_intense,
                            float* dL_daa_face_verts, const BinningState& bs, int fwd_mode, TieEntry* tie_queue, int64_t tie_cap,
                            const float* dL_dalpha, hipStream_t st);
void launch_debug_aa_overlap(int variant, int64_t n, const float* tv, const float* te, const uint8_t* tz, const float* tr,
                             const float* tn, const float* tc, const float* pixmin, float* area, float* grad, int32_t* code,
                             hipStream_t st);
hipError_t launch_exchange_mark(int B, int P, int F, int N, const int32_t* faces, const uint32_t* tiles_touched, uint8_t* flags,
                                uint32_t* counts, hipStream_t st);
hipError_t launch_exchange_pack(int B, int P, int F, int N, const uint8_t* flags, const uint32_t* counts, uint32_t* cursors,
                                const float* dverts, const float* dcolor, const float* dopacity, const float* dintense, float* send,
                                hipStream_t st);
hipError_t launch_exchange_unpack(int B, int P, int F, int N, int rank, const float* recv, const uint32_t* recv_counts_host, int64_t rows,
                                  float* slice_v, float* slice_f, hipStream_t st);
int exchange_max_ranks();
size_t tet_scratch_bytes(int64_t T);
void launch_layer_composite(const dm2_layer_composite_desc& d, float* out_color, float* out_depth, float* out_final_T,
                            int32_t* out_n_contrib, float* out_face_weights, hipStream_t st);
void launch_layer_composite_backward(const dm2_layer_composite_desc& d, const float* dL_dcolor, const float* dL_ddepth,
                                     const int32_t* n_contrib, float* dL_dverts_color, float* dL_dfaces_opacity,
                                     float* dL_dverts_ndc, float* dL_dfaces_intense, const float* dL_dalpha, hipStream_t st);
void launch_forward_alpha(ImageState is, int64_t N, float* out_alpha, hipStream_t st);
void launch_layers(const dm2_layers_desc& d, const FaceState& fs, const uint2* ranges, const uint32_t* face_list,
                   LayerImageState ls, void* tet_scratch, int32_t* render_layers, int32_t* render_layers_cnt, hipStream_t st);
void launch_rasterize(const dm2_layers_desc& d, const FaceState& fs, const uint2* ranges, const uint32_t* face_list,
                      int32_t* render_layers, int32_t* render_layers_cnt, float* bary, float* t, hipStream_t st);
void launch_rasterize_backward(const dm2_layers_desc& d, const int32_t* render_layers, const float* dL_dbary, const float* dL_dt,
                               float* dL_dverts, hipStream_t st);
void launch_interpolate(int B, int H, int W, int L, int F, int N, int C, int view_tables, const int32_t* render_layers,
                        const float* bary, const float* attr, const int32_t* attr_faces, float* out, hipStream_t st);
void launch_interpolate_backward(int B, int H, int W, int L, int F, int N, int C, int view_tables, const int32_t* render_layers,
                                 const float* bary, const float* attr, const int32_t* attr_faces, const float* dL_dout,
                                 float* dL_dattr, float* dL_dbary, hipStream_t st);
void launch_texture(int B, int H, int W, int L, int Ht, int Wt, int C, int view_textures, int filter, int boundary,
                    const int32_t* render_layers, const float* uv, const float* tex, float* out, hipStream_t st);
void launch_texture_backward(int B, int H, int W, int L, int Ht, int Wt, int C, int view_textures, int filter, int boundary,
                             const int32_t* render_layers, const float* uv, const float* tex, const float* dL_dout,
                             float* dL_dtex, float* dL_duv, hipStream_t st);

}

namespace dm2 {
enum Stage { ST_PREP = 0, ST_EMIT = 1, ST_SORT = 2, ST_RANGES = 3, ST_FWD = 4, ST_BWD = 5, ST_TIES = 6 };
void prof_begin(int stage, hipStream_t st);
void prof_end(int stage, hipStream_t st);
struct StageTimer {
    int s; hipStream_t st;
    StageTimer(int stage, hipStream_t stream) : s(stage), st(stream) { if (s >= 0) prof_begin(s, st); }
    ~StageTimer() { if (s >= 0) prof_end(s, st); }
};
}
```

include/dm2_hip.h:

```cpp
#ifndef DM2_HIP_H
#define DM2_HIP_H

#include <stddef.h>
#include <stdint.h>

#ifdef __cplusplus
extern "C" {
#endif

#define DM2_ABI_VERSION 6
#define DM2_TILE 16

typedef struct dm2_render_desc {
    int32_t B, P, F;
    int32_t W, H;
    int32_t K;
    float aa_temperature;
    int32_t flags;
    int32_t full_W, full_H;
    const float* background;
    const int32_t* patch_min;
    const float* verts;
    const int32_t* faces;
    const float* verts_color;
// ... 67 lines not shown
                        int64_t* num_rendered, int64_t* max_tile_entries, int64_t* pair_bound, int32_t* forward_mode);
int dm2_forward_run_weights(const dm2_render_desc* d, int64_t num_rendered, int64_t max_tile_entries, int64_t pair_bound,
                            void* face_scratch, size_t face_bytes,
                            void* binning_scratch, size_t binning_bytes,
                            void* image_scratch, size_t image_bytes,
                            float* out_color, float* out_depth, int32_t* out_tri_cnt, float* out_face_weights, void* stream,
                            int32_t* forward_mode);

int dm2_backward(const dm2_render_desc* d, int64_t num_rendered, int32_t forward_mode,
                 const float* dL_dout_color, const float* dL_dout_depth,
                 const void* face_scratch, size_t face_bytes,
                 void* binning_scratch, size_t binning_bytes,
                 const void* image_scratch, size_t image_bytes,
                 void* tie_scratch, size_t tie_bytes,
                 float* dL_dverts, float* dL_dverts_color, float* dL_dfaces_opacity,
                 float* dL_dverts_ndc, float* dL_dfaces_intense, float* dL_daa_face_verts,
                 void* stream);

int dm2_forward_alpha(const dm2_render_desc* d, const void* image_scratch, size_t image_bytes, float* out_alpha, void* stream);

int dm2_backward_alpha(const dm2_render_desc* d, int64_t num_rendered, int32_t forward_mode,
                       const float* dL_dout_color, const float* dL_dout_depth, const float* dL_dout_alpha,
                       const void* face_scratch, size_t face_bytes,
                       void* binning_scratch, size_t binning_bytes,
                       const void* image_scratch, size_t image_bytes,
                       void* tie_scratch, size_t tie_bytes,
                       float* dL_dverts, float* dL_dverts_color, float* dL_dfaces_opacity,
                       float* dL_dverts_ndc, float* dL_dfaces_intense, float* dL_daa_face_verts,
                       void* stream);

typedef struct dm2_layers_desc {
    int32_t B, P, F, T;
    int32_t W, H, L;
    int32_t flags;
    const float* verts;
    const int32_t* faces;
    const int32_t* tets;
    const int32_t* face_tets;
    const int32_t* tet_faces;
    const int32_t* face_existence;
    const float* verts_ndc;
    const float* verts_image;
    const float* image_ray_o;
    const float* image_ray_d;
    const float* ray_cam;
} dm2_layers_desc;

int dm2_layers_plan(const dm2_layers_desc* d, void* face_scratch, size_t face_bytes,
                    void* stream, int64_t* num_rendered, int64_t* max_tile_entries);
int dm2_layers_run(const dm2_layers_desc* d, int64_t num_rendered, int64_t max_tile_entries,
                   void* face_scratch, size_t face_bytes,
                   void* binning_scratch, size_t binning_bytes,
                   void* image_scratch, size_t image_bytes,
                   void* tet_scratch, size_t tet_bytes,
                   int32_t* render_layers, int32_t* render_layers_cnt, void* stream);

int dm2_rasterize_run(const dm2_layers_desc* d, int64_t num_rendered, int64_t max_tile_entries,
                      void* face_scratch, size_t face_bytes,
                      void* binning_scratch, size_t binning_bytes,
                      void* image_scratch, size_t image_bytes,
                      int32_t* render_layers, int32_t* render_layers_cnt, float* bary, float* t, void* stream);
int dm2_rasterize_backward(const dm2_layers_desc* d, const int32_t* render_layers, const float* dL_dbary, const float* dL_dt,
                           float* dL_dverts, void* stream);

int dm2_interpolate(int32_t B, int32_t H, int32_t W, int32_t L, int32_t F, int32_t N, int32_t C, int32_t view_tables,
                    const int32_t* render_layers, const float* bary, const float* attr, const int32_t* attr_faces,
                    float* out, void* stream);
int dm2_interpolate_backward(int32_t B, int32_t H, int32_t W, int32_t L, int32_t F, int32_t N, int32_t C, int32_t view_tables,
                             const int32_t* render_layers, const float* bary, const float* attr, const int32_t* attr_faces,
                             const float* dL_dout, float* dL_dattr, float* dL_dbary, void* stream);

#define DM2_TEX_FILTER_NEAREST 0
#define DM2_TEX_FILTER_LINEAR 1
#define DM2_TEX_BOUNDARY_WRAP 0
#define DM2_TEX_BOUNDARY_CLAMP 1
int dm2_texture(int32_t B, int32_t H, int32_t W, int32_t L, int32_t Ht, int32_t Wt, int32_t C, int32_t view_textures,
                int32_t filter, int32_t boundary, const int32_t* render_layers, const float* uv, const float* tex, float* out,
                void* stream);
int dm2_texture_backward(int32_t B, int32_t H, int32_t W, int32_t L, int32_t Ht, int32_t Wt, int32_t C, int32_t view_textures,
                         int32_t filter, int32_t boundary, const int32_t* render_layers, const float* uv, const float* tex,
                         const float* dL_dout, float* dL_dtex, float* dL_duv, void* stream);

typedef struct dm2_layer_composite_desc {
    int32_t B, P, F;
    int32_t W, H, L;
    int32_t flags;
    const int32_t* render_layers;
    const float* verts;
    const int32_t* faces;
    const float* verts_color;
    const float* faces_opacity;
    const float* faces_intense;
    const float* verts_ndc;
    const float* background;
    const float* image_ray_o;
    const float* image_ray_d;
    const float* ray_cam;
} dm2_layer_composite_desc;

int dm2_layers_composite(const dm2_layer_composite_desc* d, float* out_color, float* out_depth, float* out_final_T,
                         int32_t* out_n_contrib, void* stream);
int dm2_layers_composite_weights(const dm2_layer_composite_desc* d, float* out_color, float* out_depth, float* out_final_T,
                                 int32_t* out_n_contrib, float* out_face_weights, void* stream);
int dm2_layers_composite_backward(const dm2_layer_composite_desc* d, const float* dL_dout_color, const float* dL_dout_depth,
                                  const int32_t* n_contrib, float* dL_dverts_color, float* dL_dfaces_opacity,
                                  float* dL_dverts_ndc, float* dL_dfaces_intense, void* stream);
int dm2_layers_composite_backward_alpha(const dm2_layer_composite_desc* d, const float* dL_dout_color,
                                        const float* dL_dout_depth, const float* dL_dout_alpha,
                                        const int32_t* n_contrib, float* dL_dverts_color, float* dL_dfaces_opacity,
                                        float* dL_dverts_ndc, float* dL_dfaces_intense, void* stream);

typedef struct dm2_prep_desc {
    int32_t B, P, F;
    int32_t W, H;
    const float* verts;
    const int32_t* faces;
    const float* mv;
    const float* proj;
    float* verts_ndc;
    float* verts_image;
    float* aa_face_verts;
    float* aa_face_edges;
    uint8_t* aa_face_edges_iszero;
    float* aa_face_edges_recip;
    float* aa_face_edges_normal;
    float* aa_face_edges_normal_c;
} dm2_prep_desc;

int dm2_prepare_faces(const dm2_prep_desc* d, void* stream);
int dm2_prepare_faces_backward(const dm2_prep_desc* d, const float* g_verts_ndc, const float* g_verts_image,
                               const float* g_aa_face_verts, float* image_grad_scratch, float* g_verts,
                               void* stream);
size_t dm2_prepare_faces_camera_scratch_bytes(int32_t B, int32_t P);
int dm2_prepare_faces_backward_camera(const dm2_prep_desc* d, const float* g_verts_ndc, const float* g_verts_image,
                                      const float* g_aa_face_verts, float* image_grad_scratch, float* g_verts, float* g_mv,
                                      float* g_proj, void* camera_scratch, void* stream);

int dm2_exchange_mark(int32_t B, int32_t P, int32_t F, int32_t N, const int32_t* faces, const void* face_scratch, size_t face_bytes,
                      uint8_t* flags, uint32_t* counts, void* stream);
int dm2_exchange_pack(int32_t B, int32_t P, int32_t F, int32_t N, const uint8_t* flags, const uint32_t* counts, uint32_t* cursors,
                      const float* dverts, const float* dverts_color, const float* dfaces_opacity, const float* dfaces_intense,
                      float* send, void* stream);
int dm2_exchange_unpack(int32_t B, int32_t P, int32_t F, int32_t N, int32_t rank, const float* recv, const uint32_t* recv_counts,
                        int64_t rows, float* slice_v, float* slice_f, void* stream);

int dm2_debug_fetch(int what, int64_t count, int64_t aux, int64_t num_rendered,
                    const void* scratch, size_t scratch_bytes, void* dst, void* stream);

int dm2_debug_aa_overlap(int variant, int64_t n, const float* aa_face_verts, const float* aa_face_edges,
                         const uint8_t* aa_face_edges_iszero, const float* aa_face_edges_recip,
                         const float* aa_face_edges_normal, const float* aa_face_edges_normal_c,
                         const float* pixmin, float* area, float* grad, int32_t* code, void* stream);

#define DM2_PROFILE_STAGES 7
void dm2_profile_enable(int on);
int dm2_profile_read(float* ms, int capacity);

int dm2_debug_stamps(uint64_t* out, int capacity, int reset);

#ifdef __cplusplus
}
#endif
#endif
```

Baseline: 1067.

## Pipeline backward pool reads, batch tie-queue reservations, contract ray-triangle gradient

Restructures the fast backward kernel. Each tile now reserves a per-wave batch of tie-queue slots up front instead of issuing a wave atomic per chunk, and unused slots are padded with TIE_EMPTY markers that the tie pass skips. Coverage-ratio pool values are prefetched into LDS one chunk ahead with explicit vmcnt waits, and the scan of the next chunk overlaps the current one. The ray-triangle gradient is folded with dL/du and dL/dv into a contracted form, and global atomics are batched per wave. The trade-off is more scratch slack, empty queue entries to skip, and a fragile hand-written waitcnt protocol.

```diff
diff --git a/dmesh2_renderer_amd/_C.py b/dmesh2_renderer_amd/_C.py
--- a/dmesh2_renderer_amd/_C.py
+++ b/dmesh2_renderer_amd/_C.py
@@ -107,6 +107,7 @@
     "dm2_exchange_pack": (ctypes.c_int, [_i32, _i32, _i32, _i32, _vp, _vp, _vp, _vp, _vp, _vp, _vp, _vp, _vp]),
     "dm2_exchange_unpack": (ctypes.c_int, [_i32, _i32, _i32, _i32, _i32, _vp, _vp, _i64, _vp, _vp, _vp]),
     "dm2_debug_aa_overlap": (ctypes.c_int, [ctypes.c_int, _i64, _vp, _vp, _vp, _vp, _vp, _vp, _vp, _vp, _vp, _vp, _vp]),
+    "dm2_debug_ray_tri_grad": (ctypes.c_int, [ctypes.c_int, _i64, _vp, _vp, _vp, ctypes.c_int, _vp, _vp, _vp]),
     "dm2_debug_fetch": (ctypes.c_int, [ctypes.c_int, _i64, _i64, _i64, _vp, _sz, _vp, _vp]),
     "dm2_profile_enable": (None, [ctypes.c_int]),
     "dm2_profile_read": (ctypes.c_int, [ctypes.POINTER(ctypes.c_float), ctypes.c_int]),
@@ -514,7 +515,7 @@
             if mode not in (FWD_MASKS, FWD_NONE) and d.aa_temperature > 0.0 and not (d.flags & DM2_FLAG_LEGACY_KERNELS):
                 pool_pairs = max(0, bin_buf.numel() - lib.dm2_scratch_bytes(SCRATCH_BINNING, num_rendered, _tiles(B, W, H))) // 4
                 if pool_pairs > 0:
-                    tie_buf = _bytes(dev, lib.dm2_scratch_bytes(SCRATCH_TIE_QUEUE, pool_pairs, 0))
+                    tie_buf = _bytes(dev, lib.dm2_scratch_bytes(SCRATCH_TIE_QUEUE, pool_pairs, _tiles(B, W, H)))
             tail = (_ptr(face_buf), face_buf.numel(), _ptr(bin_buf), bin_buf.numel(), _ptr(img_buf), img_buf.numel(),
                     _ptr(tie_buf), tie_buf.numel() if tie_buf is not None else 0,
                     _ptr(g_verts), _ptr(g_color), _ptr(g_opac), _ptr(g_ndc), _ptr(g_int), _ptr(g_aa), _stream(dev))
@@ -1018,6 +1019,20 @@
     return area, grad, code
 
 
+def debug_ray_tri_grad(variant, ray_o, ray_d, tri, corrected, dL_duv):
+    lib = load_library()
+    dev = _require_gpu(ray_o, ray_d, tri, dL_duv)
+    f32 = torch.float32
+    n = ray_o.shape[0]
+    ts = [_c(ray_o, f32), _c(ray_d, f32), _c(tri, f32)]
+    g = _c(dL_duv, f32)
+    with torch.cuda.device(dev):
+        out = torch.zeros((n, 3, 3), dtype=f32, device=dev)
+        if lib.dm2_debug_ray_tri_grad(int(variant), n, *[_ptr(t) for t in ts], int(bool(corrected)), _ptr(g), _ptr(out), _stream(dev)):
+            raise _err(lib, "debug_ray_tri_grad")
+    return out
+
+
 def touched_faces(face_buf, B, F):
     t = debug_fetch(8, B * F, 1, 0, face_buf, torch.int32, B * F)
     return (t.view(B, F) != 0).any(dim=0)
diff --git a/dmesh2_renderer_amd/csrc/dm2_api.hip b/dmesh2_renderer_amd/csrc/dm2_api.hip
--- a/dmesh2_renderer_amd/csrc/dm2_api.hip
+++ b/dmesh2_renderer_amd/csrc/dm2_api.hip
@@ -184,7 +184,7 @@
         case DM2_SCRATCH_LAYER_IMAGE: dm2::LayerImageState::carve(nullptr, count, aux, &total); break;
         case DM2_SCRATCH_LAYER_TETS: return dm2::tet_scratch_bytes(count);
         case DM2_SCRATCH_PAIR_POOL: return dm2::BinningState::pool_bytes(count);
-        case DM2_SCRATCH_TIE_QUEUE: return count > 0 ? (size_t)count * sizeof(dm2::TieEntry) + dm2::ALIGN : 0;
+        case DM2_SCRATCH_TIE_QUEUE: return count > 0 ? (size_t)(count + aux * dm2::TIE_SLACK_PER_TILE) * sizeof(dm2::TieEntry) + dm2::ALIGN : 0;
         default: return 0;
     }
     return total;
@@ -342,7 +342,7 @@
                             (forward_mode == DM2_FWD_POOL || forward_mode == DM2_FWD_UNKNOWN || forward_mode == DM2_FWD_POINT);
     if (pool_route) {
         if (forward_mode == DM2_FWD_POOL && bs.pool_cap <= 0) return fail("forward_mode is DM2_FWD_POOL but the binning scratch has no pool part");
-        if (tie_cap < bs.pool_cap) return fail("tie scratch too small for the pool part of the binning scratch");
+        if (tie_cap < bs.pool_cap + Tn * dm2::TIE_SLACK_PER_TILE) return fail("tie scratch too small for the pool part of the binning scratch");
     }
     dm2::launch_render_backward(*d, is.ranges, bs.face_list, is, dL_dout_color, dL_dout_depth, dL_dverts, dL_dverts_color,
                                 dL_dfaces_opacity, dL_dverts_ndc, dL_dfaces_intense, dL_daa_face_verts, bs, forward_mode, tie_queue, tie_cap,
@@ -699,6 +699,16 @@
     return 0;
 }
 
+int dm2_debug_ray_tri_grad(int variant, int64_t n, const float* ray_o, const float* ray_d, const float* tri, int corrected,
+                           const float* dL_duv, float* dL_dtri, void* stream) {
+    if (variant < 0 || variant > 1) return fail("dm2_debug_ray_tri_grad: unknown variant");
+    if (n < 0) return fail("dm2_debug_ray_tri_grad: negative count");
+    if (n > 0 && (!ray_o || !ray_d || !tri || !dL_duv || !dL_dtri)) return fail("dm2_debug_ray_tri_grad: null pointer");
+    dm2::launch_debug_ray_tri_grad(variant, n, ray_o, ray_d, tri, corrected != 0, dL_duv, dL_dtri, (hipStream_t)stream);
+    DM2_HIP(hipGetLastError());
+    return 0;
+}
+
 int dm2_debug_fetch(int what, int64_t count, int64_t aux, int64_t num_rendered, const void* scratch, size_t scratch_bytes,
                     void* dst, void* stream) {
     hipStream_t st = (hipStream_t)stream;
diff --git a/dmesh2_renderer_amd/csrc/dm2_backward_fast.hip b/dmesh2_renderer_amd/csrc/dm2_backward_fast.hip
--- a/dmesh2_renderer_amd/csrc/dm2_backward_fast.hip
+++ b/dmesh2_renderer_amd/csrc/dm2_backward_fast.hip
@@ -32,6 +32,19 @@
     static constexpr int CAND = 32, BLOCKS = 3;
 };
 
+constexpr uint32_t TIE_BATCH = DM2_TIE_BATCH;
+__device__ __forceinline__ void vmcnt_wait_leaving(int later) {
+    later = __builtin_amdgcn_readfirstlane(later);
+    if (later <= 0) asm volatile("s_waitcnt vmcnt(0)" ::: "memory");
+    else if (later == 1) asm volatile("s_waitcnt vmcnt(1)" ::: "memory");
+    else if (later == 2) asm volatile("s_waitcnt vmcnt(2)" ::: "memory");
+    else if (later == 3) asm volatile("s_waitcnt vmcnt(3)" ::: "memory");
+    else asm volatile("s_waitcnt vmcnt(4)" ::: "memory");
+}
+__device__ __forceinline__ void global_atomic_add(float* p, float v) {
+    __hip_atomic_fetch_add((__attribute__((address_space(1))) float*)p, v, __ATOMIC_RELAXED, __HIP_MEMORY_SCOPE_AGENT);
+}
+
 template <Coverage COV, bool ALPHA>
 __global__ void __launch_bounds__(TILE_PIX, BfTraits<COV>::BLOCKS)
 k_render_backward_fast(dm2_render_desc d, const uint2* __restrict__ ranges, const uint32_t* __restrict__ face_list,
@@ -66,6 +79,7 @@
     __shared__ float s_pixc[6][TILE_PIX];
     __shared__ float* s_fl_base[32];
     __shared__ int s_fl_sel[32];
+    __shared__ uint32_t s_tie0;
 
     const uint32_t gx = (d.W + TILE - 1) / TILE, gy = (d.H + TILE - 1) / TILE;
     uint32_t tile;
@@ -73,7 +87,7 @@
     const int b = (int)(tile / (gx * gy));
     const uint32_t tyx = tile - (uint32_t)b * gx * gy;
     const int tile_y = (int)(tyx / gx), tile_x = (int)(tyx - (uint32_t)tile_y * gx);
-    const int tid = threadIdx.x, lane = tid & 63, wid = tid >> 6;
+    const int tid = threadIdx.x, lane = tid & 63, wid = __builtin_amdgcn_readfirstlane(tid >> 6);
     STAMP_DECL
     s_mask[tid] = 0;
     const int lx = tid & 15, ly = tid >> 4;
@@ -90,13 +104,15 @@
     const int total = (int)min((uint32_t)__builtin_amdgcn_readfirstlane(is.tile_max_lc[tile]), range.y - range.x);
     const uint4* const grecs = is.face_recs + (int64_t)b * d.F * FACE_REC_U4;
     auto walk_entry = [&](int k) -> int64_t { return (int64_t)range.x + (uint32_t)(total - 1 - k); };
-    const int rl = lane / REC_CHUNKS, rp = lane - rl * REC_CHUNKS;
-    const int rsrc = BfTraits<COV>::src_part(rp);
+    auto request_lane = [&]() { int l = lane; asm volatile("" : "+v"(l)); return l; };
     auto request_ids = [&](int buf, int nb) {
+        const int lane = request_lane();
         if (wid == 2 && nb + lane < total)
             glds4(face_list + walk_entry(nb + lane), &s_ids2[buf][0]);
     };
     if (total > 0) request_ids(0, 0);
+    uint32_t tie0 = 0u;
+    if (COV == POOL && tid == 0 && total > 0) tie0 = atomicAdd(hit_valid + 2, 4u * TIE_BATCH);
 
     uint32_t last_contributor = 0;
     float T = 0.f;
@@ -131,6 +147,7 @@
     const float temp = d.aa_temperature;
     const float pix_area = 1.0f;
     const float bg0 = d.background[0], bg1 = d.background[1], bg2 = d.background[2];
+    asm volatile("" :: "v"(bg0), "v"(bg1), "v"(bg2));
 
     bool T_first_pass = true;
     float accum_rec0 = 0.f, accum_rec1 = 0.f, accum_rec2 = 0.f, accum_recd = 0.f;
@@ -138,6 +155,9 @@
 
     auto request_chunk = [&](int buf, int nb, const uint32_t* ids) {
         const int nc2 = min(BM_CAND, total - nb);
+        const int lane = request_lane();
+        const int rl = lane / REC_CHUNKS, rp = lane - rl * REC_CHUNKS;
+        const int rsrc = BfTraits<COV>::src_part(rp);
         if (wid == 1 && (lane >> 1) < nc2)
             glds16(hit_masks + walk_entry(nb + (lane >> 1)) * 4 + (lane & 1) * 2, &s_hit2[buf][0]);
         if (COV == POOL && wid == 3 && lane < nc2) glds4(hit_base + walk_entry(nb + lane), &s_hb2[buf][0]);
@@ -155,25 +175,23 @@
         lds_prefetch_wait();
     }
     for (int k = tid; k < BM_CAND * BM_ACC; k += TILE_PIX) acc[k] = 0.f;
+    if (COV == POOL && tid == 0) s_tie0 = tie0;
     __syncthreads();
-
-    STAMP(0)
-    int n = 0, cur = 0;
-    for (int base = 0; base < total; base += n, cur ^= 1) {
-        STAMP(1)
-        const int nc = min(BM_CAND, total - base);
-        Rec* const recs = recs2[cur];
-        const unsigned long long* const s_hit = s_hit2[cur];
-        const uint32_t* const s_ids = s_ids2[cur];
-        const uint32_t* const s_hb = s_hb2[cur];
-        STAMP(2)
-        const ulonglong2 hh = reinterpret_cast<const ulonglong2*>(s_hit)[lane];
+    uint32_t tq_next = 0u, tq_end = 0u;
+    if (COV == POOL && total > 0) {
+        tq_next = (uint32_t)__builtin_amdgcn_readfirstlane((int)(s_tie0 + (uint32_t)wid * TIE_BATCH));
+        tq_end = tq_next + TIE_BATCH;
+    }
+    float* const pool_row = reinterpret_cast<float*>(s_mark[wid]);
+
+    auto scan_chunk = [&](int buf, int nc, int& n_, int& S_, uint32_t& mk_) {
+        const ulonglong2 hh = reinterpret_cast<const ulonglong2*>(s_hit2[buf])[lane];
         const unsigned long long h0 = (2 * lane < nc * 4) ? hh.x : 0ull, h1 = (2 * lane + 1 < nc * 4) ? hh.y : 0ull;
         const int c0 = __popcll(h0), c1 = __popcll(h1);
         const int inc = wave_inclusive_scan(c0 + c1);
         const int b0 = inc - c0 - c1, b1 = inc - c1;
-        n = max(1, __popcll(__ballot((lane & 1) && inc <= TILE_PIX && (lane >> 1) < nc)));
-        const int S = __builtin_amdgcn_readlane(inc, 2 * n - 1);
+        n_ = max(1, __popcll(__ballot((lane & 1) && inc <= TILE_PIX && (lane >> 1) < nc)));
+        S_ = __builtin_amdgcn_readlane(inc, 2 * n_ - 1);
         if ((lane & 1) == (wid >> 1) && (lane >> 1) < BM_CAND) s_wbase[wid][lane >> 1] = (uint16_t)((wid & 1) ? b1 : b0);
         if (COV == POOL && (lane & 1) == 0 && (lane >> 1) < BM_CAND) s_efirst[wid][lane >> 1] = (uint16_t)b0;
         const int lo_pair = wid * 64;
@@ -187,7 +205,29 @@
           if (e0) { const int l = 63 - __clzll((long long)e0); seed = ((uint32_t)(2 * l + 1) << 9) | (uint32_t)__builtin_amdgcn_readlane(b0, l); }
           if (e1) { const int l = 63 - __clzll((long long)e1); seed = max(seed, ((uint32_t)(2 * l + 2) << 9) | (uint32_t)__builtin_amdgcn_readlane(b1, l)); } }
         __builtin_amdgcn_fence(__ATOMIC_SEQ_CST, "wavefront");
-        const uint32_t mk = max(wave_inclusive_max(mark_row[lane]), seed);
+        mk_ = max(wave_inclusive_max(mark_row[lane]), seed);
+    };
+    auto request_pool = [&](int buf, int S_, uint32_t mk_) {
+        if (tid < S_) {
+            const int jn = ((int)(mk_ >> 9) - 1) >> 2;
+            glds4(pool + (s_hb2[buf][jn] + (uint32_t)(tid - (int)s_efirst[wid][jn])), pool_row);
+        }
+    };
+
+    STAMP(0)
+    int n = 0, S = 0, cur = 0;
+    uint32_t mk = 0u;
+    int flush_atomics = 0;
+    if (total > 0) {
+        scan_chunk(0, min(BM_CAND, total), n, S, mk);
+        if constexpr (COV == POOL) request_pool(0, S, mk);
+    }
+    for (int base = 0; base < total; cur ^= 1) {
+        STAMP(1)
+        Rec* const recs = recs2[cur];
+        const unsigned long long* const s_hit = s_hit2[cur];
+        const uint32_t* const s_ids = s_ids2[cur];
+        STAMP(2)
         STAMP(3)
 
         const bool have = tid < S;
@@ -208,7 +248,7 @@
                 seg_area_grad(recs[j].aa, pxmin, pxmin + 1, pymin, pymin + 1, pix_area, oarea, dg, recs[j].opacity > 0.9f);
                 ratio = fmaxf(oarea, 0.0f) / pix_area;
             } else {
-                ratio = COV == POINT ? 1.0f : pool[s_hb[j] + (uint32_t)(tid - (int)s_efirst[wid][j])];
+                ratio = 1.0f;
             }
             const Rec& fc = recs[j];
             BfPair out; out.alpha = 0.f; out.c0 = out.c1 = out.c2 = out.depth = 0.f; out.flags = 0;
@@ -220,6 +260,10 @@
 #pragma unroll
             for (int c = 0; c < 9; c++) k_col[c] = fc.col[c];
             k_dep[0] = fc.dep[0]; k_dep[1] = fc.dep[1]; k_dep[2] = fc.dep[2]; k_int = fc.intense; k_opa = fc.opacity;
+            if constexpr (COV == POOL) {
+                vmcnt_wait_leaving(flush_atomics);
+                ratio = pool_row[lane];
+            }
             if (ray_tri_intersection(ro, rd, p0, p1, p2, tuv)) {
                 float iuc, ivc;
                 clamp_bary_uv(tuv.y, tuv.z, iuc, ivc, code);
@@ -299,6 +343,8 @@
         __syncthreads();
         STAMP(8)
 
+        bool tie_push = false;
+        float dL_doarea = 0.f;
         {
             const int jkey = have ? j : -1;
             const int l16 = tid & 15;
@@ -316,7 +362,7 @@
             seg_scan16(nact, s1, s2, s4, s8);
             const bool emit = ((l16 == 15) | (kn != jkey)) & (jkey >= 0) & (nact > 0.f);
             float* const arow = acc + j * BM_ACC;
-            float dL_diu = 0.f, dL_div = 0.f, dL_doarea = 0.f;
+            float dL_diu = 0.f, dL_div = 0.f;
             ISA_MARK(D_group1)
             {
                 float g1[14];
@@ -327,25 +373,27 @@
                     const float qc0 = s_pixc[0][q], qc1 = s_pixc[1][q], qc2 = s_pixc[2][q], qd = s_pixc[3][q];
                     const float intense = k_int, opacity = k_opa;
                     const float* const colD = k_col; const float* const depD = k_dep;
-                    const float dics[3] = {qc0 * alpha * Tq, qc1 * alpha * Tq, qc2 * alpha * Tq};
-                    const float did = qd * alpha * Tq;
+                    const float aT = alpha * Tq;
+                    const float dics[3] = {qc0 * aT, qc1 * aT, qc2 * aT};
+                    const float did = qd * aT;
                     g1[12] = dL_dalpha * ratio;
                     const float dL_dratio = (dL_dalpha * opacity) * temp;
                     dL_doarea = dL_dratio / pix_area;
                     float dL_di0 = 0.f, dL_di1 = 0.f, dL_di2 = 0.f, dL_dfint = 0.f;
 #pragma unroll
                     for (int ch = 0; ch < 3; ch++) {
-                        dL_di0 += colD[ch] * dics[ch] * intense;
-                        dL_di1 += colD[3 + ch] * dics[ch] * intense;
-                        dL_di2 += colD[6 + ch] * dics[ch] * intense;
-                        g1[ch] = 0.f + i0 * dics[ch] * intense;
-                        g1[3 + ch] = 0.f + i1 * dics[ch] * intense;
-                        g1[6 + ch] = 0.f + i2 * dics[ch] * intense;
+                        const float dci = dics[ch] * intense;
+                        dL_di0 += colD[ch] * dci;
+                        dL_di1 += colD[3 + ch] * dci;
+                        dL_di2 += colD[6 + ch] * dci;
+                        g1[ch] = i0 * dci;
+                        g1[3 + ch] = i1 * dci;
+                        g1[6 + ch] = i2 * dci;
                         dL_dfint += (i0 * colD[ch] + i1 * colD[3 + ch] + i2 * colD[6 + ch]) * dics[ch];
                     }
                     g1[13] = dL_dfint;
                     dL_di0 += depD[0] * did; dL_di1 += depD[1] * did; dL_di2 += depD[2] * did;
-                    g1[9] = 0.f + i0 * did; g1[10] = 0.f + i1 * did; g1[11] = 0.f + i2 * did;
+                    g1[9] = i0 * did; g1[10] = i1 * did; g1[11] = i2 * did;
                     float diuc_diu, diuc_div, divc_diu, divc_div;
                     clamp_bary_uv_grad(code, diuc_diu, diuc_div, divc_diu, divc_div);
                     const float di0_diu = -1.f * diuc_diu + -1.f * divc_diu, di0_div = -1.f * diuc_div + -1.f * divc_div;
@@ -364,9 +412,6 @@
                 }
             }
             ISA_MARK(D_group2)
-            bool tie_push = false;
-            uint32_t tie_base = 0;
-            unsigned long long tie_bal = 0;
             if constexpr (COV == CLIP) {
                 float g2[6];
 #pragma unroll
@@ -389,8 +434,6 @@
                 const bool use = active && !tie;
 #pragma unroll
                 for (int c = 0; c < 6; c++) g2[c] = use ? dL_doarea * g2[c] : 0.0f;
-                tie_bal = __ballot(tie_push);
-                if (tie_bal && lane == (int)(__ffsll((long long)tie_bal) - 1)) tie_base = atomicAdd(hit_valid + 2, (uint32_t)__popcll(tie_bal));
                 seg_scan16_safe(g2, m1, m2, m4, m8, s1, s2, s4, s8);
                 if (emit) {
 #pragma unroll
@@ -404,11 +447,8 @@
                 for (int c = 0; c < 9; c++) g3[c] = 0.f;
                 if (active) {
                     const f3 ro = k_ro, rd = k_rd, p0 = k_p0, p1 = k_p1, p2 = k_p2;
-                    f3 du0, du1, du2, dv0, dv1, dv2;
-                    ray_tri_intersection_grad<true>(ro, rd, p0, p1, p2, corrected, du0, du1, du2, dv0, dv1, dv2);
-                    const f3 dp0 = dL_diu * du0 + dL_div * dv0;
-                    const f3 dp1 = dL_diu * du1 + dL_div * dv1;
-                    const f3 dp2 = dL_diu * du2 + dL_div * dv2;
+                    f3 dp0, dp1, dp2;
+                    ray_tri_intersection_grad_contracted(ro, rd, p0, p1, p2, corrected, dL_diu, dL_div, dp0, dp1, dp2);
                     g3[0] = dp0.x; g3[1] = dp0.y; g3[2] = dp0.z;
                     g3[3] = dp1.x; g3[4] = dp1.y; g3[5] = dp1.z;
                     g3[6] = dp2.x; g3[7] = dp2.y; g3[8] = dp2.z;
@@ -418,12 +458,6 @@
 #pragma unroll
                     for (int c = 0; c < 9; c++) atomicAdd(arow + M_DV + c, g3[c]);
                 }
-            }
-            if (tie_bal) {
-                const uint32_t tb = (uint32_t)__shfl((int)tie_base, __ffsll((long long)tie_bal) - 1);
-                const uint32_t at = tb + __builtin_amdgcn_mbcnt_hi((uint32_t)(tie_bal >> 32), __builtin_amdgcn_mbcnt_lo((uint32_t)tie_bal, 0u));
-                if (tie_push && at < tie_cap)
-                    tie_queue[at] = tie_pack((uint32_t)recs[j].face_id, (uint32_t)b, (uint32_t)(X0 + (q & 15)), (uint32_t)(Y0 + (q >> 4)), dL_doarea);
             }
         }
         STAMP(9)
@@ -431,28 +465,70 @@
         __syncthreads();
         STAMP(10)
 
+        if constexpr (COV == POOL) {
+            const unsigned long long tie_bal = __ballot(tie_push);
+            if (tie_bal) {
+                const uint32_t cnt = (uint32_t)__popcll(tie_bal), room = tq_end - tq_next;
+                const uint32_t rank = __builtin_amdgcn_mbcnt_hi((uint32_t)(tie_bal >> 32), __builtin_amdgcn_mbcnt_lo((uint32_t)tie_bal, 0u));
+                uint32_t fresh = 0u;
+                if (cnt > room) {
+                    uint32_t t = 0u;
+                    if (lane == 0) t = atomicAdd(hit_valid + 2, cnt - room + TIE_BATCH);
+                    fresh = (uint32_t)__builtin_amdgcn_readfirstlane((int)t);
+                }
+                const uint32_t at = rank < room ? tq_next + rank : fresh + (rank - room);
+                if (tie_push && at < tie_cap)
+                    tie_queue[at] = tie_pack((uint32_t)recs[j].face_id, (uint32_t)b, (uint32_t)(X0 + (q & 15)), (uint32_t)(Y0 + (q >> 4)), dL_doarea);
+                if (cnt > room) { tq_next = fresh + (cnt - room); tq_end = tq_next + TIE_BATCH; }
+                else tq_next += cnt;
+            }
+        }
+        int n_next = 0, S_next = 0;
+        uint32_t mk_next = 0u;
+        const int nbase = base + n;
+        if (nbase < total) {
+            scan_chunk(cur ^ 1, min(BM_CAND, total - nbase), n_next, S_next, mk_next);
+            if constexpr (COV == POOL) request_pool(cur ^ 1, S_next, mk_next);
+        }
+
         const int comp = tid & 31;
-        if (comp < (COV == POINT ? M_AA : M_N)) {
+        {
+            const bool comp_live = comp < (COV == POINT ? M_AA : M_N);
             float* const basep = s_fl_base[comp];
             const int entry = s_fl_sel[comp];
             const bool corner = (entry & 0x80) != 0;
             int sel0, mult;
             flush_id_and_mult(entry, 0u, sel0, mult);
-            for (int e = tid >> 5; e < n; e += TILE_PIX / 32) {
+            flush_atomics = 0;
+            for (int e0 = __builtin_amdgcn_readfirstlane(2 * wid); e0 < n; e0 += TILE_PIX / 32) {
+                const int e = e0 + (lane >> 5);
                 float* a = acc + e * BM_ACC;
-                const float flag = a[M_FLAG];
-                const float val = a[comp];
-                int sel = sel0;
-                if (corner) { int m_; flush_id_and_mult(entry, rec_zmask(recs[e]), sel, m_); }
-                const int id = (&recs[e].face_id)[sel];
-                if (flag != 0.f) {
-                    a[comp] = 0.f;
-                    if (comp == 0) a[M_FLAG] = 0.f;
-                    atomicAdd(basep + (int64_t)id * mult, val);
+                bool add = false;
+                float val = 0.f;
+                int id = 0;
+                if (comp_live && e < n) {
+                    add = a[M_FLAG] != 0.f;
+                    val = a[comp];
+                    int sel = sel0;
+                    if (corner) { int m_; flush_id_and_mult(entry, rec_zmask(recs[e]), sel, m_); }
+                    id = (&recs[e].face_id)[sel];
+                }
+                if (__ballot(add)) {
+                    if constexpr (COV == POOL) flush_atomics++;
+                    if (add) {
+                        a[comp] = 0.f;
+                        if (comp == 0) a[M_FLAG] = 0.f;
+                        global_atomic_add(basep + (int64_t)id * mult, val);
+                    }
                 }
             }
         }
         STAMP(11)
+        base = nbase; n = n_next; S = S_next; mk = mk_next;
+    }
+    if constexpr (COV == POOL) {
+        const uint32_t at = tq_next + (uint32_t)lane;
+        if (at < tq_end && at < tie_cap) tie_queue[at] = tie_pack(TIE_EMPTY, 0u, 0u, 0u, 0.0f);
     }
     STAMP_FLUSH
 }
@@ -468,9 +544,9 @@
     const uint32_t lane = threadIdx.x & 63u;
     for (uint32_t i0 = (blockIdx.x * blockDim.x + threadIdx.x) - lane; i0 < n; i0 += gridDim.x * blockDim.x) {
         const uint32_t i = i0 + lane;
-        const bool valid = i < n;
-        TieEntry e = tie_pack(0u, 0u, 0u, 0u, 0.0f);
-        if (valid) e = queue[i];
+        TieEntry e = tie_pack(TIE_EMPTY, 0u, 0u, 0u, 0.0f);
+        if (i < n) e = queue[i];
+        const bool valid = e.face != TIE_EMPTY;
         uint32_t b, x, y;
         tie_unpack(e, b, x, y);
         const int64_t bf = (int64_t)b * d.F + e.face;
diff --git a/dmesh2_renderer_amd/csrc/dm2_debug.hip b/dmesh2_renderer_amd/csrc/dm2_debug.hip
--- a/dmesh2_renderer_amd/csrc/dm2_debug.hip
+++ b/dmesh2_renderer_amd/csrc/dm2_debug.hip
@@ -59,4 +59,31 @@
                        pixmin, area, grad, code);
 }
 
+__global__ void __launch_bounds__(64)
+k_debug_ray_tri_grad(int variant, int64_t n, const float* __restrict__ ro, const float* __restrict__ rd, const float* __restrict__ tri,
+                     bool corrected, const float* __restrict__ dL_duv, float* __restrict__ out) {
+    const int64_t i = (int64_t)blockIdx.x * blockDim.x + threadIdx.x;
+    if (i >= n) return;
+    const f3 o = {ro[3 * i], ro[3 * i + 1], ro[3 * i + 2]}, dd = {rd[3 * i], rd[3 * i + 1], rd[3 * i + 2]};
+    const float* t = tri + 9 * i;
+    const f3 p0 = {t[0], t[1], t[2]}, p1 = {t[3], t[4], t[5]}, p2 = {t[6], t[7], t[8]};
+    const float gu = dL_duv[2 * i], gv = dL_duv[2 * i + 1];
+    f3 dp0, dp1, dp2;
+    if (variant == 0) {
+        f3 du0, du1, du2, dv0, dv1, dv2;
+        ray_tri_intersection_grad<true>(o, dd, p0, p1, p2, corrected, du0, du1, du2, dv0, dv1, dv2);
+        dp0 = gu * du0 + gv * dv0; dp1 = gu * du1 + gv * dv1; dp2 = gu * du2 + gv * dv2;
+    } else {
+        ray_tri_intersection_grad_contracted(o, dd, p0, p1, p2, corrected, gu, gv, dp0, dp1, dp2);
+    }
+    float* w = out + 9 * i;
+    w[0] = dp0.x; w[1] = dp0.y; w[2] = dp0.z; w[3] = dp1.x; w[4] = dp1.y; w[5] = dp1.z; w[6] = dp2.x; w[7] = dp2.y; w[8] = dp2.z;
 }
+
+void launch_debug_ray_tri_grad(int variant, int64_t n, const float* ro, const float* rd, const float* tri, bool corrected,
+                               const float* dL_duv, float* out, hipStream_t st) {
+    if (n <= 0) return;
+    hipLaunchKernelGGL(k_debug_ray_tri_grad, dim3((unsigned)((n + 63) / 64)), dim3(64), 0, st, variant, n, ro, rd, tri, corrected, dL_duv, out);
+}
+
+}
diff --git a/dmesh2_renderer_amd/csrc/dm2_device_math.h b/dmesh2_renderer_amd/csrc/dm2_device_math.h
--- a/dmesh2_renderer_amd/csrc/dm2_device_math.h
+++ b/dmesh2_renderer_amd/csrc/dm2_device_math.h
@@ -84,6 +84,33 @@
     dv_dp0 = -dv_dE1 - dv_dE2 - dv_dT;
     du_dp1 = du_dE1; dv_dp1 = dv_dE1;
     du_dp2 = du_dE2; dv_dp2 = dv_dE2;
+}
+
+__device__ __forceinline__ void ray_tri_intersection_grad_contracted(f3 ro, f3 rd, f3 p0, f3 p1, f3 p2, bool corrected,
+                                                                     float dL_diu, float dL_div, f3& dp0, f3& dp1, f3& dp2) {
+    const f3 T = ro - p0, E1 = p1 - p0, E2 = p2 - p0;
+    const f3 dxE2 = cross(rd, E2);
+    const float v1 = dot(dxE2, E1);
+    const float denom_inv = rcp_refined(v1 * v1);
+    const float v0 = dot(dxE2, T);
+    const f3 E1xd = cross(E1, rd);
+    const f3 TxE1 = cross(T, E1), Txd = cross(T, rd);
+    const float a = dL_diu * denom_inv, b = dL_div * denom_inv;
+    const float av1 = a * v1, bv1 = b * v1;
+    f3 dE1, dE2, dT;
+    if (!corrected) {
+        const float s = a * v0 + b * dot(TxE1, E2);
+        dE1 = cross(E2, T) * bv1 - dxE2 * s;
+        dE2 = (Txd * av1 + TxE1 * bv1) - E1xd * s;
+        dT = dxE2 * av1 + cross(E1, E2) * bv1;
+    } else {
+        const float s = a * v0 + b * dot(TxE1, rd);
+        dE1 = (-Txd) * bv1 - dxE2 * s;
+        dE2 = Txd * av1 - E1xd * s;
+        dT = dxE2 * av1 + E1xd * bv1;
+    }
+    dp0 = -(dE1 + dE2 + dT);
+    dp1 = dE1; dp2 = dE2;
 }
 
 __device__ __forceinline__ void clamp_bary_uv(float u, float v, float& u_c, float& v_c, int& code) {
diff --git a/dmesh2_renderer_amd/csrc/dm2_forward_queue.hip b/dmesh2_renderer_amd/csrc/dm2_forward_queue.hip
--- a/dmesh2_renderer_amd/csrc/dm2_forward_queue.hip
+++ b/dmesh2_renderer_amd/csrc/dm2_forward_queue.hip
@@ -233,7 +233,11 @@
 
         if (base + n < total) request_ids(base + n);
         uint32_t cbase = 0;
-        if (pool && tid == 0) cbase = atomicAdd(hit_valid + 1, (uint32_t)S);
+        if (pool && tid == 0) {
+            uint32_t word = 1u;
+            asm volatile("" : "+v"(word));
+            cbase = atomicAdd(hit_valid + word, (uint32_t)S);
+        }
         constexpr int FQ_ROUNDS = CLASSES ? (FQ_PAIRCAP + TILE_PIX - 1) / TILE_PIX : FQ_SURVCAP / TILE_PIX;
         const int ST = CLASSES ? ST0 : S;
         float pool_ratio[FQ_ROUNDS];
@@ -311,6 +315,7 @@
             }
         }
         STAMP(5)
+        asm volatile("" :: "v"(cbase));
         if (pool && tid == 0) s_cbase = cbase;
         lds_prefetch_wait();
         __syncthreads();
diff --git a/dmesh2_renderer_amd/csrc/dm2_state.h b/dmesh2_renderer_amd/csrc/dm2_state.h
--- a/dmesh2_renderer_amd/csrc/dm2_state.h
+++ b/dmesh2_renderer_amd/csrc/dm2_state.h
@@ -115,6 +115,11 @@
 };
 
 struct __attribute__((aligned(16))) TieEntry { uint32_t face, view_hi, pxy; float dL_doarea; };
+#ifndef DM2_TIE_BATCH
+#define DM2_TIE_BATCH 32
+#endif
+constexpr uint32_t TIE_EMPTY = 0xFFFFFFFFu;
+constexpr int64_t TIE_SLACK_PER_TILE = 4 * DM2_TIE_BATCH;
 __host__ __device__ inline TieEntry tie_pack(uint32_t face, uint32_t view, uint32_t x, uint32_t y, float g) {
     TieEntry e; e.face = face; e.view_hi = view | ((x >> 16) << 16) | ((y >> 16) << 24); e.pxy = (x & 0xFFFFu) | (y << 16); e.dL_doarea = g;
     return e;
@@ -164,6 +169,8 @@
 void launch_debug_aa_overlap(int variant, int64_t n, const float* tv, const float* te, const uint8_t* tz, const float* tr,
                              const float* tn, const float* tc, const float* pixmin, float* area, float* grad, int32_t* code,
                              hipStream_t st);
+void launch_debug_ray_tri_grad(int variant, int64_t n, const float* ro, const float* rd, const float* tri, bool corrected,
+                               const float* dL_duv, float* out, hipStream_t st);
 hipError_t launch_exchange_mark(int B, int P, int F, int N, const int32_t* faces, const uint32_t* tiles_touched, uint8_t* flags,
                                 uint32_t* counts, hipStream_t st);
 hipError_t launch_exchange_pack(int B, int P, int F, int N, const uint8_t* flags, const uint32_t* counts, uint32_t* cursors,
diff --git a/include/dm2_hip.h b/include/dm2_hip.h
--- a/include/dm2_hip.h
+++ b/include/dm2_hip.h
@@ -243,6 +243,9 @@
                          const float* aa_face_edges_normal, const float* aa_face_edges_normal_c,
                          const float* pixmin, float* area, float* grad, int32_t* code, void* stream);
 
+int dm2_debug_ray_tri_grad(int variant, int64_t n, const float* ray_o, const float* ray_d, const float* tri, int corrected,
+                           const float* dL_duv, float* dL_dtri, void* stream);
+
 #define DM2_PROFILE_STAGES 7
 void dm2_profile_enable(int on);
 int dm2_profile_read(float* ms, int capacity);
```

After: 1049. 0.983x the previous value.
